# tonyckc/WT-PSE-code

Hardware: AMD Instinct MI355X
Metric: training images/sec (256x256 fundus) — full WT-PSE iteration (higher is better)
Workload: dtype f32 (layers with > 16 output channels and the fused 1x1 heads: x2h (2 fp16 terms per fp32 operand — power-of-two operand scaling —, 3 fp16 MFMA products per multiply, fp32 accumulation); the 16-channel layers the same on 16x16x32, the 1-/3-channel input layers and small 1x1 convs fp32-input MFMA)

## Files before the change

include/wtpse_hip.h:

```cpp
#ifndef WTPSE_HIP_H
#define WTPSE_HIP_H
#ifdef __cplusplus
extern "C" {
#endif


int wtpse_pack_conv_weights(const float* params, const int* desc, int n_desc, float* packed, void* stream);

int wtpse_conv_fwd(const float* in0, int C0, const float* in1, int C1, const float* wpacked, const float* bias,
                   const float* pro0, const float* pro1, int pro_relu, float* out0, float* out1, int Csplit, float* stats,
                   int B, int H, int W, int Cout, int ksize, int relu_out, const float* mask_ref, unsigned* out_amax, void* stream);
int wtpse_conv_stats_blocks(int B, int H, int W);
int wtpse_conv_fwd_gram(const float* in0, int C0, const float* wpacked, const float* bias, const float* pro0, int pro_relu,
                        float* out0, float* gram_partial, int B, int H, int W, int Cout, int relu_out, unsigned* out_amax,
                        void* stream);

int wtpse_conv_x3_stats_blocks(int B, int H, int W, int Cout, int ksize);
int wtpse_x3r_enable(int on);
int wtpse_x3_xcd(int on);
int wtpse_x3_small_wide(int on);
int wtpse_x3_terms(int terms);
int wtpse_amax(const float* x, long long n, unsigned* amax_table, void* stream);
int wtpse_pack_conv_weights_x3(const float* params, const int* desc, int n_desc, unsigned short* packed, void* stream);
int wtpse_conv_fwd_x3(const float* in0, int C0, const float* in1, int C1, const unsigned short* wpacked, const float* bias,
                      const float* pro0, const float* pro1, int pro_relu, float* out0, float* out1, int Csplit, float* stats,
                      int B, int H, int W, int Cout, int ksize, int relu_out, const float* mask_ref, const unsigned* in_amax,
                      const unsigned* in_amax1, unsigned* out_amax, void* stream);

int wtpse_conv16_x3(const float* in0, int C0, const unsigned short* wx16, const float* bias, const float* pro0, int pro_relu,
                    float* out0, float* stats, float* gram_partial, const float* mask_ref, const float* bn_ss,
                    const float* bn_mean, int bn_relu, int B, int H, int W, int Cout, int relu_out, int in_is_grad,
                    const unsigned* in_amax, unsigned* out_amax, void* stream);
int wtpse_pack_conv16_x3(const float* params, const int* desc, int n_desc, unsigned short* packed, void* stream);

int wtpse_dgrad_bnb(const float* dy, int C, const float* wpacked, float* out0, float* out1, int Csplit, const float* bn_y,
                    const float* bn_ss, const float* bn_mean, int bn_relu, int bn_c0, int bn_c1, float* stats, int B, int H, int W,
                    int Cout, int ksize, void* stream);
int wtpse_dgrad_x3_bnb(const float* dy, int C, const unsigned short* wpacked, float* out0, float* out1, int Csplit,
                       const float* bn_y, const float* bn_ss, const float* bn_mean, int bn_relu, int bn_c0, int bn_c1, float* stats,
                       int B, int H, int W, int Cout, int ksize, const unsigned* in_amax, void* stream);

int wtpse_conv_fwd_bnf(const float* in0, int C0, const float* in1, int C1, const void* wpacked, int layout, const float* bias,
                       const float* pro0, const float* pro1, int pro_relu, float* out0, float* stats, const float* gamma,
                       const float* beta, float* running_mean, float* running_var, long long* num_batches, float momentum, float eps,
                       float* scale_shift, float* save_mean, float* save_invstd, double* partial2, unsigned* tickets, int B, int H,
                       int W, int Cout, int ksize, const unsigned* in_amax0, const unsigned* in_amax1, unsigned* act_amax, void* stream);

int wtpse_bnb_tail_partial2(int nblk, int Cout);
int wtpse_bnb_tail_tickets(int nblk, int Cout);
int wtpse_dgrad_bnb_coef(const float* dy, int C, const void* wpacked, int layout, float* out0, float* out1, int Csplit,
                         const float* bn_y, const float* bn_ss, const float* bn_mean, int bn_relu, int bn_c0, int bn_c1,
                         float* stats, const float* gamma, const float* invstd, float* coef, float* dgamma, float* dbeta,
                         int accumulate, double* partial2, unsigned* tickets, int B, int H, int W, int Cout, int ksize,
                         const unsigned* in_amax, void* stream);
int wtpse_dgrad_bnb_coef_frozen(const float* dy, int C, const void* wpacked, int layout, float* out0, float* out1, int Csplit,
                                const float* bn_y, const float* bn_ss, const float* bn_mean, int bn_relu, int bn_c0, int bn_c1,
                                float* stats, const float* gamma, const float* invstd, float* coef, float* dgamma, float* dbeta,
                                float* dbias, int accumulate, double* partial2, unsigned* tickets, int B, int H, int W, int Cout,
                                int ksize, const unsigned* in_amax, void* stream);

int wtpse_conv_wgrad(const float* dy, const float* x0, int C0, const float* x1, int C1, const float* pro0,
                     const float* pro1, int pro_relu, float* slab, float* dbias_slab, int ksplit, float* dw, float* dbias, int accumulate, int B, int H,
                     int W, int Cout, int ksize, void* stream);
int wtpse_wgrad_ksplit(int B, int H, int W, int Cin, int Cout);
int wtpse_wgrad_x3_supported(int Cin, int Cout, int ksize, int C0);
int wtpse_wgrad_x3_ksplit(int B, int H, int W, int Cin, int Cout);
int wtpse_conv_wgrad_x3(const float* dy, const float* x0, int C0, const float* x1, int C1, const float* pro0,
                        const float* pro1, int pro_relu, float* slab, int ksplit, float* dw, int accumulate, int B, int H, int W,
                        int Cout, int ksize, void* stream);

int wtpse_wgrad_r_supported(int Cin, int Cout, int ksize, int C0, int W);
int wtpse_wgrad_r_slabs(int B, int H, int W, int Cin, int Cout);
int wtpse_conv_wgrad_r(const float* dy, const float* x0, int C0, const float* x1, int C1, const float* pro0,
                       const float* pro1, int pro_relu, float* slab, float* dbias_slab, int nslab, float* dw, float* dbias,
                       int accumulate, int B, int H, int W, int Cout, const unsigned* dy_amax, const unsigned* x_amax0,
                       const unsigned* x_amax1, void* stream);

int wtpse_conv_wgrad_r_bn(const float* g, const float* bn_y, const float* bn_coef, const float* x0, int C0, const float* x1,
                          int C1, const float* pro0, const float* pro1, int pro_relu, float* slab, int nslab, float* dw,
                          int accumulate, int B, int H, int W, int Cout, void* stream);

int wtpse_bn_finalize(const float* stats_partial, int nblk, int C, long long count, const float* gamma, const float* beta,
                      float* running_mean, float* running_var, long long* num_batches, float momentum, float eps,
                      float* scale_shift, float* save_mean, float* save_invstd, unsigned* act_amax, void* stream);
int wtpse_act_bound(const float* scale_shift, int C, const unsigned* raw_amax, unsigned* act_amax, void* stream);
int wtpse_bn_eval_coeffs(const float* gamma, const float* beta, const float* running_mean, const float* running_var,
                         float eps, int C, float* scale_shift, void* stream);
int wtpse_affine_act(const float* y, const float* scale_shift, int relu, float* z, int B, int C, int HW, void* stream);
int wtpse_bn_bwd(const float* dz, const float* y, const float* scale_shift, int relu, const float* gamma,
                 const float* save_mean, const float* save_invstd, float* partial, float* coef, float* dgamma,
                 float* dbeta, int accumulate, float* dy, int B, int C, int HW, unsigned* amax, void* stream);
int wtpse_bn_bwd_nsplit(int B, int C, int HW);
int wtpse_bn_bwd_reduce(const float* dz, const float* y, const float* scale_shift, int relu, const float* save_mean,
                        const float* save_invstd, float* partial, float* sums_local, int B, int C, int HW, void* stream);
int wtpse_bn_bwd_apply(const float* dz, const float* y, const float* scale_shift, int relu, const float* gamma,
                       const float* save_mean, const float* save_invstd, const float* sums_local, const float* sums_global,
                       long long count_global, float* coef, float* dgamma, float* dbeta, int accumulate, float* dy, int B,
                       int C, int HW, unsigned* amax, void* stream);
int wtpse_bn_bwd_from_stats(const float* g, const float* y, const float* stats_partial, int nblk, const float* gamma,
                            const float* save_mean, const float* save_invstd, float* coef, float* dgamma, float* dbeta,
                            int accumulate, float* dy, int B, int C, int HW, unsigned* amax, void* stream);

int wtpse_bn_bwd_finalize_coef(const float* stats_partial, int nblk, int C, long long count, const float* gamma,
                               const float* save_mean, const float* save_invstd, float* coef, float* dgamma, float* dbeta,
                               int accumulate, void* stream);
int wtpse_bn_bwd_apply_coef(const float* g, const float* y, const float* coef, float* dy, int B, int C, int HW, unsigned* amax, void* stream);

int wtpse_bn_eval_coeffs_stats(const float* gamma, const float* beta, const float* running_mean, const float* running_var,
                               float eps, int C, float* scale_shift, float* save_mean, float* save_invstd, void* stream);
int wtpse_bn_bwd_frozen(const float* dz, const float* y, const float* scale_shift, int relu, const float* gamma,
                        const float* mean, const float* invstd, float* partial, float* coef, float* dgamma, float* dbeta,
                        float* dbias, int accumulate, float* dy, int B, int C, int HW, unsigned* amax, void* stream);
int wtpse_bn_bwd_from_stats_frozen(const float* g, const float* stats_partial, int nblk, const float* gamma, const float* invstd,
                                   float* coef, float* dgamma, float* dbeta, float* dbias, int accumulate, float* dy, int B, int C,
                                   int HW, unsigned* amax, void* stream);
int wtpse_bn_bwd_finalize_coef_frozen(const float* stats_partial, int nblk, int C, const float* gamma, const float* invstd,
                                      float* coef, float* dgamma, float* dbeta, float* dbias, int accumulate, void* stream);
int wtpse_bn_bwd_scale_coef(const float* g, const float* coef, float* dy, int B, int C, int HW, unsigned* amax, void* stream);

int wtpse_wt_loss_fwd(const float* z, int B, int C, int HW, float eps, float margin, int domain_num, int per_domain,
                      float* partial, float* gram, float* v, float* offdiag, float* diag, double* rowval,
                      float* dmmd_dv, float* losses, void* stream);
int wtpse_wt_split(int B, int HW, int* chunk_out);
int wtpse_wt_loss_fwd_partials(const float* partial, int S, int B, int HW, float eps, float margin, int domain_num,
                               int per_domain, float* gram, float* v, float* offdiag, float* diag, double* rowval,
                               float* dmmd_dv, float* losses, void* stream);
int wtpse_wt_gram_fwd(const float* z, int B, int C, int HW, float eps, float* partial, float* gram, float* v, float* offdiag,
                      float* diag, void* stream);
int wtpse_wt_final(const float* offdiag, const float* diag, int B, int Bnorm, float margin, const double* rowval, int R,
                   float* losses, void* stream);
int wtpse_wt_loss_bwd(const float* z, int B, int C, int HW, float margin, int domain_num, int per_domain,
                      const float* gram, const float* offdiag, const float* diag, const float* dmmd_dv,
                      const float* g_off, const float* g_diag, const float* g_dom, float w_off, float w_diag, float w_dom,
                      float* Mws, float* dz, int accumulate, void* stream);
int wtpse_wt_combine(const float* losses, int nmaps, float den, int mode, float* out, void* stream);
int wtpse_mmd_fwd(const float* v, int domain_num, int per_domain, double* rowval, float* dmmd_dv, void* stream);

int wtpse_maxpool2_fwd(const float* x, const float* pro, int relu, float* out, int B, int C, int H, int W, void* stream);
int wtpse_maxpool2_bwd(const float* x, const float* pro, int relu, const float* dout, float* dx, int accumulate, int B,
                       int C, int H, int W, void* stream);
int wtpse_maxpool2_bwd_stats_blocks(int B, int H, int W);
int wtpse_maxpool2_bwd_bnb(const float* x, const float* pro, int relu, const float* dout, float* dx, int accumulate,
                           const float* mean, float* stats, int B, int C, int H, int W, void* stream);
int wtpse_upsample2x_fwd(const float* x, const float* pro, int relu, float* out, int B, int C, int H, int W, void* stream);
int wtpse_upsample2x_bwd(const float* dout, float* dx, int accumulate, int B, int C, int H, int W, unsigned* amax, void* stream);
int wtpse_upsample2x_bwd_bn(const float* g, const float* bn_y, const float* bn_coef, float* dx, int B, int C, int H, int W,
                            unsigned* amax, void* stream);
int wtpse_upsample2x_fwd_stats(const float* x, float* out, float* stats, int B, int C, int H, int W, void* stream);
int wtpse_upsample2x_stats_blocks(int B, int H, int W);

int wtpse_resize_bilinear(const float* x, float* out, int B, int C, int H, int W, int Ho, int Wo, void* stream);

int wtpse_attn_fuse_fwd(const float* z, const float* wb, const float* emb, float coef, float* att, float* att_pre,
                        float* mask, float* fuse, int B, int CE, int HW, void* stream);
int wtpse_attn_fuse_bwd(const float* dfuse, const float* z, const float* emb, const float* att, const float* wb, float coef,
                        float* demb, float* dz, float* partial, float* d_wb, int accumulate, int B, int CE, int HW,
                        void* stream);

int wtpse_reparam_fwd(const float* mu, const float* logvar, const float* eps, float* z, long long n, void* stream);
int wtpse_reparam_bwd(const float* dz, const float* logvar, const float* eps, float* dlogvar, long long n, void* stream);
int wtpse_exp_half(const float* logvar, float* std_, long long n, void* stream);
int wtpse_reparam_student(const float* mu, const float* std_, const float* eps, float* z, long long n, void* stream);
int wtpse_nan_scrub(float* x, long long n, int* flag, void* stream);
int wtpse_randn(float* out, long long n, unsigned long long seed, unsigned long long offset,
                const unsigned long long* offset_dev, void* stream);
int wtpse_counter_add(void* counter, long long inc, int is64, void* stream);

int wtpse_reduce_blocks(long long n);
int wtpse_bce_sigmoid_fwd(const float* x, const float* t, long long n, float* partial, float* loss, void* stream);
int wtpse_bce_sigmoid_bwd(const float* x, const float* t, const float* g, float w, long long n, float* dx, void* stream);
int wtpse_pos_weight(const float* mask, const float* t, long long n, float* partial, float* sums, float* pw, void* stream);
int wtpse_pos_weight_from_sums(const float* sums, float* pw, void* stream);
int wtpse_bce_logits_pw_fwd(const float* x, const float* mask, const float* t, const float* pw, long long n, float* partial,
                            float* loss, void* stream);
int wtpse_bce_logits_pw_bwd(const float* x, const float* mask, const float* t, const float* pw, const float* g, float w,
                            long long n, float* dx, void* stream);
int wtpse_mse_fwd(const float* a, const float* b, long long n, float* partial, float* loss, void* stream);
int wtpse_mse_bwd(const float* a, const float* b, const float* g, float w, long long n, float* da, void* stream);
int wtpse_roi(const float* image, const float* logit, float* roi, float* od_pred, int B, int C, int HW, void* stream);
int wtpse_adam(float* p, const float* g, float* m, float* v, long long n, double lr, double beta1, double beta2, double eps,
               int step, const int* step_dev, void* stream);
int wtpse_adam_dev(float* p, const float* g, float* m, float* v, long long n, const float* lr_dev, double beta1, double beta2,
                   double eps, int step, const int* step_dev, const int* hold, void* stream);
int wtpse_loss_log(const float* s0, const float* s1, const float* s2, const float* s3, const float* s4, const float* s5,
                   double* acc, int check_n, int* flag, const int* step_dev, void* stream);

int wtpse_avg_step(float* a0, const float* p0, long long n0, float* a1, const float* p1, long long n1, float* a2, const float* p2,
                   long long n2, float* a3, const float* p3, long long n3, int* count, const int* gate, const int* hold, void* stream);
int wtpse_avg_merge(float* acc, const float* seg, long long n, long long n_acc, long long n_seg, void* stream);

int wtpse_head_fwd(const float* x, const float* pro, int pro_relu, const float* w1, const float* b1, const float* w2,
                   const float* b2, const float* w3, const float* b3, int nc, float* h1, float* h2, float* y,
                   const unsigned* x_amax, int B, int HW, void* stream);
int wtpse_head_bwd(const float* dy, const float* x, const float* pro, int pro_relu, const float* h1, const float* h2,
                   const float* w1, const float* b1, const float* w2, const float* w3, int nc, float* dx, float* slab,
                   float* dparams, int accumulate, const unsigned* x_amax, const unsigned* dy_amax, int B, int HW, void* stream);
int wtpse_head_slabs(int B, int HW);

int wtpse_resample_u8(const unsigned char* in, unsigned char* out, const int* bounds, const int* kk, const int* tab, int ksize,
                      int N, int Hin, int Win, int C, int L, int vertical, void* stream);
int wtpse_input_finish(const unsigned char* img, const unsigned char* od, const int* xidx, const int* yidx, float* image,
                       float* od_out, float* oc_out, int N, int S, void* stream);
int wtpse_image_finish(const unsigned char* img, float* image, int N, int S, void* stream);

int wtpse_uniform_f64(double* out, long long n, unsigned long long seed, unsigned long long pos, void* stream);
int wtpse_aug_blur(const double* src, double* dst, const double* w, const int* src_index, int radius, int planes, int S, int axis,
                   int pre, double post, void* stream);
int wtpse_aug_geometry(const unsigned char* img, const unsigned char* od, const int* xidx, const int* yidx, const int* code,
                       unsigned char* img_out, unsigned char* mask_out, int N, int S, void* stream);
int wtpse_aug_warp(const unsigned char* img, const unsigned char* mask, const double* disp, const int* slot, unsigned char* img_out,
                   unsigned char* mask_out, int N, int S, void* stream);
int wtpse_aug_photometric(unsigned char* img, const unsigned char* lut, const int* rect, const int* pts, const int* pt_off,
                          const int* pt_val, int max_pts, int N, int S, void* stream);

int wtpse_postprocess_ws(int B, int h, int w);
int wtpse_postprocess(const float* logit, unsigned char* out, void* ws, float threshold, int B, int h, int w, void* stream);
int wtpse_seg_metrics_ws(int B, int h, int w);
int wtpse_seg_metrics(const unsigned char* mask, const float* label, long long* rec, void* ws, int B, int h, int w, void* stream);

int wtpse_overlay_ws(int B, int h, int w);
int wtpse_overlay(const float* img, const unsigned char* pred_od, const unsigned char* pred_oc, const unsigned char* gt_od,
                  const unsigned char* gt_oc, unsigned char* original, unsigned char* overlay, void* ws, int B, int h, int w,
                  void* stream);
int wtpse_label_thresholds(const unsigned char* mask, float* od, float* oc, long long n, void* stream);

int wtpse_overlay_pred_ws(int B, int h, int w);
int wtpse_overlay_pred(const float* img, const unsigned char* pred_od, const unsigned char* pred_oc, unsigned char* original,
                       unsigned char* overlay, int B, int h, int w, void* stream);
int wtpse_label_map(const unsigned char* disc, const unsigned char* cup, unsigned char* out, long long n, void* stream);
int wtpse_mask_geometry(const unsigned char* mask, long long* rec, int B, int h, int w, void* stream);
int wtpse_onh_profile(const unsigned char* disc, const unsigned char* cup, const long long* geom, const int* table, unsigned* profile,
                      long long* moments, int N, int B, int h, int w, void* stream);

int wtpse_locate_cells(const unsigned char* img, long long* cells, int N, int H, int W, int c, int t, void* stream);
int wtpse_crop_u8(const unsigned char* img, const int* boxes, unsigned char* out, int H, int W, int C, int M, int s, void* stream);
int wtpse_paste_u8(unsigned char* canvas, const unsigned char* patch, int H, int W, int C, int h, int w, int top, int left, void* stream);

#define WTPSE_CAL_BINS 1024
#define WTPSE_CAL_REC (2 * (WTPSE_CAL_BINS + 1) * 2 + 4)
int wtpse_calibration_hist(const float* prob, const float* spread, const float* label, const unsigned char* region, float threshold,
                           unsigned* rec, int B, int h, int w, void* stream);

int wtpse_shape_samples(const float* emb, int CE, const float* mu, const float* logvar, const float* wb, float coef,
                        const float* wout, const float* bout, const float* wz, float scale, int K, unsigned long long seed,
                        unsigned long long offset, const float* noise, float threshold, float* mean, float* std_,
                        unsigned char* votes, float* logits, int B, int HW, void* stream);

int wtpse_shape_samples_mask(const float* ref, float* mean, float* std_, unsigned char* votes, float* logits, int K, int B, int HW,
                             void* stream);

int wtpse_dihedral_views(const float* x, float* out, const int* codes, int V, int N, int S, void* stream);

int wtpse_views_merge(const float* logits, const int* codes, int V, int B, int K, int S, float threshold, float* logits_out,
                      float* mean, float* std_, unsigned char* votes, float* mean_logit, void* stream);

int wtpse_relu_mask(const float* dz, const float* ref, float* dy, int accumulate, long long n, void* stream);
int wtpse_axpy(float* dst, const float* src, float alpha, long long n, void* stream);
int wtpse_reduce_rows(const float* partial, int rows, int cols, float* out, int accumulate, float scale, void* stream);
int wtpse_zero(void* p, long long nbytes, void* stream);
int wtpse_copy_probe(const float* src, float* dst, long long n, int bytes_per_lane, void* stream);

int wtpse_dwt2_fwd(const float* x, float* coef, float* tmp, int planes, int H, int W, int wavelet, int levels, void* stream);
int wtpse_dwt2_inv(const float* coef, float* x, float* tmp, int planes, int H, int W, int wavelet, int levels, void* stream);

int wtpse_plan_fn_count(void);
const char* wtpse_plan_fn_name(int id);
void* wtpse_plan_create(void);
int wtpse_plan_destroy(void* plan);
int wtpse_plan_size(void* plan);
int wtpse_plan_add_call(void* plan, int fn, const void* args, int nargs, void* stream);
int wtpse_plan_add_wait(void* plan, void* waiter, void* waited);
int wtpse_plan_replay(void* plan);
int wtpse_tuning_state(void);

const char* wtpse_source_hash(void);

#ifdef __cplusplus
}
#endif
#endif
```

wt-pse-code_amd/wtpse_hip/csrc/conv.hip:

```cpp
#include "internal.h"

#define WTPSE_P16_KC(KS) ((KS) == 3 ? 4 : 8)

struct ConvArgs {
  const float* in0;
  const float* in1;
  const float* wp;
  const float* bias;
  const float* pro0;
  const float* pro1;
  float* out0;
  float* out1;
  float* stats;
  const float* mask;
  const unsigned* in_amax;
  float in_scale;
  unsigned* out_amax;
  float* gram;
  const float* bn_ss;
  const float* bn_mean;
  int bn_c0, bn_c1, bn_relu;
  BnbTail tail;
  BnfTail ftail;
  int B, H, W;
  int C0, C1, Cin, CinP;
  int Cout, CoutP, Csplit;
  int pro_relu;
  int relu_out;
  int tiles_x, tiles_y;
  int xcd_tiles;
};


template <bool P16> struct AccT { typedef f32x16 type; };
template <> struct AccT<true> { typedef f32x4 type; };
__device__ __forceinline__ f32x4 mfma(float a, float b, f32x4 c) { return mfma16(a, b, c); }
__device__ __forceinline__ f32x16 mfma(float a, float b, f32x16 c) { return mfma32(a, b, c); }

template <int PE>
struct PlaneStride {
  static constexpr int value = ((PE - 16 + 31) / 32) * 32 + 16;
};

template <int KS, int MODE, int TWL, bool DB, int EPI>
__global__ __launch_bounds__(256, 3) void conv_fwd_k(ConvArgs a) {
  constexpr bool MASK = EPI == 1, BNB = EPI == 2;
  constexpr int TAPS = KS * KS, PAD = KS / 2;
  constexpr int TW = 1 << TWL, TH = 256 / TW;
  constexpr int PITCH = TW + 2 * PAD, ROWS = TH + 2 * PAD;
  constexpr int PE = PITCH * ROWS;
  constexpr int NPOS = (PE + 255) / 256;
  constexpr int S = PlaneStride<NPOS * 256>::value;
  constexpr bool XP = (MODE == 3 || MODE == 4);
  constexpr int XT = MODE == 4 ? 2 : 3;
  constexpr bool P16 = (MODE == 0) || XP;
  static_assert(!XP || KS == 3, "MODE 3 / 4 is the 3x3 path");
  constexpr int MT = P16 ? 1 : MODE;
  constexpr int MB = P16 ? 16 : 32;
  constexpr int CB = MB * MT;
  constexpr int NT = P16 ? 4 : 2;
  constexpr int NB = P16 ? 16 : 32;
  constexpr int KC = P16 ? WTPSE_P16_KC(KS) : 8;
  constexpr int KQ = P16 ? 4 : 2;
  constexpr int NACC = P16 ? 4 : 16;
  constexpr int CB4 = CB / 4;
  constexpr int NW = (KC * TAPS * CB4 + 255) / 256;
  constexpr int PEP = (PE + 7) & ~7;
  constexpr int XS_SZ = XP ? 2 * XT * PEP * 4 : KC * S;
  constexpr int WS_SZ = XP ? 0 : NW * 1024;
  constexpr int GRAM_SZ = (P16 && KS == 3) ? 4 * 16 * 65 + 4 * 256 : 0;
  constexpr int RED_SZ = 4 * CB * 2 > GRAM_SZ ? 4 * CB * 2 : GRAM_SZ;
  constexpr int MAIN_SZ = (XS_SZ + WS_SZ) > RED_SZ ? (XS_SZ + WS_SZ) : RED_SZ;
  __shared__ __attribute__((aligned(16))) float smem[MAIN_SZ + CB + (BNB ? 4 * CB : 0)];
  float* bias_s = smem + MAIN_SZ;
  const float* bnp_s = bias_s + CB;
  float* Xs = smem;
  float* Ws = smem + XS_SZ;

  const int tid = threadIdx.x, lane = tid & 63, wave = tid >> 6;
  int tile = (int)blockIdx.x, cblk = (int)blockIdx.y;
  if (a.xcd_tiles > 0) {
    const int L = (int)(blockIdx.y * gridDim.x + blockIdx.x), sl = L >> 3;
    cblk = sl % (int)gridDim.y;
    tile = (L & 7) * a.xcd_tiles + sl / (int)gridDim.y;
  }
  int bx = tile;
  const int tx = bx % a.tiles_x;
  bx /= a.tiles_x;
  const int ty = bx % a.tiles_y;
  const int b = bx / a.tiles_y;
  const int cout0 = cblk * CB;
  const int HW = a.H * a.W;
  if (tid < CB) bias_s[tid] = (a.bias && cout0 + tid < a.Cout) ? a.bias[cout0 + tid] : 0.f;
  if (BNB && tid < CB) {
    const int c = cout0 + tid;
    const bool bn = c >= a.bn_c0 && c < a.bn_c1;
    float* q = bias_s + CB + tid;
    q[0] = (bn && a.bn_relu) ? a.bn_ss[2 * (c - a.bn_c0)] : 0.f;
    q[CB] = (bn && a.bn_relu) ? a.bn_ss[2 * (c - a.bn_c0) + 1] : 1.f;
    q[2 * CB] = bn ? a.bn_mean[c - a.bn_c0] : 0.f;
  }

  int off[NT];
#pragma unroll
  for (int nt = 0; nt < NT; ++nt) {
    int p = wave * 64 + nt * NB + (lane & (NB - 1));
    off[nt] = (p >> TWL) * PITCH + (p & (TW - 1));
  }

  typename AccT<P16>::type acc[MT][NT];
#pragma unroll
  for (int mt = 0; mt < MT; ++mt)
#pragma unroll
    for (int nt = 0; nt < NT; ++nt)
#pragma unroll
      for (int r = 0; r < NACC; ++r) acc[mt][nt][r] = 0.f;

  if constexpr (XP) {
    u32x4* Xq = reinterpret_cast<u32x4*>(smem);
    const int g4 = lane >> 4;
    constexpr int PB = (PE + 63) / 64, NIT = (2 * PB + 3) / 4;
    const __amdgpu_buffer_rsrc_t rs0 = make_rsrc(a.in0 + (size_t)b * a.C0 * HW, (unsigned)a.C0 * HW * 4u);
    const bool any_pro = MODE == 4 || a.pro0 != nullptr || a.pro_relu != 0;
    const unsigned sx_raw = MODE == 4 ? amax_load(a.in_amax) : 0u;
    __builtin_amdgcn_sched_barrier(0);
    float xv[NIT][8];
    int ipos[NIT], ihalf[NIT];
    bool iin[NIT];
    float psc[2][8], psh[2][8];
#pragma unroll
    for (int hh = 0; hh < 2; ++hh)
#pragma unroll
      for (int j = 0; j < 8; ++j) {
        const int cg = min(hh * 8 + j, a.C0 - 1);
        psc[hh][j] = a.pro0 ? a.pro0[2 * cg] : 1.f;
        psh[hh][j] = a.pro0 ? a.pro0[2 * cg + 1] : 0.f;
      }
#pragma unroll
    for (int i = 0; i < NIT; ++i) {
      const int blk = __builtin_amdgcn_readfirstlane(i * 4 + wave);
      ihalf[i] = blk >= PB ? 1 : 0;
      const int p = (blk - ihalf[i] * PB) * 64 + lane;
      ipos[i] = (blk < 2 * PB && p < PE) ? p : -1;
      const int r = p / PITCH, x = p - r * PITCH;
      const int gy = ty * TH + r - PAD, gx = tx * TW + x - PAD;
      iin[i] = ipos[i] >= 0 && gy >= 0 && gy < a.H && gx >= 0 && gx < a.W;
      const unsigned vo = iin[i] ? (unsigned)(gy * a.W + gx) * 4u : BUF_OOB;
#pragma unroll
      for (int j = 0; j < 8; ++j)
        xv[i][j] = buf_load(rs0, vo, (unsigned)min(ihalf[i] * 8 + j, a.C0) * (unsigned)HW * 4u);
    }
    const u32x4* wq = reinterpret_cast<const u32x4*>(a.wp) + 1 + (MODE == 4 ? 15 * 64 : 0);
    u32x4 afr[5][XT];
#pragma unroll
    for (int s5 = 0; s5 < 5; ++s5)
#pragma unroll
      for (int t = 0; t < XT; ++t) afr[s5][t] = wq[(s5 * XT + t) * 64 + lane];
    const float sx = MODE == 4 ? (a.in_amax ? x3_scale_from_amax(amax_reduce(sx_raw)) : a.in_scale) : 1.f;
    if constexpr (MODE == 4) {
#pragma unroll
      for (int hh = 0; hh < 2; ++hh)
#pragma unroll
        for (int j = 0; j < 8; ++j) {
          psc[hh][j] *= sx;
          psh[hh][j] *= sx;
        }
    }
    if (any_pro) {
      const float lo = (a.pro_relu & 1) ? 0.f : -INFINITY;
#pragma unroll
      for (int i = 0; i < NIT; ++i) {
        const int nc = iin[i] ? a.C0 - ihalf[i] * 8 : 0;
#pragma unroll
        for (int j = 0; j < 8; ++j) {
          const float sc = ihalf[i] ? psc[1][j] : psc[0][j], sh = ihalf[i] ? psh[1][j] : psh[0][j];
          const float v = fmaxf(fmaf(xv[i][j], sc, sh), lo);
          xv[i][j] = j < nc ? v : 0.f;
        }
      }
    }
#pragma unroll
    for (int i = 0; i < NIT; ++i) {
      if (ipos[i] >= 0) {
        u32x4 tt[XT];
#pragma unroll
        for (int j = 0; j < 4; ++j) {
          unsigned q0, q1, q2 = 0u;
          if constexpr (XT == 3) wt_split3_pair(xv[i][2 * j], xv[i][2 * j + 1], q0, q1, q2);
          else split2h_pair(xv[i][2 * j], xv[i][2 * j + 1], q0, q1);
          tt[0][j] = q0; tt[1][j] = q1;
          if constexpr (XT == 3) tt[2][j] = q2;
        }
#pragma unroll
        for (int t = 0; t < XT; ++t) Xq[(t * 2 + ihalf[i]) * PEP + ipos[i]] = tt[t];
      }
    }
    __syncthreads();
    int toff[5];
#pragma unroll
    for (int s5 = 0; s5 < 5; ++s5) {
      const int t = min(2 * s5 + (g4 >> 1), TAPS - 1);
      toff[s5] = (t / KS) * PITCH + (t % KS);
    }
    const int hsel = (g4 & 1) * PEP;
#pragma unroll
    for (int nt = 0; nt < NT; ++nt) {
#pragma unroll
      for (int s5 = 0; s5 < 5; ++s5) {
        u32x4 bfr[XT];
#pragma unroll
        for (int t = 0; t < XT; ++t) bfr[t] = Xq[(t * 2) * PEP + hsel + off[nt] + toff[s5]];
        f32x4 c = acc[0][nt];
        if constexpr (XT == 3) {
          c = wt_mfma16x32(afr[s5][0], bfr[2], c);
          c = wt_mfma16x32(afr[s5][1], bfr[1], c);
          c = wt_mfma16x32(afr[s5][2], bfr[0], c);
          c = wt_mfma16x32(afr[s5][0], bfr[1], c);
          c = wt_mfma16x32(afr[s5][1], bfr[0], c);
          c = wt_mfma16x32(afr[s5][0], bfr[0], c);
        } else {
          c = wt_mfma16x32h(afr[s5][0], bfr[1], c);
          c = wt_mfma16x32h(afr[s5][1], bfr[0], c);
          c = wt_mfma16x32h(afr[s5][0], bfr[0], c);
        }
        acc[0][nt] = c;
      }
    }
    if constexpr (MODE == 4) {
      const float inv = a.wp[0] / sx;
#pragma unroll
      for (int nt = 0; nt < NT; ++nt) acc[0][nt] *= inv;
    }
    __syncthreads();
  } else {
  int gpos[NPOS];
#pragma unroll
  for (int i = 0; i < NPOS; ++i) {
    int p = tid + 256 * i;
    int r = p / PITCH, x = p - r * PITCH;
    int gy = ty * TH + r - PAD, gx = tx * TW + x - PAD;
    gpos[i] = (p < PE && gy >= 0 && gy < a.H && gx >= 0 && gx < a.W) ? gy * a.W + gx : -1;
  }

  const __amdgpu_buffer_rsrc_t rs0 = make_rsrc(a.in0 + (size_t)b * a.C0 * HW, (unsigned)a.C0 * HW * 4u);
  const __amdgpu_buffer_rsrc_t rs1 = a.in1 ? make_rsrc(a.in1 + (size_t)b * a.C1 * HW, (unsigned)a.C1 * HW * 4u) : rs0;
  unsigned voff[NPOS];
#pragma unroll
  for (int i = 0; i < NPOS; ++i) voff[i] = gpos[i] >= 0 ? (unsigned)gpos[i] * 4u : BUF_OOB;
  const __amdgpu_buffer_rsrc_t rsw = make_rsrc(a.wp, (unsigned)a.CinP * TAPS * (unsigned)a.CoutP * 4u);
  unsigned woff[NW];
#pragma unroll
  for (int it = 0; it < NW; ++it) {
    const int e4 = tid + 256 * it;
    const int row = e4 / CB4, j4 = e4 - row * CB4;
    woff[it] = (row < KC * TAPS && cout0 + j4 * 4 < a.CoutP) ? (unsigned)(row * a.CoutP + cout0 + j4 * 4) * 4u : BUF_OOB;
  }
  const bool any_pro = a.pro0 != nullptr || a.pro1 != nullptr || a.pro_relu != 0;
  float xv[KC][NPOS];
  f32x4 wv[NW];
  auto issue_loads = [&](int c0) {
    const bool first = c0 < a.C0;
    const __amdgpu_buffer_rsrc_t rs = first ? rs0 : rs1;
    const int cbase = first ? c0 : c0 - a.C0;
    const int cmax = (first ? a.C0 : a.C1) - 1;
#pragma unroll
    for (int c = 0; c < KC; ++c) {
      const unsigned soff = (unsigned)min(cbase + c, cmax) * (unsigned)HW * 4u;
#pragma unroll
      for (int i = 0; i < NPOS; ++i) xv[c][i] = buf_load(rs, voff[i], soff);
    }
#pragma unroll
    for (int it = 0; it < NW; ++it) wv[it] = buf_load4(rsw, woff[it], (unsigned)(c0 * TAPS) * (unsigned)a.CoutP * 4u);
  };
  auto stash = [&](int c0) {
    const bool first = c0 < a.C0;
    if (any_pro) {
      const bool relu = first ? (a.pro_relu & 1) : (a.pro_relu & 2);
      const float* pro = first ? a.pro0 : a.pro1;
      const int cbase = first ? c0 : c0 - a.C0;
      const int cmax = (first ? a.C0 : a.C1) - 1;
#pragma unroll
      for (int c = 0; c < KC; ++c) {
        const int cg = min(cbase + c, cmax);
        const float sc = pro ? pro[2 * cg] : 1.f, sh = pro ? pro[2 * cg + 1] : 0.f;
#pragma unroll
        for (int i = 0; i < NPOS; ++i) {
          float v = fmaf(xv[c][i], sc, sh);
          if (relu) v = fmaxf(v, 0.f);
          xv[c][i] = gpos[i] >= 0 ? v : 0.f;
        }
      }
    }
#pragma unroll
    for (int c = 0; c < KC; ++c)
#pragma unroll
      for (int i = 0; i < NPOS; ++i) Xs[c * S + tid + 256 * i] = xv[c][i];
#pragma unroll
    for (int it = 0; it < NW; ++it) *reinterpret_cast<f32x4*>(Ws + (tid + 256 * it) * 4) = wv[it];
  };
  if (DB) issue_loads(0);
  for (int c0 = 0; c0 < a.CinP; c0 += KC) {
    const int kc = min(KC, a.CinP - c0);
    __syncthreads();
    if (!DB) issue_loads(c0);
    stash(c0);
    __syncthreads();
    if (DB && c0 + KC < a.CinP) issue_loads(c0 + KC);
    const int nq = kc / KQ;
    for (int q = 0; q < nq; ++q) {
      const int cl = q * KQ + (lane / NB);
      const float* xrow = Xs + cl * S;
      const float* wrow = Ws + cl * TAPS * CB + (lane & (MB - 1));
      float av[TAPS][MT], bv[TAPS][NT];
#pragma unroll
      for (int t = 0; t < TAPS; ++t) {
        const int toff = (t / KS) * PITCH + (t % KS);
#pragma unroll
        for (int mt = 0; mt < MT; ++mt) av[t][mt] = wrow[t * CB + mt * MB];
#pragma unroll
        for (int nt = 0; nt < NT; ++nt) bv[t][nt] = xrow[off[nt] + toff];
      }
#pragma unroll
      for (int t = 0; t < TAPS; ++t)
#pragma unroll
        for (int nt = 0; nt < NT; ++nt)
#pragma unroll
          for (int mt = 0; mt < MT; ++mt) acc[mt][nt] = mfma(av[t][mt], bv[t][nt], acc[mt][nt]);
    }
  }
  }
  if (a.bias) {
    float bz[MT][NACC];
#pragma unroll
    for (int mt = 0; mt < MT; ++mt)
#pragma unroll
      for (int r = 0; r < NACC; ++r)
        bz[mt][r] = bias_s[P16 ? ((lane >> 4) * 4 + r) : (mt * 32 + (r & 3) + 8 * (r >> 2) + 4 * (lane >> 5))];
#pragma unroll
    for (int mt = 0; mt < MT; ++mt)
#pragma unroll
      for (int r = 0; r < NACC; ++r)
#pragma unroll
        for (int nt = 0; nt < NT; ++nt) acc[mt][nt][r] += bz[mt][r];
  }

  const bool want_stats = a.stats != nullptr;
  if (want_stats) __syncthreads();
  float* red = smem;
  const int C1out = a.Cout - a.Csplit;
  int poff[NT];
#pragma unroll
  for (int nt = 0; nt < NT; ++nt) {
    int p = wave * 64 + nt * NB + (lane & (NB - 1));
    int gy = ty * TH + (p >> TWL), gx = tx * TW + (p & (TW - 1));
    poff[nt] = (gy < a.H && gx < a.W) ? gy * a.W + gx : -1;
  }
  const __amdgpu_buffer_rsrc_t rs_o0 = make_rsrc(a.out0 + (size_t)b * a.Csplit * HW, (unsigned)a.Csplit * HW * 4u);
  const __amdgpu_buffer_rsrc_t rs_o1 = a.out1 ? make_rsrc(a.out1 + (size_t)b * C1out * HW, (unsigned)C1out * HW * 4u) : rs_o0;
  const int Cbn = a.bn_c1 - a.bn_c0;
  const __amdgpu_buffer_rsrc_t rs_m = MASK ? make_rsrc(a.mask + (size_t)b * a.Cout * HW, (unsigned)a.Cout * HW * 4u)
                                      : BNB ? make_rsrc(a.mask + (size_t)b * Cbn * HW, (unsigned)Cbn * HW * 4u) : rs_o0;
  const int clane = P16 ? (lane >> 4) * 4 : (lane >> 5) * 4;
  unsigned pvo[NT];
#pragma unroll
  for (int nt = 0; nt < NT; ++nt) pvo[nt] = poff[nt] >= 0 ? (unsigned)(clane * HW + poff[nt]) * 4u : BUF_OOB;
  constexpr int NSV = NACC * 2;
  const bool full = ty * TH + TH <= a.H && tx * TW + TW <= a.W && cout0 + CB <= a.Cout;
  if (!full) {
#pragma unroll
    for (int mt = 0; mt < MT; ++mt)
#pragma unroll
      for (int r = 0; r < NACC; ++r) {
        const bool cvalid = cout0 + (P16 ? r : (mt * 32 + (r & 3) + 8 * (r >> 2))) + clane < a.Cout;
#pragma unroll
        for (int nt = 0; nt < NT; ++nt) acc[mt][nt][r] = (cvalid && poff[nt] >= 0) ? acc[mt][nt][r] : 0.f;
      }
  }
  if (a.relu_out) {
#pragma unroll
    for (int mt = 0; mt < MT; ++mt)
#pragma unroll
      for (int nt = 0; nt < NT; ++nt)
#pragma unroll
        for (int r = 0; r < NACC; ++r) acc[mt][nt][r] = out_clamp<EPI>(acc[mt][nt][r], 0.f);
  }
  if constexpr (P16 && KS == 3) {
    if (a.gram) {
      __syncthreads();
      float* zs = smem + wave * (16 * 65);
#pragma unroll
      for (int nt = 0; nt < NT; ++nt)
#pragma unroll
        for (int r = 0; r < NACC; ++r) zs[((lane >> 4) * 4 + r) * 65 + nt * 16 + (lane & 15)] = acc[0][nt][r];
      __builtin_amdgcn_wave_barrier();
      f32x4 g = {0.f, 0.f, 0.f, 0.f};
#pragma unroll
      for (int st = 0; st < 16; ++st) {
        const float v = zs[(lane & 15) * 65 + 4 * st + (lane >> 4)];
        g = mfma16(v, v, g);
      }
      float* gs = smem + 4 * 16 * 65 + wave * 256;
#pragma unroll
      for (int r = 0; r < 4; ++r) gs[((lane >> 4) * 4 + r) * 16 + (lane & 15)] = g[r];
      __syncthreads();
      const float* g0 = smem + 4 * 16 * 65;
      a.gram[(size_t)tile * 256 + tid] = g0[tid] + g0[256 + tid] + g0[512 + tid] + g0[768 + tid];
      __syncthreads();
    }
  }
  if constexpr (EPI == 0) {
    if (a.out_amax) {
      unsigned am = 0u;
#pragma unroll
      for (int mt = 0; mt < MT; ++mt)
#pragma unroll
        for (int nt = 0; nt < NT; ++nt)
#pragma unroll
          for (int r = 0; r < NACC; ++r) am = max(am, amax_bits(acc[mt][nt][r]));
      amax_publish_wave(a.out_amax, am, (unsigned)tile * 4u + (unsigned)wave);
    }
  }
  const unsigned hw4 = (unsigned)HW * 4u;
  const bool defer = want_stats && (BNB ? a.tail.tickets != nullptr : a.ftail.tickets != nullptr);
#pragma unroll
  for (int mt = 0; mt < MT; ++mt) {
    float mk[NACC][NT];
    if (MASK) {
#pragma unroll
      for (int r = 0; r < NACC; ++r) {
        const int cbase = cout0 + (P16 ? r : (mt * 32 + (r & 3) + 8 * (r >> 2)));
#pragma unroll
        for (int nt = 0; nt < NT; ++nt) mk[r][nt] = buf_load(rs_m, pvo[nt], (unsigned)min(cbase, a.Cout) * hw4);
      }
    }
    if (BNB) {
#pragma unroll
      for (int r = 0; r < NACC; ++r) {
        const int cbase = cout0 + (P16 ? r : (mt * 32 + (r & 3) + 8 * (r >> 2)));
        const bool bn = cbase >= a.bn_c0 && cbase < a.bn_c1;
        const unsigned soff = (unsigned)(bn ? cbase - a.bn_c0 : 0) * hw4;
#pragma unroll
        for (int nt = 0; nt < NT; ++nt) mk[r][nt] = buf_load(rs_m, bn ? pvo[nt] : BUF_OOB, soff);
      }
    }
    float bmu[NACC];
#pragma unroll
    for (int r = 0; r < NACC; ++r) {
      const int cbase = cout0 + (P16 ? r : (mt * 32 + (r & 3) + 8 * (r >> 2)));
      const bool second = a.out1 != nullptr && cbase >= a.Csplit;
      const __amdgpu_buffer_rsrc_t rs_o = second ? rs_o1 : rs_o0;
      const unsigned soff = (unsigned)(second ? min(cbase, a.Cout) - a.Csplit : min(cbase, a.Csplit)) * hw4;
      float bsc = 0.f, bsh = 1.f;
      bmu[r] = 0.f;
      if (BNB) {
        const int crel = (P16 ? r : (mt * 32 + (r & 3) + 8 * (r >> 2))) + clane;
        bsc = bnp_s[crel];
        bsh = bnp_s[CB + crel];
        bmu[r] = bnp_s[2 * CB + crel];
      }
#pragma unroll
      for (int nt = 0; nt < NT; ++nt) {
        float v = acc[mt][nt][r];
        if (MASK && !(mk[r][nt] > 0.f)) v = 0.f;
        if (BNB) {
          float zz = __builtin_fmaf(mk[r][nt], bsc, bsh);
          asm volatile("" : "+v"(zz));
          if (!(zz > 0.f)) v = 0.f;
          acc[mt][nt][r] = v;
        }
        if (!defer) buf_store(rs_o, pvo[nt], soff, v);
      }
    }
    if (want_stats) {
      float sv[NSV];
#pragma unroll
      for (int r = 0; r < NACC; ++r) {
        float s1 = 0.f, s2 = 0.f;
#pragma unroll
        for (int nt = 0; nt < NT; ++nt) {
#pragma clang fp contract(off)
          if (BNB) {
            const float v = acc[mt][nt][r];
            s1 += v;
            s2 += v * (mk[r][nt] - bmu[r]);
          } else {
            const float v = acc[mt][nt][r];
            s1 += v;
            s2 += v * v;
          }
        }
        sv[r * 2 + 0] = s1;
        sv[r * 2 + 1] = s2;
      }
      constexpr int LB = P16 ? 4 : 5;
      constexpr int HB = P16 ? 3 : 5;
#pragma unroll
      for (int st = 0; st < HB; ++st) {
        const int half = NSV >> (st + 1);
        const bool up = (lane >> st) & 1;
#pragma unroll
        for (int i = 0; i < NSV / 2; ++i) {
          if (i < half) {
            float keep = up ? sv[i + half] : sv[i];
            float send = up ? sv[i] : sv[i + half];
            sv[i] = keep + __shfl_xor(send, 1 << st, 64);
          }
        }
      }
#pragma unroll
      for (int st = HB; st < LB; ++st) sv[0] += __shfl_xor(sv[0], 1 << st, 64);
      int idx = 0;
#pragma unroll
      for (int st = 0; st < HB; ++st) idx += ((lane >> st) & 1) * (NSV >> (st + 1));
      const int k = idx & 1, rr = idx >> 1;
      const int crel = P16 ? ((lane >> 4) * 4 + rr) : (mt * 32 + (rr & 3) + 8 * (rr >> 2) + 4 * (lane >> 5));
      if (((lane & (NB - 1)) >> HB) == 0) red[(wave * CB + crel) * 2 + k] = sv[0];
    }
  }
  if (want_stats) {
    __syncthreads();
    if (tid < CB * 2) {
      int crel = tid >> 1;
      const float s = red[tid] + red[CB * 2 + tid] + red[2 * CB * 2 + tid] + red[3 * CB * 2 + tid];
      if (BNB) {
        const int c = cout0 + crel;
        if (c >= a.bn_c0 && c < a.bn_c1) pub_store(a.stats + ((size_t)tile * Cbn + c - a.bn_c0) * 2 + (tid & 1), s);
      } else if (cout0 + crel < a.Cout) {
        pub_store(a.stats + ((size_t)tile * a.Cout + cout0 + crel) * 2 + (tid & 1), s);
      }
    }
  }
  TailTicket tk;
  tk.old = 0u;
  tk.armed = 0;
  if (defer) {
    if constexpr (BNB) tk = bnb_tail_begin<CB>(a.tail, a.bn_c0, a.bn_c1, cout0, tile, cblk, tid);
    else tk = bnf_tail_begin(a.ftail, tile, cblk, tid);
  }
  if (defer) {
#pragma unroll
    for (int mt = 0; mt < MT; ++mt)
#pragma unroll
      for (int r = 0; r < NACC; ++r) {
        const int cbase = cout0 + (P16 ? r : (mt * 32 + (r & 3) + 8 * (r >> 2)));
        const bool second = a.out1 != nullptr && cbase >= a.Csplit;
        const __amdgpu_buffer_rsrc_t rs_o = second ? rs_o1 : rs_o0;
        const unsigned soff = (unsigned)(second ? min(cbase, a.Cout) - a.Csplit : min(cbase, a.Csplit)) * hw4;
#pragma unroll
        for (int nt = 0; nt < NT; ++nt) buf_store(rs_o, pvo[nt], soff, acc[mt][nt][r]);
      }
    if constexpr (BNB)
      bnb_tail<CB>(tk, a.tail, a.stats, a.bn_mean, a.bn_c0, a.bn_c1, cout0, tile, cblk, tid,
                   reinterpret_cast<double*>(red), reinterpret_cast<int*>(red + 520));
    else
      bnf_tail<CB>(tk, a.ftail, a.stats, a.Cout, cout0, tile, cblk, tid, reinterpret_cast<double*>(red),
                   reinterpret_cast<int*>(red + 520));
  }
}

template <int KS, int MODE, bool DB, int EPI>
static int launch_fwd(const ConvArgs& a, hipStream_t st) {
  constexpr int CB = (MODE == 0 || MODE == 3 || MODE == 4) ? 16 : 32 * MODE;
  ConvArgs args = a;
  const Tiling t = conv_tiling(a.B, a.H, a.W);
  args.tiles_x = t.tiles_x;
  args.tiles_y = t.tiles_y;
  dim3 grid((unsigned)t.tiles, (unsigned)ceil_div(a.CoutP, CB));
  static const bool xcd_on = [] { const char* e = getenv("WTPSE_C16_XCD"); return !(e && e[0] == '0'); }();
  args.xcd_tiles = (xcd_on && grid.x % 8 == 0 && (long long)grid.x * grid.y >= 64) ? (int)(grid.x / 8) : 0;
  const bool in_launch = tail_in_launch((long long)grid.x * grid.y);
  if (!in_launch) args.tail.tickets = args.ftail.tickets = nullptr;
  if (args.tail.tickets) bnb_tail_geometry(args.tail, (int)grid.x, a.Cout, (double)a.B * a.H * a.W);
  if (args.ftail.tickets) bnf_tail_geometry(args.ftail, (int)grid.x, a.Cout, (double)a.B * a.H * a.W);
  if (t.TW == 16)
    hipLaunchKernelGGL((conv_fwd_k<KS, MODE, 4, DB, EPI>), grid, dim3(256), 0, st, args);
  else
    hipLaunchKernelGGL((conv_fwd_k<KS, MODE, 5, DB, EPI>), grid, dim3(256), 0, st, args);
  const int rc = wtpse_status();
  return rc == 0 && !in_launch ? tail_after_launch(a, (int)grid.x, st) : rc;
}

extern "C" int wtpse_conv_stats_blocks(int B, int H, int W) { return conv_tiling(B, H, W).tiles; }

static int conv_check(const ConvCall& c, int layout) {
  const BnbArgs& bn = c.bn;
  const BnbTail& t = c.tail;
  const BnfTail& f = c.ftail;
  const bool bnb = bn.mean != nullptr;
  WTPSE_REQUIRE(layout == CONV_FP32 || layout == CONV_X3 || layout == CONV_C16);
  WTPSE_REQUIRE(c.in0 && c.w && c.out0 && c.B > 0 && c.H > 0 && c.W > 0 && c.C0 > 0 && c.C1 >= 0 && c.Cout > 0);
  WTPSE_REQUIRE(c.ksize == 1 || c.ksize == 3);
  WTPSE_REQUIRE((c.C1 == 0) == (c.in1 == nullptr));
  WTPSE_REQUIRE(c.Csplit > 0 && c.Csplit <= c.Cout && ((c.Csplit == c.Cout) == (c.out1 == nullptr)));
  WTPSE_REQUIRE(c.Csplit == c.Cout || c.Csplit % 16 == 0);
  WTPSE_REQUIRE(!(c.stats && c.relu_out));
  WTPSE_REQUIRE(bnb || !(c.stats && c.mask_ref));
  WTPSE_REQUIRE(bnb || !(c.mask_ref && c.out1));
  WTPSE_REQUIRE(!bnb || (c.mask_ref && c.stats && bn.ss && !c.bias && !c.relu_out && !c.gram && bn.c0 >= 0 && bn.c0 < bn.c1 &&
                         bn.c1 <= c.Cout && bn.c0 % 16 == 0 && (bn.c1 % 16 == 0 || bn.c1 == c.Cout)));
  WTPSE_REQUIRE(c.C1 == 0 || c.C0 % 16 == 0);
  WTPSE_REQUIRE(!(c.out_amax && (c.mask_ref || bnb)));
  WTPSE_REQUIRE(!c.gram || (c.Cout == 16 && !c.relu_out));
  WTPSE_REQUIRE(!t.tickets || (bnb && t.partial2 && t.gamma && t.invstd && t.coef && t.dgamma && t.dbeta));
  WTPSE_REQUIRE(!f.tickets || (!bnb && c.stats && !c.gram && f.partial2 && f.gamma && f.beta && f.scale_shift && f.save_mean &&
                               f.save_invstd && (f.rmean == nullptr) == (f.rvar == nullptr)));
  if (layout == CONV_X3) {
    const X3Tiling g = x3_tiling(c.B, c.H, c.W, c.Cout, c.ksize);
    WTPSE_REQUIRE(!c.gram && !(c.in_amax1 && !c.in1) && ((c.C0 + c.C1 + 15) & ~15) <= (g.mt == 2 && !g.half ? 512 : 256));
  }
  if (layout == CONV_C16)
    WTPSE_REQUIRE(c.ksize == 3 && c.C0 <= 16 && c.Cout <= 16 && (((uintptr_t)c.w) & 15) == 0 && !c.in1 && !c.pro1);
  return 0;
}

static int conv_launch_fwd(const ConvCall& c, bool c16, hipStream_t st) {
  const bool bnb = c.bn.mean != nullptr;
  ConvArgs a;
  a.tail = c.tail;
  a.ftail = c.ftail;
  a.bn_ss = c.bn.ss; a.bn_mean = c.bn.mean; a.bn_relu = c.bn.relu; a.bn_c0 = bnb ? c.bn.c0 : 0; a.bn_c1 = bnb ? c.bn.c1 : 0;
  a.in0 = c.in0; a.in1 = c.in1; a.wp = static_cast<const float*>(c.w); a.bias = c.bias; a.pro0 = c.pro0; a.pro1 = c.pro1;
  a.out0 = c.out0; a.out1 = c.out1; a.stats = c.stats; a.mask = c.mask_ref; a.gram = c.gram;
  a.in_amax = c16 ? c.in_amax0 : nullptr; a.in_scale = c16 ? X3_FWD_SCALE : 1.f; a.out_amax = c.out_amax;
  a.B = c.B; a.H = c.H; a.W = c.W; a.C0 = c.C0; a.C1 = c.C1; a.Cin = c.C0 + c.C1; a.CinP = c16 ? 16 : (a.Cin + 3) & ~3;
  a.Cout = c.Cout; a.CoutP = (c.Cout + 15) & ~15; a.Csplit = c.Csplit; a.pro_relu = c.pro_relu; a.relu_out = c.relu_out;
  a.tiles_x = a.tiles_y = 0;
#define FWD(KS, M, DB) (bnb ? launch_fwd<KS, M, DB, 2>(a, st) : c.mask_ref ? launch_fwd<KS, M, DB, 1>(a, st) : launch_fwd<KS, M, DB, 0>(a, st))
  if (c16) return (g_x3_terms == 2 && (!c.in_is_grad || c.in_amax0)) ? FWD(3, 4, false) : FWD(3, 3, false);
  int mode = c.Cout <= 16 ? 0 : (c.Cout % 64 == 0 ? 2 : 1);
  const int tiles = conv_tiling(c.B, c.H, c.W).tiles;
  if (mode == 2 && tiles * (a.CoutP / 64) < 512) mode = 1;
  if (mode == 1 && tiles * ceil_div(a.CoutP, 32) < 384) mode = 0;
  const int cb = mode == 0 ? 16 : 32 * mode;
  const bool db = tiles * ceil_div(a.CoutP, cb) < 768 && a.CinP > (mode == 0 ? WTPSE_P16_KC(c.ksize) : 8);
#define FWD_DB(KS, M) (db ? FWD(KS, M, true) : FWD(KS, M, false))
  if (c.ksize == 3) return mode == 0 ? FWD_DB(3, 0) : mode == 1 ? FWD_DB(3, 1) : FWD_DB(3, 2);
  return mode == 0 ? FWD_DB(1, 0) : mode == 1 ? FWD_DB(1, 1) : FWD_DB(1, 2);
#undef FWD_DB
#undef FWD
}

int conv_run(const ConvCall& c, int layout, hipStream_t st) {
  if (const int rc = conv_check(c, layout)) return rc;
  return layout == CONV_X3 ? conv_launch_x3(c, st) : conv_launch_fwd(c, layout == CONV_C16, st);
}

extern "C" int wtpse_conv_fwd(const float* in0, int C0, const float* in1, int C1, const float* wpacked,
                              const float* bias, const float* pro0, const float* pro1, int pro_relu, float* out0, float* out1,
                              int Csplit, float* stats, int B, int H, int W, int Cout, int ksize, int relu_out,
                              const float* mask_ref, unsigned* out_amax, void* stream) {
  ConvCall c;
  c.in0 = in0; c.C0 = C0; c.in1 = in1; c.C1 = C1; c.w = wpacked; c.bias = bias; c.pro0 = pro0; c.pro1 = pro1; c.pro_relu = pro_relu;
  c.out0 = out0; c.out1 = out1; c.Csplit = Csplit; c.stats = stats; c.mask_ref = mask_ref; c.out_amax = out_amax;
  c.B = B; c.H = H; c.W = W; c.Cout = Cout; c.ksize = ksize; c.relu_out = relu_out;
  return conv_run(c, CONV_FP32, (hipStream_t)stream);
}

extern "C" int wtpse_dgrad_bnb(const float* dy, int C, const float* wpacked, float* out0, float* out1, int Csplit,
                               const float* bn_y, const float* bn_ss, const float* bn_mean, int bn_relu, int bn_c0, int bn_c1,
                               float* stats, int B, int H, int W, int Cout, int ksize, void* stream) {
  WTPSE_REQUIRE(bn_y && bn_ss && bn_mean && stats);
  ConvCall c;
  c.in0 = dy; c.C0 = C; c.w = wpacked; c.out0 = out0; c.out1 = out1; c.Csplit = Csplit; c.stats = stats; c.mask_ref = bn_y;
  c.bn.ss = bn_ss; c.bn.mean = bn_mean; c.bn.relu = bn_relu; c.bn.c0 = bn_c0; c.bn.c1 = bn_c1;
  c.B = B; c.H = H; c.W = W; c.Cout = Cout; c.ksize = ksize;
  return conv_run(c, CONV_FP32, (hipStream_t)stream);
}

extern "C" int wtpse_conv16_x3(const float* in0, int C0, const unsigned short* wx16, const float* bias, const float* pro0,
                               int pro_relu, float* out0, float* stats, float* gram_partial, const float* mask_ref,
                               const float* bn_ss, const float* bn_mean, int bn_relu, int B, int H, int W, int Cout, int relu_out,
                               int in_is_grad, const unsigned* in_amax, unsigned* out_amax, void* stream) {
  ConvCall c;
  c.in0 = in0; c.C0 = C0; c.w = wx16; c.bias = bias; c.pro0 = pro0; c.pro_relu = pro_relu; c.out0 = out0; c.Csplit = Cout;
  c.stats = stats; c.gram = gram_partial; c.mask_ref = mask_ref; c.in_amax0 = in_amax; c.in_is_grad = in_is_grad; c.out_amax = out_amax;
  c.bn.ss = bn_ss; c.bn.mean = bn_mean; c.bn.relu = bn_relu; c.bn.c1 = Cout;
  c.B = B; c.H = H; c.W = W; c.Cout = Cout; c.ksize = 3; c.relu_out = relu_out;
  return conv_run(c, CONV_C16, (hipStream_t)stream);
}

extern "C" int wtpse_conv_fwd_bnf(const float* in0, int C0, const float* in1, int C1, const void* wpacked, int layout,
                                  const float* bias, const float* pro0, const float* pro1, int pro_relu, float* out0, float* stats,
                                  const float* gamma, const float* beta, float* running_mean, float* running_var,
                                  long long* num_batches, float momentum, float eps, float* scale_shift, float* save_mean,
                                  float* save_invstd, double* partial2, unsigned* tickets, int B, int H, int W, int Cout, int ksize,
                                  const unsigned* in_amax0, const unsigned* in_amax1, unsigned* act_amax, void* stream) {
  WTPSE_REQUIRE(stats && gamma && beta && scale_shift && save_mean && save_invstd && partial2 && tickets);
  ConvCall c;
  c.in0 = in0; c.C0 = C0; c.in1 = in1; c.C1 = C1; c.w = wpacked; c.bias = bias; c.pro0 = pro0; c.pro1 = pro1; c.pro_relu = pro_relu;
  c.out0 = out0; c.Csplit = Cout; c.stats = stats; c.in_amax0 = in_amax0; c.in_amax1 = in_amax1;
  BnfTail& t = c.ftail;
  t.partial2 = partial2; t.tickets = tickets; t.gamma = gamma; t.beta = beta; t.rmean = running_mean; t.rvar = running_var;
  t.nbt = num_batches; t.momentum = momentum; t.eps = eps; t.scale_shift = scale_shift; t.save_mean = save_mean;
  t.save_invstd = save_invstd; t.act_amax = act_amax;
  c.B = B; c.H = H; c.W = W; c.Cout = Cout; c.ksize = ksize;
  return conv_run(c, layout, (hipStream_t)stream);
}

extern "C" int wtpse_bnb_tail_partial2(int nblk, int Cout) { return bnb_tail_groups(nblk) * bnb_tail_ctot(Cout) * 2; }
extern "C" int wtpse_bnb_tail_tickets(int nblk, int Cout) { return bnb_tail_t2off(nblk, Cout) + (Cout + 15) / 16; }

static int dgrad_bnb_coef(ConvCall c, int layout, void* stream) {
  const BnbTail& t = c.tail;
  WTPSE_REQUIRE(c.mask_ref && c.bn.ss && c.bn.mean && c.stats && t.gamma && t.invstd && t.coef && t.dgamma && t.dbeta && t.partial2 &&
                t.tickets);
  c.in_is_grad = 1;
  return conv_run(c, layout, (hipStream_t)stream);
}

extern "C" int wtpse_dgrad_bnb_coef(const float* dy, int C, const void* wpacked, int layout, float* out0, float* out1, int Csplit,
                                    const float* bn_y, const float* bn_ss, const float* bn_mean, int bn_relu, int bn_c0, int bn_c1,
                                    float* stats, const float* gamma, const float* invstd, float* coef, float* dgamma,
                                    float* dbeta, int accumulate, double* partial2, unsigned* tickets, int B, int H, int W,
                                    int Cout, int ksize, const unsigned* in_amax, void* stream) {
  ConvCall c;
  c.in0 = dy; c.C0 = C; c.w = wpacked; c.out0 = out0; c.out1 = out1; c.Csplit = Csplit; c.stats = stats; c.mask_ref = bn_y;
  c.bn.ss = bn_ss; c.bn.mean = bn_mean; c.bn.relu = bn_relu; c.bn.c0 = bn_c0; c.bn.c1 = bn_c1; c.in_amax0 = in_amax;
  BnbTail& t = c.tail;
  t.partial2 = partial2; t.tickets = tickets; t.gamma = gamma; t.invstd = invstd; t.coef = coef; t.dgamma = dgamma; t.dbeta = dbeta;
  t.accumulate = accumulate;
  c.B = B; c.H = H; c.W = W; c.Cout = Cout; c.ksize = ksize;
  return dgrad_bnb_coef(c, layout, stream);
}

extern "C" int wtpse_dgrad_bnb_coef_frozen(const float* dy, int C, const void* wpacked, int layout, float* out0, float* out1,
                                           int Csplit, const float* bn_y, const float* bn_ss, const float* bn_mean, int bn_relu,
                                           int bn_c0, int bn_c1, float* stats, const float* gamma, const float* invstd, float* coef,
                                           float* dgamma, float* dbeta, float* dbias, int accumulate, double* partial2,
                                           unsigned* tickets, int B, int H, int W, int Cout, int ksize, const unsigned* in_amax,
                                           void* stream) {
  WTPSE_REQUIRE(dbias);
  ConvCall c;
  c.in0 = dy; c.C0 = C; c.w = wpacked; c.out0 = out0; c.out1 = out1; c.Csplit = Csplit; c.stats = stats; c.mask_ref = bn_y;
  c.bn.ss = bn_ss; c.bn.mean = bn_mean; c.bn.relu = bn_relu; c.bn.c0 = bn_c0; c.bn.c1 = bn_c1; c.in_amax0 = in_amax;
  BnbTail& t = c.tail;
  t.partial2 = partial2; t.tickets = tickets; t.gamma = gamma; t.invstd = invstd; t.coef = coef; t.dgamma = dgamma; t.dbeta = dbeta;
  t.dbias = dbias; t.accumulate = accumulate;
  c.B = B; c.H = H; c.W = W; c.Cout = Cout; c.ksize = ksize;
  return dgrad_bnb_coef(c, layout, stream);
}

__global__ __launch_bounds__(256) void pack_weights_x3p16_k(const float* __restrict__ params, const int* __restrict__ desc,
                                                            unsigned short* __restrict__ packed) {
  const int* d = desc + blockIdx.y * 8;
  const int w_off = d[0], Co = d[1], Ci = d[2];
  const float* w = params + w_off;
  __shared__ float red[4];
  float m = 0.f;
  for (int e = threadIdx.x; e < Co * Ci * 9; e += 256) m = fmaxf(m, fabsf(w[e]));
  for (int o = 32; o > 0; o >>= 1) m = fmaxf(m, __shfl_xor(m, o, 64));
  if ((threadIdx.x & 63) == 0) red[threadIdx.x >> 6] = m;
  __syncthreads();
  m = fmaxf(fmaxf(red[0], red[1]), fmaxf(red[2], red[3]));
  const float sc = x3_scale_from_amax(__builtin_bit_cast(unsigned, m));
  for (int dir = 0; dir < 2; ++dir) {
    const int base = d[4 + dir];
    if (base < 0) continue;
    const int R = dir == 0 ? Co : Ci, K = dir == 0 ? Ci : Co;
    if (blockIdx.x == 0 && threadIdx.x == 0) {
      float* hdr = reinterpret_cast<float*>(packed + base);
      hdr[0] = 1.f / sc; hdr[1] = sc; hdr[2] = hdr[3] = 0.f;
    }
    for (int e = blockIdx.x * 256 + threadIdx.x; e < 5 * 64 * 8; e += gridDim.x * 256) {
      const int j = e & 7, lane = (e >> 3) & 63, s5 = e >> 9;
      const int row = lane & 15, g = lane >> 4;
      const int tap = 2 * s5 + (g >> 1), k = 8 * (g & 1) + j;
      float v = 0.f;
      if (tap < 9 && row < R && k < K) v = dir == 0 ? w[(row * Ci + k) * 9 + tap] : w[(k * Ci + row) * 9 + (8 - tap)];
      unsigned q0, q1, q2;
      wt_split3_pair(v, 0.f, q0, q1, q2);
      unsigned short* o = packed + base + 8;
      o[((s5 * 3 + 0) * 64 + lane) * 8 + j] = (unsigned short)(q0 & 0xFFFFu);
      o[((s5 * 3 + 1) * 64 + lane) * 8 + j] = (unsigned short)(q1 & 0xFFFFu);
      o[((s5 * 3 + 2) * 64 + lane) * 8 + j] = (unsigned short)(q2 & 0xFFFFu);
      split2h_pair(v * sc, 0.f, q0, q1);
      unsigned short* oh = o + 5 * 3 * 64 * 8;
      oh[((s5 * 2 + 0) * 64 + lane) * 8 + j] = (unsigned short)(q0 & 0xFFFFu);
      oh[((s5 * 2 + 1) * 64 + lane) * 8 + j] = (unsigned short)(q1 & 0xFFFFu);
    }
  }
}

extern "C" int wtpse_pack_conv16_x3(const float* params, const int* desc, int n_desc, unsigned short* packed, void* stream) {
  WTPSE_REQUIRE(params && desc && packed && n_desc > 0);
  hipLaunchKernelGGL(pack_weights_x3p16_k, dim3(2, n_desc), dim3(256), 0, (hipStream_t)stream, params, desc, packed);
  return wtpse_status();
}

extern "C" int wtpse_conv_fwd_gram(const float* in0, int C0, const float* wpacked, const float* bias, const float* pro0,
                                   int pro_relu, float* out0, float* gram_partial, int B, int H, int W, int Cout, int relu_out,
                                   unsigned* out_amax, void* stream) {
  WTPSE_REQUIRE(gram_partial);
  ConvCall c;
  c.in0 = in0; c.C0 = C0; c.w = wpacked; c.bias = bias; c.pro0 = pro0; c.pro_relu = pro_relu; c.out0 = out0; c.Csplit = Cout;
  c.gram = gram_partial; c.out_amax = out_amax;
  c.B = B; c.H = H; c.W = W; c.Cout = Cout; c.ksize = 3; c.relu_out = relu_out;
  return conv_run(c, CONV_FP32, (hipStream_t)stream);
}

__global__ __launch_bounds__(256) void pack_weights_k(const float* __restrict__ params, const int* __restrict__ desc,
                                                      float* __restrict__ packed) {
  const int* d = desc + blockIdx.y * 8;
  const int w_off = d[0], Co = d[1], Ci = d[2], T = d[3], wf_off = d[4], wd_off = d[5];
  const int CiP4 = (Ci + 3) & ~3, CoP16 = (Co + 15) & ~15;
  const int CoP4 = (Co + 3) & ~3, CiP16 = (Ci + 15) & ~15;
  const float* w = params + w_off;
  const int nf = wf_off >= 0 ? CiP4 * T * CoP16 : 0;
  for (int e = blockIdx.x * 256 + threadIdx.x; e < nf; e += gridDim.x * 256) {
    int co = e % CoP16;
    int t = (e / CoP16) % T;
    int ci = e / (CoP16 * T);
    packed[wf_off + e] = (co < Co && ci < Ci) ? w[(co * Ci + ci) * T + t] : 0.f;
  }
  if (wd_off >= 0) {
    const int nd = CoP4 * T * CiP16;
    for (int e = blockIdx.x * 256 + threadIdx.x; e < nd; e += gridDim.x * 256) {
      int ci = e % CiP16;
      int t = (e / CiP16) % T;
      int co = e / (CiP16 * T);
      packed[wd_off + e] = (co < Co && ci < Ci) ? w[(co * Ci + ci) * T + (T - 1 - t)] : 0.f;
    }
  }
}

extern "C" int wtpse_pack_conv_weights(const float* params, const int* desc, int n_desc, float* packed, void* stream) {
  WTPSE_REQUIRE(params && desc && packed && n_desc > 0);
  hipLaunchKernelGGL(pack_weights_k, dim3(16, n_desc), dim3(256), 0, (hipStream_t)stream, params, desc, packed);
  return wtpse_status();
}

struct WgradArgs {
  const float* dy;
  const float* x0;
  const float* x1;
  const float* pro0;
  const float* pro1;
  float* slab;
  float* dbias;
  int B, H, W, C0, C1, Cin, Cout;
  int pro_relu;
  int tiles_x, tiles_y, ntiles;
  int cg, ngroups, nblk;
};

template <int KS, bool P32, int TWL, int NBLK>
__global__ __launch_bounds__(256, 2) void conv_wgrad_k(WgradArgs a) {
  constexpr int TAPS = KS * KS, PAD = KS / 2;
  constexpr int TW = 1 << TWL, TH = 256 / TW;
  constexpr int PITCH = TW + 2 * PAD, ROWS = TH + 2 * PAD;
  constexpr int PE = PITCH * ROWS;
  constexpr int MB = P32 ? 32 : 16;
  constexpr int KQ = P32 ? 2 : 4;
  constexpr int NACC = P32 ? 16 : 4;
  constexpr int MAXNB = NBLK;
  constexpr int SA = P32 ? 257 : 258;
  constexpr int SX = P32 ? (PE | 1) : (((PE - 2 + 31) / 32) * 32 + 2);
  constexpr int TILE_SZ = MB * SA + MB * SX;
  constexpr int RED_SZ = P32 ? 4 * 1024 : 4 * MAXNB * 256;
  __shared__ float smem[TILE_SZ > RED_SZ ? TILE_SZ : RED_SZ];
  float* Ys = smem;
  float* Xs = smem + MB * SA;

  const int tid = threadIdx.x, lane = tid & 63, wave = tid >> 6;
  int bx = blockIdx.x, ky = blockIdx.y;
  if ((gridDim.y & 7) == 0) {
    const int lin = blockIdx.y * gridDim.x + blockIdx.x;
    const int k = lin >> 3;
    ky = (lin & 7) + 8 * (k / (int)gridDim.x);
    bx = k % (int)gridDim.x;
  }
  const int group = bx % a.ngroups;
  const int cout0 = (bx / a.ngroups) * MB;
  const int cin0 = group * a.cg;
  const int HW = a.H * a.W;
  const int j = lane & (MB - 1), kl = lane / MB;
  const bool any_pro = a.pro0 != nullptr || a.pro1 != nullptr || a.pro_relu != 0;

  int boff[MAXNB];
#pragma unroll
  for (int nb = 0; nb < MAXNB; ++nb) {
    int slot = nb * MB + j;
    int ci = slot % a.cg, t = slot / a.cg;
    boff[nb] = (t < TAPS) ? ci * SX + (t / KS) * PITCH + (t % KS) : 0;
  }
  typename AccT<!P32>::type acc[MAXNB];
#pragma unroll
  for (int nb = 0; nb < MAXNB; ++nb)
#pragma unroll
    for (int r = 0; r < NACC; ++r) acc[nb][r] = 0.f;
  double db = 0.0;

  const int tiles_per_img = a.tiles_x * a.tiles_y;
  int it = 0;
  for (int tile = ky; tile < a.ntiles; tile += gridDim.y, ++it) {
    const int b = tile / tiles_per_img;
    const int trem = tile - b * tiles_per_img;
    const int ty = trem / a.tiles_x, tx = trem - ty * a.tiles_x;
    __syncthreads();
    const int gyp = ty * TH + (tid >> TWL), gxp = tx * TW + (tid & (TW - 1));
    const int ypos = (gyp < a.H && gxp < a.W) ? gyp * a.W + gxp : -1;
    constexpr int NPOS = (PE + 255) / 256;
    int lpos[NPOS], gpos[NPOS];
#pragma unroll
    for (int i = 0; i < NPOS; ++i) {
      int p = tid + 256 * i;
      int r = p / PITCH, x = p - r * PITCH;
      int gy = ty * TH + r - PAD, gx = tx * TW + x - PAD;
      lpos[i] = p < PE ? p : -1;
      gpos[i] = (p < PE && gy >= 0 && gy < a.H && gx >= 0 && gx < a.W) ? gy * a.W + gx : -1;
    }
#pragma unroll
    for (int g = 0; g < MB / 16; ++g) {
      float yv[16];
      float xv[16][NPOS];
      const __amdgpu_buffer_rsrc_t rsy = make_rsrc(a.dy + (size_t)b * a.Cout * HW, (unsigned)a.Cout * HW * 4u);
      const int ch0 = cin0 + g * 16;
      const bool xfirst = ch0 < a.C0 || a.x1 == nullptr;
      const int xbase = xfirst ? ch0 : ch0 - a.C0;
      const int xmax = (xfirst ? a.C0 : a.C1) - 1;
      const __amdgpu_buffer_rsrc_t rsx = xfirst ? make_rsrc(a.x0 + (size_t)b * a.C0 * HW, (unsigned)a.C0 * HW * 4u)
                                                : make_rsrc(a.x1 + (size_t)b * a.C1 * HW, (unsigned)a.C1 * HW * 4u);
      const unsigned yoff = ypos >= 0 ? (unsigned)ypos * 4u : BUF_OOB;
      unsigned voff[NPOS];
#pragma unroll
      for (int i = 0; i < NPOS; ++i) voff[i] = gpos[i] >= 0 ? (unsigned)gpos[i] * 4u : BUF_OOB;
#pragma unroll
      for (int c = 0; c < 16; ++c)
        yv[c] = buf_load(rsy, yoff, (unsigned)min(cout0 + g * 16 + c, a.Cout - 1) * (unsigned)HW * 4u);
#pragma unroll
      for (int c = 0; c < 16; ++c) {
        const unsigned soff = (unsigned)min(xbase + c, xmax) * (unsigned)HW * 4u;
#pragma unroll
        for (int i = 0; i < NPOS; ++i) xv[c][i] = buf_load(rsx, voff[i], soff);
      }
      if (any_pro) {
        const bool relu = xfirst ? (a.pro_relu & 1) : (a.pro_relu & 2);
        const float* pro = xfirst ? a.pro0 : a.pro1;
#pragma unroll
        for (int c = 0; c < 16; ++c) {
          const int cgl = min(xbase + c, xmax);
          const float sc = pro ? pro[2 * cgl] : 1.f, sh = pro ? pro[2 * cgl + 1] : 0.f;
#pragma unroll
          for (int i = 0; i < NPOS; ++i) {
            float v = fmaf(xv[c][i], sc, sh);
            if (relu) v = fmaxf(v, 0.f);
            xv[c][i] = gpos[i] >= 0 ? v : 0.f;
          }
        }
      }
#pragma unroll
      for (int c = 0; c < 16; ++c) Ys[(g * 16 + c) * SA + tid] = yv[c];
#pragma unroll
      for (int c = 0; c < 16; ++c)
#pragma unroll
        for (int i = 0; i < NPOS; ++i)
          if (lpos[i] >= 0) Xs[(g * 16 + c) * SX + lpos[i]] = xv[c][i];
    }
    __syncthreads();
    if (a.dbias && group == 0) {
      int c = tid / (256 / MB), part = tid % (256 / MB);
      constexpr int PER = MB;
      float s = 0.f;
      for (int i = 0; i < PER; ++i) s += Ys[c * SA + part * PER + i];
      db += s;
    }
    constexpr int STEPS = 64 / KQ;
    const float* yrow = Ys + j * SA + wave * 64 + kl;
    auto lds_step = [&](int s, float& av, float (&bv)[MAXNB]) {
      const int pbase = wave * 64 + s * KQ;
      const int rowbase = (pbase >> TWL) * PITCH + (pbase & (TW - 1)) + kl;
      av = yrow[s * KQ];
      if constexpr (KS == 3 && NBLK == 9) {
        const float* xb = Xs + j * SX + rowbase;
#pragma unroll
        for (int nb = 0; nb < MAXNB; ++nb) bv[nb] = xb[(nb / 3) * PITCH + (nb % 3)];
      } else {
#pragma unroll
        for (int nb = 0; nb < MAXNB; ++nb) bv[nb] = Xs[boff[nb] + rowbase];
      }
    };
    float a0, a1, b0[MAXNB], b1[MAXNB];
    lds_step(0, a0, b0);
    for (int s = 0; s < STEPS; s += 2) {
      lds_step(s + 1, a1, b1);
      __builtin_amdgcn_sched_barrier(0);
#pragma unroll
      for (int nb = 0; nb < MAXNB; ++nb) acc[nb] = mfma(a0, b0[nb], acc[nb]);
      __builtin_amdgcn_sched_barrier(0);
      lds_step(s + 2 < STEPS ? s + 2 : s, a0, b0);
      __builtin_amdgcn_sched_barrier(0);
#pragma unroll
      for (int nb = 0; nb < MAXNB; ++nb) acc[nb] = mfma(a1, b1[nb], acc[nb]);
      __builtin_amdgcn_sched_barrier(0);
    }
  }

  float* slab = a.slab + (size_t)ky * a.Cout * a.Cin * TAPS;
  float* red = smem;
  if constexpr (!P32) {
    __syncthreads();
#pragma unroll
    for (int nb = 0; nb < MAXNB; ++nb)
#pragma unroll
      for (int r = 0; r < 4; ++r) red[((wave * MAXNB + nb) * 16 + (lane >> 4) * 4 + r) * 16 + j] = acc[nb][r];
    __syncthreads();
    for (int e = tid; e < MAXNB * 256; e += 256) {
      int nb = e >> 8, co = (e >> 4) & 15, jj = e & 15;
      float v = 0.f;
#pragma unroll
      for (int w = 0; w < 4; ++w) v += red[((w * MAXNB + nb) * 16 + co) * 16 + jj];
      int slot = nb * 16 + jj;
      int ci = slot % a.cg, t = slot / a.cg;
      if (t < TAPS && cout0 + co < a.Cout && cin0 + ci < a.Cin)
        slab[((size_t)(cout0 + co) * a.Cin + cin0 + ci) * TAPS + t] = v;
    }
  } else {
#pragma unroll
    for (int nb = 0; nb < MAXNB; ++nb) {
      {
        __syncthreads();
#pragma unroll
        for (int r = 0; r < 16; ++r) {
          int co = (r & 3) + 8 * (r >> 2) + 4 * (lane >> 5);
          red[(wave * 32 + co) * 32 + j] = acc[nb][r];
        }
        __syncthreads();
        for (int e = tid; e < 1024; e += 256) {
          int co = e >> 5, jj = e & 31;
          float v = red[e] + red[1024 + e] + red[2048 + e] + red[3072 + e];
          int slot = nb * 32 + jj;
          int ci = slot % a.cg, t = slot / a.cg;
          if (t < TAPS && cout0 + co < a.Cout && cin0 + ci < a.Cin)
            slab[((size_t)(cout0 + co) * a.Cin + cin0 + ci) * TAPS + t] = v;
        }
      }
    }
  }
  if (a.dbias && group == 0) {
    constexpr int TPC = 256 / MB;
    for (int m = 1; m <= TPC / 2; m <<= 1) db += __shfl_xor(db, m, 64);
    int c = tid / TPC;
    if ((tid % TPC) == 0 && cout0 + c < a.Cout) a.dbias[(size_t)ky * a.Cout + cout0 + c] = (float)db;
  }
}

__global__ __launch_bounds__(256) void wgrad_reduce_k(const float* __restrict__ slab, int ksplit, int n,
                                                      float* __restrict__ out, int accumulate, int nblk_w,
                                                      const float* __restrict__ slab_b, int n_b, float* __restrict__ out_b) {
  __shared__ double sh[8][32];
  const int j = threadIdx.x & 31, kq = threadIdx.x >> 5;
  int blk = blockIdx.x;
  if (blk >= nblk_w) { blk -= nblk_w; slab = slab_b; n = n_b; out = out_b; }
  const int i = blk * 32 + j;
  double s = 0.0;
  if (i < n)
    for (int k = kq; k < ksplit; k += 8) s += (double)slab[(size_t)k * n + i];
  sh[kq][j] = s;
  __syncthreads();
  if (kq == 0 && i < n) {
    double t = sh[0][j] + sh[1][j] + sh[2][j] + sh[3][j] + sh[4][j] + sh[5][j] + sh[6][j] + sh[7][j];
    out[i] = accumulate ? out[i] + (float)t : (float)t;
  }
}

__global__ __launch_bounds__(256) void wgrad_fold4_k(const float* __restrict__ slab, int ksplit, int n, float* __restrict__ out,
                                                     int accumulate) {
  __shared__ double sh[8][32][4];
  const int j = threadIdx.x & 31, kq = threadIdx.x >> 5;
  const int i = (blockIdx.x * 32 + j) * 4;
  double s0 = 0.0, s1 = 0.0, s2 = 0.0, s3 = 0.0;
  if (i < n) {
    int k = kq;
    for (; k + 24 < ksplit; k += 32) {
      const f32x4 a = *reinterpret_cast<const f32x4*>(slab + (size_t)k * n + i);
      const f32x4 b = *reinterpret_cast<const f32x4*>(slab + (size_t)(k + 8) * n + i);
      const f32x4 c = *reinterpret_cast<const f32x4*>(slab + (size_t)(k + 16) * n + i);
      const f32x4 d = *reinterpret_cast<const f32x4*>(slab + (size_t)(k + 24) * n + i);
      s0 += (double)a[0]; s1 += (double)a[1]; s2 += (double)a[2]; s3 += (double)a[3];
      s0 += (double)b[0]; s1 += (double)b[1]; s2 += (double)b[2]; s3 += (double)b[3];
// ... 108 lines not shown
```

wt-pse-code_amd/wtpse_hip/csrc/conv_x3.hip:

```cpp
#include "conv_x3_kernels.h"

int x3_dispatch_t1(const ConvX3Args& a, const X3Launch& L, hipStream_t st);
int x3_dispatch_t2(const ConvX3Args& a, const X3Launch& L, hipStream_t st);
int x3_dispatch_t3(const ConvX3Args& a, const X3Launch& L, hipStream_t st);

__global__ __launch_bounds__(1024) void pack_scale_x3_k(const float* __restrict__ params, const int* __restrict__ desc,
                                                        unsigned short* __restrict__ packed, int terms) {
  const int* d = desc + blockIdx.y * 8;
  const int n = d[1] * d[2] * d[3];
  const float* w = params + d[0];
  float m = 0.f;
  if (terms == 2)
    for (int e = blockIdx.x * 1024 + threadIdx.x; e < n; e += X3_WSLICES * 1024) m = fmaxf(m, fabsf(w[e]));
  __shared__ float red[16];
  for (int o = 32; o > 0; o >>= 1) m = fmaxf(m, __shfl_xor(m, o, 64));
  if ((threadIdx.x & 63) == 0) red[threadIdx.x >> 6] = m;
  __syncthreads();
  if (threadIdx.x == 0) {
    for (int i = 1; i < 16; ++i) m = fmaxf(m, red[i]);
    reinterpret_cast<float*>(packed + (d[4] >= 0 ? d[4] : d[5]))[4 + blockIdx.x] = m;
  }
}

__global__ __launch_bounds__(256) void pack_weights_x3_k(const float* __restrict__ params, const int* __restrict__ desc,
                                                         unsigned short* __restrict__ packed, int terms) {
  const int* d = desc + blockIdx.y * 8;
  const int w_off = d[0], Co = d[1], Ci = d[2], T = d[3];
  const float* w = params + w_off;
  for (int dir = 0; dir < 2; ++dir) {
    const int base = d[4 + dir];
    if (base < 0) continue;
    float sc = 1.f;
    if (terms == 2) {
      const float* part = reinterpret_cast<const float*>(packed + (d[4] >= 0 ? d[4] : d[5])) + 4;
      float m = 0.f;
#pragma unroll
      for (int i = 0; i < X3_WSLICES; ++i) m = fmaxf(m, part[i]);
      sc = x3_scale_from_amax(__builtin_bit_cast(unsigned, m));
    }
    if (blockIdx.x == 0 && threadIdx.x == 0) {
      float* hdr = reinterpret_cast<float*>(packed + base);
      hdr[0] = 1.f / sc;
      hdr[1] = sc;
      hdr[2] = hdr[3] = 0.f;
    }
    const int R = dir == 0 ? Co : Ci, K = dir == 0 ? Ci : Co;
    const int RP = (R + 31) & ~31, KP = (K + 15) & ~15;
    const int n = (KP / 8) * RP * T;
    for (int e = blockIdx.x * 256 + threadIdx.x; e < n; e += gridDim.x * 256) {
      const int row32 = e & 31, hh = (e >> 5) & 1;
      int q = e >> 6;
      const int t = q % T; q /= T;
      const int rb = q % (RP / 32), chunk = q / (RP / 32);
      const int row = rb * 32 + row32, k0 = chunk * 16 + hh * 8;
      float v[8];
#pragma unroll
      for (int k8 = 0; k8 < 8; ++k8) {
        const int k = k0 + k8;
        v[k8] = (row < R && k < K) ? (dir == 0 ? w[(row * Ci + k) * T + t] : w[(k * Ci + row) * T + (T - 1 - t)]) : 0.f;
      }
      u32x4v o0, o1, o2;
#pragma unroll
      for (int j = 0; j < 4; ++j) {
        unsigned q0, q1, q2;
        if (terms == 2) {
          split2h_pair(v[2 * j] * sc, v[2 * j + 1] * sc, q0, q1);
          q2 = 0u;
        } else {
          split3_pair(v[2 * j], v[2 * j + 1], q0, q1, q2);
        }
        o0[j] = q0; o1[j] = q1; o2[j] = q2;
      }
      const size_t slot = ((((size_t)chunk * (RP / 32) + rb) * T + t) * 6);
      u32x4v* o = reinterpret_cast<u32x4v*>(packed + base + X3_WHDR);
      o[(slot + 0 * 2 + hh) * 32 + row32] = o0;
      o[(slot + 1 * 2 + hh) * 32 + row32] = o1;
      o[(slot + 2 * 2 + hh) * 32 + row32] = o2;
    }
  }
}

int g_x3_terms = [] { const char* e = getenv("WTPSE_X3_TERMS"); return (e && e[0] >= '1' && e[0] <= '3') ? e[0] - '0' : 2; }();
extern "C" int wtpse_x3_terms(int terms) {
  const int was = g_x3_terms;
  if (terms >= 1 && terms <= 3) g_x3_terms = terms;
  return was;
}

extern "C" int wtpse_pack_conv_weights_x3(const float* params, const int* desc, int n_desc, unsigned short* packed, void* stream) {
  WTPSE_REQUIRE(params && desc && packed && n_desc > 0);
  hipLaunchKernelGGL(pack_scale_x3_k, dim3(X3_WSLICES, n_desc), dim3(1024), 0, (hipStream_t)stream, params, desc, packed, g_x3_terms);
  hipLaunchKernelGGL(pack_weights_x3_k, dim3(48, n_desc), dim3(256), 0, (hipStream_t)stream, params, desc, packed, g_x3_terms);
  return wtpse_status();
}

static int g_x3_small_wide = [] { const char* e = getenv("WTPSE_X3_SMALL_WIDE"); return (e && e[0] >= '0' && e[0] <= '1') ? e[0] - '0' : 0; }();
extern "C" int wtpse_x3_small_wide(int on) {
  const int was = g_x3_small_wide;
  if (on >= 0) g_x3_small_wide = on ? 1 : 0;
  return was;
}
static bool x3_small_tiles(int B, int H, int W, int CoutP, bool mt2) {
  if (mt2) return false;
  if (W > 16) return g_x3_small_wide != 0 && W % 32 == 0;
  return conv_tiling(B, H, W).tiles * (CoutP / 32) < 512;
}

static int g_x3r = [] { const char* e = getenv("WTPSE_X3R"); return (e && e[0] >= '0' && e[0] <= '2') ? e[0] - '0' : 1; }();
extern "C" int wtpse_x3r_enable(int on) {
  const int was = g_x3r;
  if (on >= 0) g_x3r = on > 2 ? 2 : on;
  return was;
}

static int g_x3_xcd = [] { const char* e = getenv("WTPSE_X3_XCD"); return (e && e[0] == '0') ? 0 : 1; }();
extern "C" int wtpse_x3_xcd(int on) {
  const int was = g_x3_xcd;
  if (on >= 0) g_x3_xcd = on ? 1 : 0;
  return was;
}

extern "C" int wtpse_tuning_state(void) { return g_x3_terms | (g_x3r << 4) | (g_x3_xcd << 8) | (g_x3_small_wide << 12); }

static bool x3_mt2(int B, int H, int W, int CoutP) {
  const int tiles = conv_tiling(B, H, W).tiles;
  bool mt2 = (CoutP % 64 == 0) && tiles * (CoutP / 64) >= 512;
  static const int mt_override = [] { const char* e = getenv("WTPSE_X3_MT"); return (e && (e[0] == '1' || e[0] == '2')) ? e[0] - '0' : 0; }();
  if (mt_override == 1) mt2 = false;
  if (mt_override == 2 && CoutP % 64 == 0) mt2 = true;
  return mt2;
}

static int g_x3_half_min = [] { const char* e = getenv("WTPSE_X3_HALF"); if (e && e[0] == '0') return 0;
                                const char* m = getenv("WTPSE_X3_HALF_MIN"); const int v = m ? atoi(m) : 256; return v > 0 ? v : 256; }();
static bool x3_half(int B, int H, int W, int CoutP, int ksize, bool mt2) {
  if (ksize != 3 || g_x3_half_min == 0 || g_x3r == 0 || CoutP % 64 != 0 || mt2) return false;
  return conv_tiling(B, H, W, 128).tiles * (CoutP / 64) >= g_x3_half_min;
}

X3Tiling x3_tiling(int B, int H, int W, int Cout, int ksize) {
  const int CoutP = (Cout + 31) & ~31;
  const bool mt2 = x3_mt2(B, H, W, CoutP);
  X3Tiling g;
  g.half = x3_half(B, H, W, CoutP, ksize, mt2) ? 1 : 0;
  g.small = !g.half && x3_small_tiles(B, H, W, CoutP, mt2) ? 1 : 0;
  g.mt = (mt2 || g.half) ? 2 : 1;
  g.px = (g.half || g.small) ? 128 : 256;
  g.t = conv_tiling(B, H, W, g.px);
  return g;
}

extern "C" int wtpse_conv_x3_stats_blocks(int B, int H, int W, int Cout, int ksize) { return x3_tiling(B, H, W, Cout, ksize).t.tiles; }

int conv_launch_x3(const ConvCall& c, hipStream_t st) {
  const bool bnb = c.bn.mean != nullptr;
  ConvX3Args a;
  a.in0 = c.in0; a.in1 = c.in1; a.wx = static_cast<const unsigned short*>(c.w); a.bias = c.bias; a.pro0 = c.pro0; a.pro1 = c.pro1;
  a.out0 = c.out0; a.out1 = c.out1; a.stats = c.stats; a.mask = c.mask_ref;
  a.in_amax = c.in_amax0; a.in_amax1 = c.in_amax1; a.in_scale = X3_FWD_SCALE; a.out_amax = c.out_amax;
  a.bn_ss = c.bn.ss; a.bn_mean = c.bn.mean; a.bn_relu = c.bn.relu; a.bn_c0 = bnb ? c.bn.c0 : 0; a.bn_c1 = bnb ? c.bn.c1 : 0;
  a.tail = c.tail;
  a.ftail = c.ftail;
  a.B = c.B; a.H = c.H; a.W = c.W; a.C0 = c.C0; a.C1 = c.C1; a.Cin = c.C0 + c.C1; a.CinP = (a.Cin + 15) & ~15;
  a.Cout = c.Cout; a.CoutP = (c.Cout + 31) & ~31; a.Csplit = c.Csplit; a.pro_relu = c.pro_relu; a.relu_out = c.relu_out;
  a.tiles_x = a.tiles_y = 0;
  X3Launch L;
  L.g = x3_tiling(c.B, c.H, c.W, c.Cout, c.ksize);
  L.ksize = c.ksize; L.epi = bnb ? 2 : c.mask_ref ? 1 : 0; L.x3r = g_x3r; L.xcd = g_x3_xcd;
  return g_x3_terms == 1 ? x3_dispatch_t1(a, L, st) : g_x3_terms == 2 ? x3_dispatch_t2(a, L, st) : x3_dispatch_t3(a, L, st);
}

extern "C" int wtpse_conv_fwd_x3(const float* in0, int C0, const float* in1, int C1, const unsigned short* wpacked,
                                 const float* bias, const float* pro0, const float* pro1, int pro_relu, float* out0, float* out1,
                                 int Csplit, float* stats, int B, int H, int W, int Cout, int ksize, int relu_out,
                                 const float* mask_ref, const unsigned* in_amax, const unsigned* in_amax1, unsigned* out_amax,
                                 void* stream) {
  ConvCall c;
  c.in0 = in0; c.C0 = C0; c.in1 = in1; c.C1 = C1; c.w = wpacked; c.bias = bias; c.pro0 = pro0; c.pro1 = pro1; c.pro_relu = pro_relu;
  c.out0 = out0; c.out1 = out1; c.Csplit = Csplit; c.stats = stats; c.mask_ref = mask_ref;
  c.in_amax0 = in_amax; c.in_amax1 = in_amax1; c.out_amax = out_amax;
  c.B = B; c.H = H; c.W = W; c.Cout = Cout; c.ksize = ksize; c.relu_out = relu_out;
  return conv_run(c, CONV_X3, (hipStream_t)stream);
}

extern "C" int wtpse_dgrad_x3_bnb(const float* dy, int C, const unsigned short* wpacked, float* out0, float* out1, int Csplit,
                                  const float* bn_y, const float* bn_ss, const float* bn_mean, int bn_relu, int bn_c0, int bn_c1,
                                  float* stats, int B, int H, int W, int Cout, int ksize, const unsigned* in_amax, void* stream) {
  WTPSE_REQUIRE(bn_y && bn_ss && bn_mean && stats);
  ConvCall c;
  c.in0 = dy; c.C0 = C; c.w = wpacked; c.out0 = out0; c.out1 = out1; c.Csplit = Csplit; c.stats = stats; c.mask_ref = bn_y;
  c.bn.ss = bn_ss; c.bn.mean = bn_mean; c.bn.relu = bn_relu; c.bn.c0 = bn_c0; c.bn.c1 = bn_c1; c.in_amax0 = in_amax;
  c.B = B; c.H = H; c.W = W; c.Cout = Cout; c.ksize = ksize;
  return conv_run(c, CONV_X3, (hipStream_t)stream);
}

typedef short s16x4 __attribute__((ext_vector_type(4)));
typedef short s16x8 __attribute__((ext_vector_type(8)));

struct WgradX3Args {
  const float* dy;
  const float* x0;
  const float* x1;
  const float* pro0;
  const float* pro1;
  float* slab;
  int B, H, W, C0, C1, Cin, Cout;
  int pro_relu;
  int tiles_x, tiles_y, ntiles;
  int nci;
};

__device__ __forceinline__ bf16x8 lds_tr8(const u32x4v* base, int byte_off) {
  typedef s16x4 __attribute__((address_space(3))) * lds_p;
  const char __attribute__((address_space(3)))* p =
      (const char __attribute__((address_space(3)))*)base + byte_off;
  const s16x4 lo = __builtin_amdgcn_ds_read_tr16_b64_v4i16((lds_p)p);
  const s16x4 hi = __builtin_amdgcn_ds_read_tr16_b64_v4i16((lds_p)(p + 64));
  const s16x8 v = __builtin_shufflevector(lo, hi, 0, 1, 2, 3, 4, 5, 6, 7);
  return __builtin_bit_cast(bf16x8, v);
}

constexpr int pad_plane(int n) {
  for (int m = n;; ++m)
    if (m % 16 == 4 || m % 16 == 12) return m;
}

#define WSPLIT(a, b, q0, q1, q2) split3_pair(a, b, q0, q1, q2)
#define WSTORE(dst, v) dst = v
template <int KS, int TWL, bool Q>
__global__ __launch_bounds__(256, 2) void conv_wgrad_x3_k(WgradX3Args a) {
  constexpr int TAPS = KS * KS, PAD = KS / 2;
  constexpr int NPX = Q ? 64 : 128;
  constexpr int TW = 1 << TWL, TH = NPX >> TWL;
  constexpr int PITCH = TW + 2 * PAD, ROWS = TH + 2 * PAD;
  constexpr int PE = PITCH * ROWS;
  constexpr int NCG = Q ? 8 : 4;
  constexpr int BLK = NCG * 8;
  constexpr int XP = pad_plane(PE), YP = pad_plane(NPX);
  constexpr int XS_U4 = 3 * NCG * XP, YS_U4 = 3 * NCG * YP;
  constexpr int RED_U4 = Q ? 0 : 4 * 1024 / 4;
  constexpr int SM_U4 = (XS_U4 + YS_U4) > RED_U4 ? (XS_U4 + YS_U4) : RED_U4;
  __shared__ u32x4v smem[SM_U4];
  u32x4v* Xs = smem;
  u32x4v* Ys = smem + XS_U4;

  const int tid = threadIdx.x, lane = tid & 63, wave = tid >> 6;
  int bx = blockIdx.x, ky = blockIdx.y;
  if ((gridDim.y & 7) == 0) {
    const int lin = blockIdx.y * gridDim.x + blockIdx.x;
    const int k = lin >> 3;
    ky = (lin & 7) + 8 * (k / (int)gridDim.x);
    bx = k % (int)gridDim.x;
  }
  const int cin0 = (bx % a.nci) * BLK, cout0 = (bx / a.nci) * BLK;
  const int HW = a.H * a.W;
  const int wco = Q ? (wave >> 1) : 0, wci = Q ? (wave & 1) : 0;
  const bool any_pro = a.pro0 != nullptr || a.pro1 != nullptr || a.pro_relu != 0;

  const int g = lane >> 4, q = (lane >> 2) & 3, p = lane & 3, h = g >> 1;
  const int cgl = 2 * (g & 1) + (p >> 1);
  const int a_base = (((wco * 4 + cgl) * YP) + 8 * h + q) * 16 + 8 * (p & 1);
  const int b_base = (((wci * 4 + cgl) * XP) + 8 * h + q) * 16 + 8 * (p & 1);

  f32x16 acc[TAPS];
#pragma unroll
  for (int t = 0; t < TAPS; ++t)
#pragma unroll
    for (int r = 0; r < 16; ++r) acc[t][r] = 0.f;

  constexpr int PBX = (PE + 63) / 64, NITX = (NCG * PBX + 3) / 4;
  constexpr int PBY = NPX / 64, NITY = NCG * PBY / 4;
  const int tiles_per_img = a.tiles_x * a.tiles_y;

  for (int tile = ky; tile < a.ntiles; tile += gridDim.y) {
    const int b = tile / tiles_per_img;
    const int trem = tile - b * tiles_per_img;
    const int ty = trem / a.tiles_x, tx = trem - ty * a.tiles_x;
    const __amdgpu_buffer_rsrc_t rsy = make_rsrc(a.dy + (size_t)b * a.Cout * HW, (unsigned)a.Cout * HW * 4u);
    const __amdgpu_buffer_rsrc_t rsx0 = make_rsrc(a.x0 + (size_t)b * a.C0 * HW, (unsigned)a.C0 * HW * 4u);
    const __amdgpu_buffer_rsrc_t rsx1 = a.x1 ? make_rsrc(a.x1 + (size_t)b * a.C1 * HW, (unsigned)a.C1 * HW * 4u) : rsx0;
    __syncthreads();
    auto x_item = [&](int i, float (&v)[8], int& cg, int& pos, bool& in, bool& first, int& cb, int& cn) {
      const int blk = __builtin_amdgcn_readfirstlane(i * 4 + wave);
      cg = blk / PBX;
      pos = (blk - cg * PBX) * 64 + lane;
      const int r = pos / PITCH, x = pos - r * PITCH;
      const int gy = ty * TH + r - PAD, gx = tx * TW + x - PAD;
      in = blk < NCG * PBX && pos < PE && gy >= 0 && gy < a.H && gx >= 0 && gx < a.W;
      if (blk >= NCG * PBX) pos = PE;
      const unsigned vo = in ? (unsigned)(gy * a.W + gx) * 4u : BUF_OOB;
      const int c = cin0 + min(cg, NCG - 1) * 8;
      first = c < a.C0 || a.x1 == nullptr;
      const __amdgpu_buffer_rsrc_t rs = first ? rsx0 : rsx1;
      cb = first ? c : c - a.C0;
      cn = first ? a.C0 : a.C1;
#pragma unroll
      for (int j = 0; j < 8; ++j) v[j] = buf_load(rs, vo, (unsigned)min(cb + j, cn) * (unsigned)HW * 4u);
    };
    auto x_finish = [&](float (&v)[8], int cg, int pos, bool in, bool first, int cb, int cn) {
      if (any_pro) {
        const bool relu = first ? (a.pro_relu & 1) : (a.pro_relu & 2);
        const float* pro = first ? a.pro0 : a.pro1;
#pragma unroll
        for (int j = 0; j < 8; ++j) {
          const int cgi = min(cb + j, cn - 1);
          const float sc = pro ? pro[2 * cgi] : 1.f, sh = pro ? pro[2 * cgi + 1] : 0.f;
          float w = fmaf(v[j], sc, sh);
          if (relu) w = fmaxf(w, 0.f);
          v[j] = in ? w : 0.f;
        }
      }
      if (pos < PE) {
        u32x4v t0, t1, t2;
#pragma unroll
        for (int j = 0; j < 4; ++j) {
          unsigned q0, q1, q2;
          WSPLIT(v[2 * j], v[2 * j + 1], q0, q1, q2);
          t0[j] = q0; t1[j] = q1; t2[j] = q2;
        }
        WSTORE(Xs[(0 * NCG + cg) * XP + pos], t0);
        WSTORE(Xs[(1 * NCG + cg) * XP + pos], t1);
        WSTORE(Xs[(2 * NCG + cg) * XP + pos], t2);
      }
    };
#pragma unroll
    for (int i = 0; i < NITX; i += 2) {
      float v0[8], v1[8];
      int cg0, pos0, cb0, cn0, cg1 = 0, pos1 = PE, cb1 = 0, cn1 = 1;
      bool in0, f0, in1 = false, f1 = true;
      x_item(i, v0, cg0, pos0, in0, f0, cb0, cn0);
      if (i + 1 < NITX) x_item(i + 1, v1, cg1, pos1, in1, f1, cb1, cn1);
      x_finish(v0, cg0, pos0, in0, f0, cb0, cn0);
      if (i + 1 < NITX) x_finish(v1, cg1, pos1, in1, f1, cb1, cn1);
      __builtin_amdgcn_sched_barrier(0);
    }
#pragma unroll
    for (int i = 0; i < NITY; ++i) {
      const int blk = __builtin_amdgcn_readfirstlane(i * 4 + wave);
      const int cg = blk / PBY;
      const int px = (blk - cg * PBY) * 64 + lane;
      const int gy = ty * TH + (px >> TWL), gx = tx * TW + (px & (TW - 1));
      const unsigned vo = (gy < a.H && gx < a.W) ? (unsigned)(gy * a.W + gx) * 4u : BUF_OOB;
      const int c = cout0 + cg * 8;
      float v[8];
#pragma unroll
      for (int j = 0; j < 8; ++j) v[j] = buf_load(rsy, vo, (unsigned)min(c + j, a.Cout) * (unsigned)HW * 4u);
      u32x4v t0, t1, t2;
#pragma unroll
      for (int j = 0; j < 4; ++j) {
        unsigned q0, q1, q2;
        WSPLIT(v[2 * j], v[2 * j + 1], q0, q1, q2);
        t0[j] = q0; t1[j] = q1; t2[j] = q2;
      }
      WSTORE(Ys[(0 * NCG + cg) * YP + px], t0);
      WSTORE(Ys[(1 * NCG + cg) * YP + px], t1);
      WSTORE(Ys[(2 * NCG + cg) * YP + px], t2);
    }
    __builtin_amdgcn_sched_barrier(0);
    __syncthreads();
    constexpr int NSTEP = Q ? NPX / 16 : NPX / 64;
    auto step_p0 = [&](int s) { return (Q ? s : wave * NSTEP + s) * 16; };
    auto load_a = [&](int s, bf16x8 (&af)[3]) {
      const int p0 = step_p0(s);
#pragma unroll
      for (int t = 0; t < 3; ++t) af[t] = lds_tr8(Ys, a_base + (t * NCG * YP + p0) * 16);
    };
    auto load_b = [&](int s, int tap, bf16x8 (&bfr)[3]) {
      const int p0 = step_p0(s);
      const int toff = ((p0 >> TWL) + tap / KS) * PITCH + (p0 & (TW - 1)) + tap % KS;
#pragma unroll
      for (int t = 0; t < 3; ++t) bfr[t] = lds_tr8(Xs, b_base + (t * NCG * XP + toff) * 16);
    };
    bf16x8 af[2][3], bfr[2][3];
    load_a(0, af[0]);
    load_b(0, 0, bfr[0]);
#pragma unroll
    for (int idx = 0; idx < NSTEP * TAPS; ++idx) {
      const int s = idx / TAPS, tap = idx % TAPS;
      const int cur = idx & 1, acur = s & 1;
      if (idx + 1 < NSTEP * TAPS) {
        load_b((idx + 1) / TAPS, (idx + 1) % TAPS, bfr[cur ^ 1]);
        if (tap == TAPS - 1) load_a(s + 1, af[acur ^ 1]);
      }
      __builtin_amdgcn_sched_barrier(0);
      f32x16 c = acc[tap];
      c = mfma_bf16(af[acur][0], bfr[cur][2], c);
      c = mfma_bf16(af[acur][1], bfr[cur][1], c);
      c = mfma_bf16(af[acur][2], bfr[cur][0], c);
      c = mfma_bf16(af[acur][0], bfr[cur][1], c);
      c = mfma_bf16(af[acur][1], bfr[cur][0], c);
      c = mfma_bf16(af[acur][0], bfr[cur][0], c);
      acc[tap] = c;
      __builtin_amdgcn_sched_barrier(0);
    }
  }

  float* slab = a.slab + (size_t)ky * a.Cout * a.Cin * TAPS;
  if constexpr (Q) {
    const int ci = cin0 + wci * 32 + (lane & 31);
#pragma unroll
    for (int r = 0; r < 16; ++r) {
      const int co = cout0 + wco * 32 + (r & 3) + 8 * (r >> 2) + 4 * (lane >> 5);
      if (co < a.Cout && ci < a.Cin) {
        float* dst = slab + ((size_t)co * a.Cin + ci) * TAPS;
#pragma unroll
        for (int t = 0; t < TAPS; ++t) dst[t] = acc[t][r];
      }
    }
  } else {
    float* red = reinterpret_cast<float*>(smem);
#pragma unroll
    for (int t = 0; t < TAPS; ++t) {
      __syncthreads();
#pragma unroll
      for (int r = 0; r < 16; ++r) {
        const int co = (r & 3) + 8 * (r >> 2) + 4 * (lane >> 5);
        red[(wave * 32 + co) * 32 + (lane & 31)] = acc[t][r];
      }
      __syncthreads();
      for (int e = tid; e < 1024; e += 256) {
        const int co = e >> 5, ci = e & 31;
        const float v = red[e] + red[1024 + e] + red[2048 + e] + red[3072 + e];
        if (cout0 + co < a.Cout && cin0 + ci < a.Cin) slab[((size_t)(cout0 + co) * a.Cin + cin0 + ci) * TAPS + t] = v;
      }
    }
// ... 71 lines not shown
```

wt-pse-code_amd/wtpse_hip/csrc/internal.h:

```cpp
#pragma once
#include <cstdlib>
#include "common.h"

#define WTPSE_INTERNAL __attribute__((visibility("hidden")))

WTPSE_INTERNAL extern int g_x3_terms;

struct BnbArgs {
  const float* ss = nullptr;
  const float* mean = nullptr;
  int relu = 0, c0 = 0, c1 = 0;
};
struct ConvCall {
  const float* in0 = nullptr; int C0 = 0;
  const float* in1 = nullptr; int C1 = 0;
  const void* w = nullptr;
  const float* bias = nullptr;
  const float* pro0 = nullptr; const float* pro1 = nullptr; int pro_relu = 0;
  float* out0 = nullptr; float* out1 = nullptr; int Csplit = 0;
  float* stats = nullptr;
  const float* mask_ref = nullptr;
  float* gram = nullptr;
  const unsigned* in_amax0 = nullptr; const unsigned* in_amax1 = nullptr;
  int in_is_grad = 0;
  unsigned* out_amax = nullptr;
  BnbArgs bn;
  BnbTail tail = bnb_tail_none();
  BnfTail ftail = bnf_tail_none();
  int B = 0, H = 0, W = 0, Cout = 0, ksize = 0, relu_out = 0;
};
enum { CONV_FP32 = 0, CONV_X3 = 1, CONV_C16 = 2 };
WTPSE_INTERNAL int conv_run(const ConvCall& c, int layout, hipStream_t st);
WTPSE_INTERNAL int conv_launch_x3(const ConvCall& c, hipStream_t st);

struct Tiling {
  int TW, TH, tiles_x, tiles_y, tiles;
};
static inline Tiling make_tiling(int B, int H, int W, bool narrow, int pixels) {
  Tiling t;
  t.TW = narrow ? 16 : 32; t.TH = pixels / t.TW;
  t.tiles_x = ceil_div(W, t.TW); t.tiles_y = ceil_div(H, t.TH); t.tiles = B * t.tiles_x * t.tiles_y;
  return t;
}
static inline Tiling conv_tiling(int B, int H, int W, int pixels = 256) { return make_tiling(B, H, W, W <= 16, pixels); }
struct X3Tiling {
  int mt;
  int px;
  int half;
  int small;
  Tiling t;
};
WTPSE_INTERNAL X3Tiling x3_tiling(int B, int H, int W, int Cout, int ksize);

WTPSE_INTERNAL void wgrad_reduce_launch(const float* slab, int ksplit, int n, float* dw, int accumulate, void* stream);
WTPSE_INTERNAL void wgrad_reduce_launch2(const float* slab, int ksplit, int n, float* dw, int accumulate, const float* slab_b,
                                         int n_b, float* db, void* stream);

static inline bool tail_in_launch(long long workgroups) {
  static const long long max_wgs = [] { const char* e = getenv("WTPSE_TAIL_MAX_WGS"); return e ? atoll(e) : 8192ll; }();
  return workgroups <= max_wgs;
}
template <class Args>
static inline int tail_after_launch(const Args& a, int nblk, hipStream_t stream) {
  const BnbTail& tl = a.tail;
  const BnfTail& fl = a.ftail;
  const long long count = (long long)a.B * a.H * a.W;
  if (tl.tickets && tl.dbias)
    return wtpse_bn_bwd_finalize_coef_frozen(a.stats, nblk, a.bn_c1 - a.bn_c0, tl.gamma, tl.invstd, tl.coef, tl.dgamma, tl.dbeta,
                                             tl.dbias, tl.accumulate, stream);
  if (tl.tickets)
    return wtpse_bn_bwd_finalize_coef(a.stats, nblk, a.bn_c1 - a.bn_c0, count, tl.gamma, a.bn_mean, tl.invstd, tl.coef, tl.dgamma,
                                      tl.dbeta, tl.accumulate, stream);
  if (fl.tickets)
    return wtpse_bn_finalize(a.stats, nblk, a.Cout, count, fl.gamma, fl.beta, fl.rmean, fl.rvar, fl.nbt, fl.momentum, fl.eps,
                             fl.scale_shift, fl.save_mean, fl.save_invstd, fl.act_amax, stream);
  return 0;
}
```

wt-pse-code_amd/wtpse_hip/nn.py:

```python
import math
import os

import torch
import torch.nn as nn

from . import ops


class ConvP(nn.Module):

    def __init__(self, cin, cout, k):
        super().__init__()
        self.cin, self.cout, self.k = cin, cout, k
        self.weight = nn.Parameter(torch.empty(cout, cin, k, k))
        self.bias = nn.Parameter(torch.empty(cout))
        nn.init.kaiming_uniform_(self.weight, a=math.sqrt(5))
        bound = 1.0 / math.sqrt(cin * k * k)
        nn.init.uniform_(self.bias, -bound, bound)
        self.wf_off = self.wd_off = -1
        self.xf_off = self.xd_off = -1
        self.x16f_off = self.x16d_off = -1


class BNP(nn.Module):

    def __init__(self, c):
        super().__init__()
        self.c = c
        self.weight = nn.Parameter(torch.ones(c))
        self.bias = nn.Parameter(torch.zeros(c))
        self.register_buffer("running_mean", torch.zeros(c))
        self.register_buffer("running_var", torch.ones(c))
        self.register_buffer("num_batches_tracked", torch.tensor(0, dtype=torch.long))


class Seq(nn.Module):

    def __init__(self, **children):
        super().__init__()
        for name, mod in children.items():
            self.add_module(name.lstrip("_"), mod)

    def __getitem__(self, i):
        return getattr(self, str(i))


class ConvDBlock(nn.Module):
    def __init__(self, cin, c, first=False):
        super().__init__()
        self.first = first
        self.conv1, self.bn1 = ConvP(cin, c, 3), BNP(c)
        self.conv2, self.bn2 = ConvP(c, c, 3), BNP(c)
        self.conv3, self.bn3 = ConvP(c, c, 3), BNP(c)


class ConvUBlock(nn.Module):
    def __init__(self, planes, first=False):
        super().__init__()
        self.first = first
        if not first:
            self.conv1, self.bn1 = ConvP(2 * planes, planes, 3), BNP(planes)
        self.conv2, self.bn2 = ConvP(planes, planes // 2, 1), BNP(planes // 2)
        self.conv3, self.bn3 = ConvP(planes, planes, 3), BNP(planes)


class DoubleConvWTP(nn.Module):
    def __init__(self, cin, cout):
        super().__init__()
        self.double_conv = Seq(_0=ConvP(cin, cout, 3), _2=ConvP(cout, cout, 3))


class DeepWTP(nn.Module):

    def __init__(self, cin=3, c=16):
        super().__init__()
        self.DoubleConv = DoubleConvWTP(cin, c)
        self.DoubleConv2 = DoubleConvWTP(c, c)

    def forward(self, x):
        self._root.ensure_ready(repack=True)
        with ops.fwd_scope(x.device):
            t = deepwt_fwd(self, x.detach().to(torch.float32).contiguous(), want_tape=False)
            return [t.z1, t.z2, Act(t.z2, None, True).dense()]


class DoubleConvP(nn.Module):
    def __init__(self, cin, cout):
        super().__init__()
        self.double_conv = Seq(_0=ConvP(cin, cout, 3), _1=BNP(cout), _3=ConvP(cout, cout, 3), _4=BNP(cout))


def head_p(n=16, n_classes=1):
    return Seq(_0=ConvP(2 * n, 2 * n, 1), _2=ConvP(2 * n, 8, 1), _4=ConvP(8, n_classes, 1))


class UNetBody(nn.Module):

    def _make_body(self, n=16):
        self.down1 = ConvDBlock(n, 2 * n)
        self.down2 = ConvDBlock(2 * n, 4 * n)
        self.down3 = ConvDBlock(4 * n, 8 * n)
        self.down4 = ConvDBlock(8 * n, 16 * n)
        self.up1 = ConvUBlock(16 * n, first=True)
        self.up2 = ConvUBlock(8 * n)
        self.up3 = ConvUBlock(4 * n)
        self.up4 = ConvUBlock(2 * n)


class AttentionP(nn.Module):
    def __init__(self):
        super().__init__()
        self.layer1 = ConvP(1, 1, 1)

    def forward(self, x):
        root = self.layer1._root
        root.ensure_ready(repack=True)
        dummy = x.new_zeros((x.shape[0], 1, x.shape[2], x.shape[3]))
        att, pre, _, _ = ops.attn_fuse_fwd(x.contiguous(), self.layer1.weight.data_ptr(), dummy, 0.0, True, True, False)
        return att, pre


class TeacherP(UNetBody):

    def __init__(self, n=16):
        super().__init__()
        self.inc = DoubleConvP(1, n)
        self.fusion = Seq(_0=ConvP(2 * n, n, 1))
        self._make_body(n)
        self.mu_prior = head_p(n)
        self.logvar_prior = head_p(n)

    def sample_forward(self, inputs, mask=None, training=True):
        root = self.fusion[0]._root
        root.ensure_ready(repack=True)
        with ops.fwd_scope(inputs.device):
            t = teacher_fwd(self, inputs.contiguous(), mask.contiguous(), self.training, want_logvar=training,
                            want_tape=False)
        if not training:
            return t.mu
        eps = root.next_noise(t.mu.shape)
        return ops.reparam_fwd(t.mu, t.logvar, eps), t.mu


def _invalidate_on_load(module, incompatible_keys):
    root = module.__dict__.get("_root")
    if root is not None:
        root.invalidate_packed()


class HipNet(nn.Module):

    def _finish_init(self):
        for name, value in dict(_flat=None, _gflat=None, _gwork=None, _packed=None, _x3=None, _xdesc=None, _x16desc=None, _desc=None,
                                _packed_version=-1, _touched=[], _noise_queue=[], _noise_seed=0x5eed, _noise_ctr=None, _dp=None,
                                _flag=None, _packed_valid=False, _attach_grads=True, _defer_allreduce=False, _join=[],
                                _frozen_bias={}, _frozen_pass=False, bn_momentum=0.1).items():
            object.__setattr__(self, name, value)
        self._convs = [m for m in self.modules() if isinstance(m, ConvP)]
        for m in self.modules():
            if isinstance(m, (ConvP, BNP, AttentionP, TeacherP, DeepWTP)):
                object.__setattr__(m, "_root", self)
        for m in self.modules():
            if isinstance(m, (ConvP, BNP)):
                m.register_load_state_dict_post_hook(_invalidate_on_load)
        off = 0
        self._x3_convs = []
        for c in self._convs:
            fwd = x3_eligible(c.cin, c.cout, c.k) and os.environ.get("WTPSE_X3_FWD", "1") != "0"
            bwd = x3_eligible(c.cout, c.cin, c.k) and os.environ.get("WTPSE_X3_DGRAD", "1") != "0"
            if fwd:
                c.xf_off = off
                off += ops.x3_packed_size(c.cout, c.cin, c.k * c.k)
            if bwd:
                c.xd_off = off
                off += ops.x3_packed_size(c.cin, c.cout, c.k * c.k)
            if fwd or bwd:
                self._x3_convs.append(c)
        self._x16_convs = []
        for c in self._convs:
            c.x16f_off = c.x16d_off = -1
            if X16 and c.k == 3 and c.cin <= 16 and c.cout <= 16:
                if c.cin >= X16_MIN_K:
                    c.x16f_off = off
                    off += ops.X16_SIZE
                if c.cout >= X16_MIN_K:
                    c.x16d_off = off
                    off += ops.X16_SIZE
                if c.x16f_off >= 0 or c.x16d_off >= 0:
                    self._x16_convs.append(c)
        self._x3_size = off
        off = 0
        for c in self._convs:
            t = c.k * c.k
            c.wf_off = c.wd_off = -1
            if c.xf_off < 0:
                c.wf_off = off
                off += ((c.cin + 3) & ~3) * t * ((c.cout + 15) & ~15)
            if c.xd_off < 0:
                c.wd_off = off
                off += ((c.cout + 3) & ~3) * t * ((c.cin + 15) & ~15)
        self._packed_size = max(off, 4)

    def _is_flat(self):
        f = self._flat
        if f is None:
            return False
        p0, pl = self._plist[0], self._plist[-1]
        return (p0.device == f.device and p0.data_ptr() == f.data_ptr()
                and pl.data_ptr() == f.data_ptr() + 4 * self._offsets[-1])

    def _flatten(self):
        params = list(self.parameters())
        dev = params[0].device
        if dev.type != "cuda":
            raise RuntimeError("the WT-PSE MI355X path runs in device memory only: move the module to a HIP device "
                               "(`.to('cuda')`); there is no CPU fallback")
        total = sum(p.numel() for p in params)
        flat = torch.empty(total, dtype=torch.float32, device=dev)
        offsets, off = [], 0
        with torch.no_grad():
            for p in params:
                n = p.numel()
                flat[off:off + n].copy_(p.detach().reshape(-1).to(dev, torch.float32))
                p.data = flat[off:off + n].view(p.shape)
                p.grad = None
                offsets.append(off)
                off += n
        object.__setattr__(self, "_flat", flat)
        object.__setattr__(self, "_offsets", offsets)
        object.__setattr__(self, "_pindex", {id(p): i for i, p in enumerate(params)})
        object.__setattr__(self, "_plist", params)
        object.__setattr__(self, "_gflat", torch.zeros(total, dtype=torch.float32, device=dev))
        object.__setattr__(self, "_gwork", None)
        object.__setattr__(self, "_packed", torch.empty(self._packed_size, dtype=torch.float32, device=dev))

        def table(convs, fwd, bwd):
            desc = [v for c in convs for v in (self.param_offset(c.weight), c.cout, c.cin, c.k * c.k, getattr(c, fwd), getattr(c, bwd), 0, 0)]
            return torch.tensor(desc, dtype=torch.int32).to(dev) if desc else None

        object.__setattr__(self, "_desc", table(self._convs, "wf_off", "wd_off"))
        object.__setattr__(self, "_packed_version", -1)
        object.__setattr__(self, "_x3", torch.empty(max(self._x3_size, 8), dtype=torch.int16, device=dev))
        object.__setattr__(self, "_xdesc", table(self._x3_convs, "xf_off", "xd_off"))
        object.__setattr__(self, "_x16desc", table(self._x16_convs, "x16f_off", "x16d_off"))
        object.__setattr__(self, "_flag", torch.zeros(1, dtype=torch.int32, device=dev))
        ops._tickets(0, dev)
        ops.amax_begin(dev)
        object.__setattr__(self, "_noise_ctr", torch.zeros(1, dtype=torch.int64, device=dev))
        for b in self.buffers():
            if b.device != dev:
                raise RuntimeError("parameters and buffers live on different devices")

    def ensure_ready(self, repack=False):
        if not self._is_flat():
            self._flatten()
        terms = ops.x3_terms()
        if self._packed_version < 0 or (repack and not self._packed_valid) or self._packed_version != terms:
            ops.lib().call("wtpse_pack_conv_weights", self._flat.data_ptr(), self._desc.data_ptr(), len(self._convs),
                           self._packed.data_ptr(), ops.stream_ptr())
            if self._xdesc is not None:
                ops.lib().call("wtpse_pack_conv_weights_x3", self._flat.data_ptr(), self._xdesc.data_ptr(), len(self._x3_convs),
                               self._x3.data_ptr(), ops.stream_ptr())
            if self._x16desc is not None:
                ops.lib().call("wtpse_pack_conv16_x3", self._flat.data_ptr(), self._x16desc.data_ptr(), len(self._x16_convs),
                               self._x3.data_ptr(), ops.stream_ptr())
            object.__setattr__(self, "_packed_version", terms)

    def invalidate_packed(self):
        object.__setattr__(self, "_packed_version", -1)

    def packed_ptr(self, off):
        return self._packed.data_ptr() + 4 * off

    def x3_ptr(self, off):
        return self._x3.data_ptr() + 2 * off

    def flat_params(self):
        self.ensure_ready()
        return self._flat

    def flat_grads(self):
        self.ensure_ready()
        return self._gflat

    def param_offset(self, p):
        return self._offsets[self._pindex[id(p)]]

    def grange(self, first_param, n):
        off = self.param_offset(first_param)
        return self._gtarget[off:off + n]

    @property
    def bn_synced(self):
        return self._dp is not None and self._dp.bn_sync

    def begin_backward(self):
        self._touched.clear()
        ops.amax_begin(self._flat.device)
        clean = all(p.grad is None for p in self._plist)
        if clean:
            object.__setattr__(self, "_gtarget", self._gflat)
        else:
            if self._gwork is None:
                object.__setattr__(self, "_gwork", torch.zeros_like(self._gflat))
            object.__setattr__(self, "_gtarget", self._gwork)

    def gview(self, p):
        self._touched.append(p)
        return self.grange(p, p.numel())

    def gbias(self, conv):
        object.__setattr__(self, "_frozen_pass", True)
        if self._gtarget is self._gflat:
            self._frozen_bias[id(conv.bias)] = conv.bias
        return self.gview(conv.bias)

    def grads_ready(self, first, last=None):
        dp = self._dp
        if dp is None or not dp.overlap or self._gtarget is not self._gflat or ops.lib()._rec is not None:
            return
        if self._gflat.is_cuda and torch.cuda.is_current_stream_capturing():
            return
        last = first if last is None else last
        pf, pl = next(first.parameters()), list(last.parameters())[-1]
        lo, hi = self.param_offset(pf), self.param_offset(pl) + pl.numel()
        cur = torch.cuda.current_stream()
        streams = [cur]
        side = _SIDE.get((self._gflat.device, ops.stream_ptr()))
        if side is not None:
            streams.append(side)
        dp.bucket_ready(self, self._gtarget, lo, hi, streams)

    def end_backward(self):
        joins = self._join
        if joins:
            cur = torch.cuda.current_stream()
            for st in joins:
                stream_wait(cur, st)
            joins.clear()
        if self._dp is not None and not self._defer_allreduce:
            self._dp.allreduce_grads(self, self._gtarget)
        direct = self._gtarget is self._gflat
        if direct and self._frozen_bias and not self._frozen_pass:
            for p in self._frozen_bias.values():
                ops.zero_(self.grange(p, p.numel()))
            self._frozen_bias.clear()
        object.__setattr__(self, "_frozen_pass", False)
        if direct and not self._attach_grads:
            self._touched.clear()
            return
        for p in self._touched:
            g = self.grange(p, p.numel()).view(p.shape)
            if direct:
                p.grad = g
            elif p.grad is None:
                p.grad = g.clone()
            else:
                ops.axpy(p.grad, g.contiguous(), 1.0) if p.grad.is_contiguous() else p.grad.add_(g)
        self._touched.clear()

    def set_noise(self, tensors):
        object.__setattr__(self, "_noise_queue", list(tensors))

    def seed_noise(self, seed):
        self.ensure_ready()
        object.__setattr__(self, "_noise_seed", int(seed))
        ops.zero_(self._noise_ctr)

    def next_noise(self, shape):
        if self._noise_queue:
            e = self._noise_queue.pop(0)
            assert tuple(e.shape) == tuple(shape), (e.shape, shape)
            return e.to(self._flat.device, torch.float32).contiguous()
        ctr = self._noise_ctr
        if self._dp is not None:
            eps, used = self._dp.noise(tuple(int(v) for v in shape), self._noise_seed, ctr)
        else:
            n = 1
            for s in shape:
                n *= int(s)
            eps, used = ops.randn(shape, self._flat.device, self._noise_seed, 0, ctr), (n + 3) & ~3
        ops.counter_add(ctr, used)
        return eps


class Tape:
    frozen = False


class Act:
    __slots__ = ("t", "pro", "relu", "amax")

    def __init__(self, t, pro=None, relu=False, amax=None):
        self.t, self.pro, self.relu = t, pro, bool(relu)
        self.amax = amax if amax is not None else (getattr(t, "wt_amax", None) if pro is None else None)

    def dense(self):
        if self.pro is None and not self.relu:
            return self.t
        z = ops.affine_act(self.t, self.pro, self.relu)
        if self.amax is not None:
            z.wt_amax = self.amax
        return z


    @staticmethod
    def parts(a):
        return (a.t, a.pro) if a is not None else (None, None)


def as_act(x):
    return x if isinstance(x, Act) else Act(x)


FWD_AMAX = os.environ.get("WTPSE_FWD_AMAX", "1") != "0"


def act_amax(a):
    if a is None or ops.x3_terms() != 2 or not FWD_AMAX:
        return None
    if a.amax is None:
        raw = ops.amax_of(a.t)
        a.amax = raw if a.pro is None else ops.act_bound(a.pro, raw)
    return a.amax


def _relu_bits(a0, a1):
    return (1 if a0.relu else 0) | (2 if (a1 is not None and a1.relu) else 0)


X3 = os.environ.get("WTPSE_X3", "1") != "0"
X3_WGRAD = os.environ.get("WTPSE_X3_WGRAD", "1") != "0"
WGRAD_R = os.environ.get("WTPSE_WGRAD_R", "1") != "0"
X16 = os.environ.get("WTPSE_X16", "1") != "0" and X3
X16_MIN_K = int(os.environ.get("WTPSE_X16_MIN_K", "8"))


def x3_eligible(k_dim, rows, ksize):
    return X3 and rows > 16 and 16 <= k_dim <= 256 and (ksize == 3 or k_dim >= 64)


def _weights(layer, dgrad=False, wide=False):
    root = layer._root
    x16, x3, w = (layer.x16d_off, layer.xd_off, layer.wd_off) if dgrad else (layer.x16f_off, layer.xf_off, layer.wf_off)
    if x16 >= 0 and not wide:
        return 2, root.x3_ptr(x16)
    if x3 >= 0:
        return 1, root.x3_ptr(x3)
    return 0, root.packed_ptr(w)


def _conv(layer, a0, a1=None, relu_out=False, want_stats=False, want_amax=False):
    a0 = as_act(a0)
    a1 = as_act(a1) if a1 is not None else None
    t1, pro1 = Act.parts(a1)
    out_amax = ops.fwd_amax_table(a0.t.device) if want_amax else None
    layout, wptr = _weights(layer, wide=a1 is not None)
    if layout == 2:
        y, stats, _ = ops.conv16_x3(a0.t, wptr, layer.bias, layer.cout, a0.pro, _relu_bits(a0, None), relu_out, want_stats,
                                    in_amax=act_amax(a0), out_amax=out_amax)
    elif layout == 1:
        y, _, stats = ops.conv_fwd_x3(a0.t, t1, wptr, layer.bias, layer.cout, layer.k, a0.pro, _relu_bits(a0, a1), relu_out, want_stats,
                                      None, None, pro1, act_amax(a0), act_amax(a1), out_amax)
    else:
        y, _, stats = ops.conv_fwd(a0.t, t1, wptr, layer.bias, layer.cout, layer.k, a0.pro, _relu_bits(a0, a1), relu_out, want_stats,
                                   None, None, pro1, out_amax)
    return y, stats


class PreBN:
    __slots__ = ("g", "stats", "coef")

    def __init__(self, g, stats, coef=None):
        self.g, self.stats, self.coef = g, stats, coef


BN_FUSED_STATS = os.environ.get("WTPSE_BN_FUSED_STATS", "1") != "0"
BN_TAIL = os.environ.get("WTPSE_BN_TAIL", "1") != "0"


def _gamax(dy):
    return ops.amax_of(dy) if ops.x3_terms() == 2 else None


def _dgrad(layer, dy, split=None, mask_ref=None, below0=None, below1=None):
    root = layer._root
    below = below0 if below0 is not None else below1
    layout, wptr = _weights(layer, dgrad=True, wide=split is not None)
    if (BN_FUSED_STATS and below is not None and mask_ref is None and below.mean is not None
            and not root.bn_synced and (below1 is None or split is not None)):
        bn = below.bn
        tail = (bn.weight, below.invstd, root.gview(bn.weight), root.gview(bn.bias)) if BN_TAIL else None
        if tail is not None and below.frozen:
            tail += (root.gbias(below.conv),)
        d0, d1, stats, coef = ops.dgrad_bnb(dy, wptr, layout, layer.cin, layer.k, below.y, below.ss, below.mean, below.relu, split,
                                            below1 is not None and below0 is None, tail,
                                            _gamax(dy) if layout == 1 else getattr(dy, "wt_amax", None) if layout == 2 else None)
        if below0 is not None:
            return PreBN(d0, stats, coef), d1
        return d0, PreBN(d1, stats, coef)
    if layout == 2:
        return ops.conv16_x3(dy, wptr, None, layer.cin, mask_ref=mask_ref, grad_in=True)[0], None
    if layout == 1:
        return ops.conv_fwd_x3(dy, None, wptr, None, layer.cin, layer.k, None, 0, False, False, split, mask_ref, None, _gamax(dy))[:2]
    return ops.conv_fwd(dy, None, wptr, None, layer.cin, layer.k, None, 0, False, False, split, mask_ref)[:2]


_SIDE = {}
WGRAD_SIDE_STREAM = os.environ.get("WTPSE_WGRAD_STREAM", "1") != "0"


def _side_stream(device, owner=None):
    key = (device, ops.stream_ptr() if owner is None else owner)
    st = _SIDE.get(key)
    if st is None:
        st = _SIDE[key] = torch.cuda.Stream(device=device)
    return st


_SECOND = {}
TEACHER_SIDE_STREAM = os.environ.get("WTPSE_TEACHER_STREAM", "1") != "0"


def second_stream(device):
    if not TEACHER_SIDE_STREAM:
        return None
    key = (device, ops.stream_ptr())
    st = _SECOND.get(key)
    if st is None:
        st = _SECOND[key] = torch.cuda.Stream(device=device)
    return st


def stream_wait(waiter, waited):
    waiter.wait_stream(waited)
    ops.lib().plan_wait(waiter.cuda_stream, waited.cuda_stream)


def note_join(root, stream):
    if all(s is not stream for s in root._join):
        root._join.append(stream)


def _wgrad_side(layer, dy, a0, a1=None):
    root = layer._root
    if not WGRAD_SIDE_STREAM:
        return _wgrad(layer, dy, a0, a1, with_bias=False)
    a0 = as_act(a0)
    a1 = as_act(a1) if a1 is not None else None
    amax = _gamax(dy)
    kernel, tables = _wgrad_kernel(layer, dy, a0, a1, False)
    main = torch.cuda.current_stream()
    side = _side_stream(dy.device)
    stream_wait(side, main)
    with torch.cuda.stream(side):
        _wgrad_launch(kernel, tables, layer, dy, a0, a1, False)
    for t in (dy, amax, a0.t, a0.pro) + tables[1:] + Act.parts(a1):
        if t is not None:
            t.record_stream(side)
    note_join(root, side)


def _wgrad_kernel(layer, dy, a0, a1, with_bias):
    c0, small = a0.t.shape[1], layer.cin % 32 != 0 and layer.cout % 32 != 0
    if (X3 and X3_WGRAD and WGRAD_R and layer.k == 3 and
            ops.wgrad_r_supported(layer.cin, layer.cout, 3, c0 if a1 is not None else 16, a0.t.shape[3]) and (not with_bias or small)):
        return "r", (getattr(dy, "wt_amax", None) if small else _gamax(dy), act_amax(a0), act_amax(a1))
    if X3 and X3_WGRAD and not with_bias and ops.wgrad_x3_supported(layer.cin, layer.cout, layer.k, c0 if a1 is not None else 8):
        return "x3", (None, None, None)
    return "fp32", (None, None, None)


def _wgrad_launch(kernel, tables, layer, dy, a0, a1, with_bias):
    root = layer._root
    t1, pro1 = Act.parts(a1)
    dw = root.gview(layer.weight)
    db = root.gview(layer.bias) if with_bias else None
    if kernel == "r":
        ops.conv_wgrad_r(dy, a0.t, t1, dw, db, a0.pro, _relu_bits(a0, a1), False, pro1, *tables)
    elif kernel == "x3":
        ops.conv_wgrad_x3(dy, a0.t, t1, layer.k, dw, a0.pro, _relu_bits(a0, a1), False, pro1)
    else:
        ops.conv_wgrad(dy, a0.t, t1, layer.k, dw, db, a0.pro, _relu_bits(a0, a1), False, pro1)


def _wgrad(layer, dy, a0, a1=None, with_bias=True):
    a0 = as_act(a0)
    a1 = as_act(a1) if a1 is not None else None
    kernel, tables = _wgrad_kernel(layer, dy, a0, a1, with_bias)
    _wgrad_launch(kernel, tables, layer, dy, a0, a1, with_bias)


def _bn_coeffs(root, bn, y, stats, training, tab=None, raw_amax=None, want_tape=False):
    if not training:
        if want_tape:
            ss, mean, invstd = ops.bn_eval_coeffs_stats(bn.weight, bn.bias, bn.running_mean, bn.running_var)
        else:
            ss, mean, invstd = ops.bn_eval_coeffs(bn.weight, bn.bias, bn.running_mean, bn.running_var), None, None
        return ss, mean, invstd, (ops.act_bound(ss, raw_amax) if raw_amax is not None else None)
    B, _, H, W = y.shape
    count = B * H * W
    if root.bn_synced:
        stats, count = root._dp.sync_bn_stats(stats, count)
    if tab is None:
        tab = ops.fwd_amax_table(y.device)
    return ops.bn_finalize(stats, count, bn.weight, bn.bias, bn.running_mean, bn.running_var, bn.num_batches_tracked,
                           momentum=root.bn_momentum, act_amax=tab) + (tab,)


def convbn_fwd(conv, bn, a0, a1, relu, training, want_tape=True):
    root = conv._root
    a0 = as_act(a0)
    a1 = as_act(a1) if a1 is not None else None
    tab = ops.fwd_amax_table(a0.t.device) if training else None
    if training and BN_TAIL and not root.bn_synced:
        layout, wptr = _weights(conv, wide=a1 is not None)
        t1, pro1 = Act.parts(a1)
        y, ss, mean, invstd = ops.conv_fwd_bnf(a0.t, t1, wptr, layout, conv.bias, conv.cout, conv.k, a0.pro, _relu_bits(a0, a1), pro1,
                                               bn.weight, bn.bias, bn.running_mean, bn.running_var, bn.num_batches_tracked,
                                               momentum=root.bn_momentum, in_amax0=act_amax(a0) if layout else None,
                                               in_amax1=act_amax(a1) if layout == 1 else None, act_amax=tab)
    else:
        y, stats = _conv(conv, a0, a1, False, training, want_amax=not training)
        ss, mean, invstd, tab = _bn_coeffs(root, bn, y, stats, training, tab, getattr(y, "wt_amax", None), want_tape)
    z = Act(y, ss, relu, tab)
    if not want_tape:
        return z, None
    t = Tape()
    t.a0, t.a1, t.y, t.ss, t.mean, t.invstd, t.relu = a0, a1, y, ss, mean, invstd, relu
    t.bn, t.conv, t.frozen = bn, conv, not training
    return z, t


BN_IN = os.environ.get("WTPSE_BN_IN", "1") != "0"
def _bn_bwd(bn, t, dz, root):
    if t.frozen:
        if root.bn_synced:
            raise RuntimeError("frozen BatchNorm statistics are not supported together with synchronised BatchNorm")
        if isinstance(dz, PreBN):
            if dz.coef is not None:
                return ops.bn_bwd_scale_coef(dz.g, dz.coef)
            return ops.bn_bwd_from_stats_frozen(dz.g, dz.stats, bn.weight, t.invstd, root.gview(bn.weight), root.gview(bn.bias),
                                                root.gbias(t.conv))
        return ops.bn_bwd_frozen(dz, t.y, t.ss, t.relu, bn.weight, t.mean, t.invstd, root.gview(bn.weight), root.gview(bn.bias),
                                 root.gbias(t.conv))
    if isinstance(dz, PreBN):
        if dz.coef is not None:
            return ops.bn_bwd_apply_coef(dz.g, t.y, dz.coef)
        return ops.bn_bwd_from_stats(dz.g, t.y, dz.stats, bn.weight, t.mean, t.invstd, root.gview(bn.weight), root.gview(bn.bias))
    if root.bn_synced:
        return root._dp.bn_bwd_synced(dz, t, bn, root)
    return ops.bn_bwd(dz, t.y, t.ss, t.relu, bn.weight, t.mean, t.invstd, root.gview(bn.weight), root.gview(bn.bias))


def convbn_bwd(conv, bn, t, dz, need_dx=True, below0=None, below1=None):
    root = conv._root
    dy = _bn_bwd(bn, t, dz, root)
    _wgrad_side(conv, dy, t.a0, t.a1)
    if not need_dx:
        return None, None
    split = t.a0.t.shape[1] if t.a1 is not None else None
    return _dgrad(conv, dy, split, below0=below0, below1=below1)


def convd_fwd(blk, x, training, want_tape=True):
    t = Tape()
    x = as_act(x)
    t.x = x
    h = x if blk.first else Act(ops.maxpool2_fwd(x.t, x.pro, x.relu), amax=x.amax)
    a, t.c1 = convbn_fwd(blk.conv1, blk.bn1, h, None, False, training, want_tape)
    b, t.c2 = convbn_fwd(blk.conv2, blk.bn2, a, None, True, training, want_tape)
    c, t.c3 = convbn_fwd(blk.conv3, blk.bn3, b, None, True, training, want_tape)
    return c, t


def convd_bwd(blk, t, dz, dx_accum=None, need_dx=True, mask_x=False, below=None):
    d, _ = convbn_bwd(blk.conv3, blk.bn3, t.c3, dz, below0=t.c2)
    d, _ = convbn_bwd(blk.conv2, blk.bn2, t.c2, d, below0=t.c1)
    d, _ = convbn_bwd(blk.conv1, blk.bn1, t.c1, d, need_dx=need_dx)
    if not need_dx:
        return None
    if blk.first:
        if dx_accum is not None:
            ops.axpy(dx_accum, d)
            d = dx_accum
        return ops.relu_mask(d, t.x.t) if mask_x else d
    root = blk.conv1._root
    if (BN_FUSED_STATS and below is not None and below.mean is not None and t.x.relu and t.x.pro is not None
            and not root.bn_synced):
        r = ops.maxpool2_bwd_bnb(t.x.t, d, dx_accum, t.x.pro, t.x.relu, below.mean)
        if r is not None:
            return PreBN(r[0], r[1])
    return ops.maxpool2_bwd(t.x.t, d, dx_accum, dx_accum is not None, t.x.pro, t.x.relu, mask=mask_x)


CONVU_CONV_FIRST = os.environ.get("WTPSE_CONVU_REFERENCE_ORDER", "0") != "1"


def upbn_fwd(conv, bn, a0, training, want_tape=True):
    root = conv._root
    z, _ = _conv(conv, a0, None, False, False, want_amax=not training)
    y, stats = ops.upsample2x_fwd_stats(z) if training else (ops.upsample2x_fwd(z), None)
    ss, mean, invstd, tab = _bn_coeffs(root, bn, y, stats, training, None, getattr(z, "wt_amax", None), want_tape)
    out = Act(y, ss, True, tab)
    if not want_tape:
        return out, None
    t = Tape()
    t.a0, t.a1, t.y, t.ss, t.mean, t.invstd, t.relu = a0, None, y, ss, mean, invstd, True
    t.bn, t.conv, t.frozen = bn, conv, not training
    return out, t


def upbn_bwd(conv, bn, t, dz, below=None):
    root = conv._root
    if BN_IN and isinstance(dz, PreBN) and dz.coef is not None and dz.g.shape[3] % 8 == 0:
        dzl = ops.upsample2x_bwd_bn(dz.g, t.y, dz.coef)
    else:
        dzl = ops.upsample2x_bwd(_bn_bwd(bn, t, dz, root))
    _wgrad_side(conv, dzl, t.a0, None)
    return _dgrad(conv, dzl, below0=below)[0]


def convu_fwd(blk, x, prev, training, want_tape=True):
    t = Tape()
    x = as_act(x)
    if not blk.first:
        x, t.c1 = convbn_fwd(blk.conv1, blk.bn1, x, None, True, training, want_tape)
    B, _, H, W = x.t.shape
    t.swapped = CONVU_CONV_FIRST and W % 2 == 0 and B * blk.conv2.cout < 32768
    if t.swapped:
        y, t.c2 = upbn_fwd(blk.conv2, blk.bn2, x, training, want_tape)
    else:
        u = Act(ops.upsample2x_fwd(x.t, x.pro, x.relu), amax=x.amax)
        y, t.c2 = convbn_fwd(blk.conv2, blk.bn2, u, None, True, training, want_tape)
    out, t.c3 = convbn_fwd(blk.conv3, blk.bn3, prev, y, True, training, want_tape)
    return out, t


def convu_bwd(blk, t, dout, below_x=None):
    dprev, dy = convbn_bwd(blk.conv3, blk.bn3, t.c3, dout, below1=t.c2)
    if t.swapped:
        dx = upbn_bwd(blk.conv2, blk.bn2, t.c2, dy, below=(below_x if blk.first else t.c1))
    else:
        du, _ = convbn_bwd(blk.conv2, blk.bn2, t.c2, dy)
        dx = ops.upsample2x_bwd(du)
    if not blk.first:
        dx, _ = convbn_bwd(blk.conv1, blk.bn1, t.c1, dx, below0=below_x)
    return dx, dprev


def unet_fwd(net, x1, training, want_tape=True):
    t = Tape()
    x1 = as_act(x1)
    x2, t.d1 = convd_fwd(net.down1, x1, training, want_tape)
    x3, t.d2 = convd_fwd(net.down2, x2, training, want_tape)
    x4, t.d3 = convd_fwd(net.down3, x3, training, want_tape)
    x5, t.d4 = convd_fwd(net.down4, x4, training, want_tape)
    x, t.u1 = convu_fwd(net.up1, x5, x4, training, want_tape)
    x, t.u2 = convu_fwd(net.up2, x, x3, training, want_tape)
    x, t.u3 = convu_fwd(net.up3, x, x2, training, want_tape)
    x, t.u4 = convu_fwd(net.up4, x, x1, training, want_tape)
    return x, t


def unet_bwd(net, t, dfeat, need_dx1=True, decoder_done=None, mask_x=None, below_x1=None):
    d, g1 = convu_bwd(net.up4, t.u4, dfeat, below_x=t.u3.c3)
    d, g2 = convu_bwd(net.up3, t.u3, d, below_x=t.u2.c3)
    d, g3 = convu_bwd(net.up2, t.u2, d, below_x=t.u1.c3)
    g5, g4 = convu_bwd(net.up1, t.u1, d, below_x=t.d4.c3)
    if decoder_done is not None:
        decoder_done()
    g4 = convd_bwd(net.down4, t.d4, g5, g4, below=t.d3.c3)
    g3 = convd_bwd(net.down3, t.d3, g4, g3, below=t.d2.c3)
    g2 = convd_bwd(net.down2, t.d2, g3, g2, below=t.d1.c3)
    g1 = convd_bwd(net.down1, t.d1, g2, g1, mask_x=mask_x is not None, below=below_x1)
    return g1 if need_dx1 else None


def _head_fusable(seq, idxs, x):
    ls = [seq[i] for i in idxs]
    if len(ls) not in (2, 3) or (ls[0].cin, ls[0].cout, ls[1].cin, ls[1].cout) != (32, 32, 32, 8):
        return None
    if len(ls) == 3 and not (ls[2].cin == 8 and 1 <= ls[2].cout <= 4):
        return None
    if any(l.k != 1 for l in ls) or (x.t.shape[2] * x.t.shape[3]) % 32 != 0:
        return None
    root = ls[0]._root
    off = root.param_offset(ls[0].weight)
    for l in ls:
        for prm in (l.weight, l.bias):
            if root.param_offset(prm) != off:
                return None
            off += prm.numel()
    return ls


def head_fwd(seq, x, idxs, want_tape=True):
    t = Tape()
    t.x, t.acts = as_act(x), []
    ls = _head_fusable(seq, idxs, t.x)
    t.fused = ls is not None
    if t.fused:
        w3, b3 = (ls[2].weight, ls[2].bias) if len(ls) == 3 else (None, None)
        out, t.h1, t.h2 = ops.head_fwd(t.x.t, t.x.pro, t.x.relu, ls[0].weight, ls[0].bias, ls[1].weight, ls[1].bias, w3, b3,
                                       want_tape, x_amax=act_amax(t.x))
# ... 100 lines not shown
```

wt-pse-code_amd/wtpse_hip/ops.py:

```python
import torch

from .lib import lib

_WS = {}


_RAW_STREAM = getattr(torch._C, "_cuda_getCurrentRawStream", None)


def stream_ptr():
    if _RAW_STREAM is not None:
        return _RAW_STREAM(torch.cuda.current_device())
    return torch.cuda.current_stream().cuda_stream


def ptr(t):
    return 0 if t is None else t.data_ptr()


def _chk(t, name="tensor"):
    if t is None:
        return
    if not (t.is_cuda and t.dtype == torch.float32 and t.is_contiguous()):
        raise ValueError("%s must be a contiguous fp32 tensor in device memory (got %s, %s, contiguous=%s)"
                         % (name, t.device, t.dtype, t.is_contiguous()))


def workspace(tag, nfloats, device):
    key = (str(device), stream_ptr(), tag)
    buf = _WS.get(key)
    if buf is None or buf.numel() < nfloats:
        buf = torch.empty(max(int(nfloats), 1024), dtype=torch.float32, device=device)
        _WS[key] = buf
    return buf


def _out_pair(split, B, cout, H, W, device):
    if split is None:
        return torch.empty((B, cout, H, W), dtype=torch.float32, device=device), None, cout
    csplit = int(split)
    return (torch.empty((B, csplit, H, W), dtype=torch.float32, device=device),
            torch.empty((B, cout - csplit, H, W), dtype=torch.float32, device=device), csplit)


def _stats_blocks(layout, B, H, W, cout=0, ksize=0):
    if layout == 1:
        return lib().query("wtpse_conv_x3_stats_blocks", B, H, W, cout, int(ksize))
    return lib().query("wtpse_conv_stats_blocks", B, H, W)


def _conv_launch(name, layout, in_amax, in0, in1, wpacked_ptr, bias, cout, ksize, pro0, pro_relu, relu_out, want_stats, split, mask_ref,
                 pro1, out_amax):
    _chk(in0, "in0"); _chk(in1, "in1"); _chk(pro0, "pro0"); _chk(pro1, "pro1")
    B, C0, H, W = in0.shape
    C1 = 0 if in1 is None else in1.shape[1]
    out0, out1, csplit = _out_pair(split, B, cout, H, W, in0.device)
    stats = None
    if want_stats:
        stats = torch.empty((_stats_blocks(layout, B, H, W, cout, ksize), cout, 2), dtype=torch.float32, device=in0.device)
    lib().call(name, ptr(in0), C0, ptr(in1), C1, wpacked_ptr, ptr(bias), ptr(pro0), ptr(pro1), int(pro_relu), ptr(out0),
               ptr(out1), csplit, ptr(stats), B, H, W, cout, ksize, int(relu_out), ptr(mask_ref), *in_amax, ptr(out_amax), stream_ptr())
    if out_amax is not None:
        out0.wt_amax = out_amax
    return out0, out1, stats


def conv_fwd(in0, in1, wpacked_ptr, bias, cout, ksize, pro0=None, pro_relu=0, relu_out=False, want_stats=False,
             split=None, mask_ref=None, pro1=None, out_amax=None):
    return _conv_launch("wtpse_conv_fwd", 0, (), in0, in1, wpacked_ptr, bias, cout, ksize, pro0, pro_relu, relu_out, want_stats, split,
                        mask_ref, pro1, out_amax)


def conv_fwd_gram(in0, wpacked_ptr, bias, pro0=None, pro_relu=0, relu_out=False, out_amax=None):
    _chk(in0, "in0"); _chk(pro0, "pro0")
    B, C0, H, W = in0.shape
    L = lib()
    out = torch.empty((B, 16, H, W), dtype=torch.float32, device=in0.device)
    nblk = _stats_blocks(0, B, H, W)
    partial = torch.empty((nblk, 256), dtype=torch.float32, device=in0.device)
    L.call("wtpse_conv_fwd_gram", ptr(in0), C0, wpacked_ptr, ptr(bias), ptr(pro0), int(pro_relu), ptr(out), ptr(partial), B, H, W,
           16, int(relu_out), ptr(out_amax), stream_ptr())
    if out_amax is not None:
        out.wt_amax = out_amax
    return out, (partial, nblk // B)


X16_SIZE = 8 + 5 * 3 * 64 * 8 + 5 * 2 * 64 * 8


def conv16_x3(in0, wx16_ptr, bias, cout, pro0=None, pro_relu=0, relu_out=False, want_stats=False, want_gram=False, mask_ref=None,
              bnb=None, grad_in=False, in_amax=None, out_amax=None):
    _chk(in0, "in0"); _chk(pro0, "pro0"); _chk(mask_ref, "mask_ref")
    B, C0, H, W = in0.shape
    L = lib()
    out = torch.empty((B, cout, H, W), dtype=torch.float32, device=in0.device)
    nblk = _stats_blocks(2, B, H, W)
    stats = torch.empty((nblk, cout, 2), dtype=torch.float32, device=in0.device) if (want_stats or bnb is not None) else None
    gram = torch.empty((nblk, 256), dtype=torch.float32, device=in0.device) if want_gram else None
    bn_ss = bn_mean = None
    bn_relu = 0
    if bnb is not None:
        mask_ref, bn_ss, bn_mean, bn_relu = bnb
        _chk(mask_ref, "bn_y"); _chk(bn_ss, "bn_ss"); _chk(bn_mean, "bn_mean")
        assert mask_ref.shape == out.shape
    L.call("wtpse_conv16_x3", ptr(in0), C0, wx16_ptr, ptr(bias), ptr(pro0), int(pro_relu), ptr(out), ptr(stats), ptr(gram),
           ptr(mask_ref), ptr(bn_ss), ptr(bn_mean), int(bool(bn_relu)), B, H, W, cout, int(relu_out), int(bool(grad_in)),
           ptr(getattr(in0, "wt_amax", None)) if grad_in else ptr(in_amax), ptr(out_amax), stream_ptr())
    if out_amax is not None:
        out.wt_amax = out_amax
    return out, stats, ((gram, nblk // B) if want_gram else None)


def x3_packed_size(rows, k, taps):
    return 32 + ((k + 15) & ~15) * ((rows + 31) & ~31) * taps * 3


def x3_terms():
    return lib().query("wtpse_x3_terms", -1)


AMAX_WORDS = 1024
_AMAX = {}
_AMAX_TABLES = 512


class _Arena:
    __slots__ = ("buf", "next", "retired")

    def __init__(self, buf):
        self.buf, self.next, self.retired = buf, 0, []

    def take(self, n):
        off = self.next
        if self.buf is None or off + n > self.buf.numel():
            return None
        self.next = off + n
        return self.buf[off:off + n]

    def renew(self, buf):
        self.retired.append(self.buf)
        del self.retired[:-3]
        self.buf, self.next = buf, 0

    def __getitem__(self, i):
        return (self.buf, self.next)[i]


def amax_begin(device):
    buf = zero_(torch.empty(_AMAX_TABLES * AMAX_WORDS, dtype=torch.int32, device=device))
    st = _AMAX.get(device)
    if st is None:
        _AMAX[device] = _Arena(buf)
    else:
        st.renew(buf)


def _amax_table(device):
    if x3_terms() != 2:
        return None
    st = _AMAX.get(device)
    t = st.take(AMAX_WORDS) if st is not None else None
    return t if t is not None else zero_(torch.empty(AMAX_WORDS, dtype=torch.int32, device=device))


_FWD_SCOPES = []
FWD_SCOPE_TABLES = 256


class fwd_scope(_Arena):
    __slots__ = ()

    def __init__(self, device):
        super().__init__(zero_(torch.empty(FWD_SCOPE_TABLES * AMAX_WORDS, dtype=torch.int32, device=device)) if x3_terms() == 2 else None)

    def __enter__(self):
        _FWD_SCOPES.append(self)
        return self

    def __exit__(self, *exc):
        assert _FWD_SCOPES and _FWD_SCOPES[-1] is self
        _FWD_SCOPES.pop()
        return False


def fwd_amax_table(device):
    if x3_terms() != 2:
        return None
    sc = _FWD_SCOPES[-1] if _FWD_SCOPES else None
    t = sc.take(AMAX_WORDS) if sc is not None and sc.buf is not None and sc.buf.device == device else None
    return t if t is not None else zero_(torch.empty(AMAX_WORDS, dtype=torch.int32, device=device))


def act_bound(ss, raw_amax):
    tab = torch.empty(AMAX_WORDS, dtype=torch.int32, device=ss.device)
    lib().call("wtpse_act_bound", ptr(ss), ss.shape[0], ptr(raw_amax), ptr(tab), stream_ptr())
    return tab


def amax_of(t):
    tab = getattr(t, "wt_amax", None)
    if tab is None:
        tab = torch.empty(AMAX_WORDS, dtype=torch.int32, device=t.device)
        lib().call("wtpse_amax", ptr(t), t.numel(), ptr(tab), stream_ptr())
        t.wt_amax = tab
    return tab


def conv_fwd_x3(in0, in1, wpacked_ptr, bias, cout, ksize, pro0=None, pro_relu=0, relu_out=False, want_stats=False,
                split=None, mask_ref=None, pro1=None, in_amax=None, in_amax1=None, out_amax=None):
    return _conv_launch("wtpse_conv_fwd_x3", 1, (ptr(in_amax), ptr(in_amax1)), in0, in1, wpacked_ptr, bias, cout, ksize, pro0, pro_relu,
                        relu_out, want_stats, split, mask_ref, pro1, out_amax)


_TICKETS = {}
_TICKET_RING = 1 << 22
_TICKET_SCOPE = None
_DEBUG = __import__("os").environ.get("WTPSE_DEBUG", "0") == "1"


class ticket_scope(_Arena):
    __slots__ = ()

    def __init__(self, device, n=1 << 21):
        super().__init__(torch.zeros(n, dtype=torch.int32, device=device))
        torch.cuda.current_stream(device).synchronize()

    def __enter__(self):
        global _TICKET_SCOPE
        assert _TICKET_SCOPE is None, "ticket scopes do not nest"
        self.next = 0
        _TICKET_SCOPE = self
        return self

    def __exit__(self, *exc):
        global _TICKET_SCOPE
        _TICKET_SCOPE = None
        return False


def _tickets(n, device):
    n = (n + 63) & ~63
    st = _TICKET_SCOPE
    if st is not None:
        view = st.take(n)
        if view is None:
            raise RuntimeError("ticket_scope exhausted (%d unsigneds): a recorded step uses more ticket words than reserved" % st.buf.numel())
        return st.buf.data_ptr() + 4 * view.storage_offset(), view
    st = _TICKETS.get(device)
    if st is None:
        if torch.cuda.is_current_stream_capturing():
            raise RuntimeError("the ticket ring must exist before a step is captured: HipNet.ensure_ready() creates it")
        st = _TICKETS[device] = _Arena(torch.zeros(_TICKET_RING, dtype=torch.int32, device=device))
        torch.cuda.current_stream(device).synchronize()
    view = st.take(n)
    if view is None:
        st.next = 0
        view = st.take(n)
    if _DEBUG and n and not torch.cuda.is_current_stream_capturing():
        torch.cuda.synchronize(device)
        off = view.storage_offset()
        assert not bool(view.any()), "ticket slice [%d, %d) is not zero on entry: a launch that used it failed or is still running" % (off, off + n)
    return st.buf.data_ptr() + 4 * view.storage_offset(), view


def _ticket_call(view, name, *args):
    try:
        lib().call(name, *args)
    except Exception:
        if view.numel() and not torch.cuda.is_current_stream_capturing():
            torch.cuda.synchronize(view.device)
            zero_(view)
        raise


def dgrad_bnb(dy, wpacked_ptr, layout, cout, ksize, bn_y, bn_ss, bn_mean, bn_relu, split=None, bn_second=False, tail=None,
              in_amax=None):
    _chk(dy, "dy"); _chk(bn_y, "bn_y"); _chk(bn_ss, "bn_ss"); _chk(bn_mean, "bn_mean")
    layout = int(layout)
    B, C, H, W = dy.shape
    L = lib()
    out0, out1, csplit = _out_pair(split, B, cout, H, W, dy.device)
    c0, c1 = (csplit, cout) if (bn_second and split is not None) else (0, csplit)
    assert bn_y.shape == (B, c1 - c0, H, W), (bn_y.shape, (B, c1 - c0, H, W))
    nblk = _stats_blocks(layout, B, H, W, cout, ksize)
    stats = torch.empty((nblk, c1 - c0, 2), dtype=torch.float32, device=dy.device)
    if tail is not None:
        gamma, invstd, dgamma, dbeta = tail[:4]
        coef = torch.empty((c1 - c0, 3), dtype=torch.float32, device=dy.device)
        partial2 = torch.empty(L.query("wtpse_bnb_tail_partial2", nblk, cout), dtype=torch.float64, device=dy.device)
        tickets, tview = _tickets(L.query("wtpse_bnb_tail_tickets", nblk, cout), dy.device)
        frozen = len(tail) == 5
        args = [ptr(dy), C, wpacked_ptr, layout, ptr(out0), ptr(out1), csplit, ptr(bn_y), ptr(bn_ss), ptr(bn_mean), int(bool(bn_relu)),
                c0, c1, ptr(stats), ptr(gamma), ptr(invstd), ptr(coef), ptr(dgamma), ptr(dbeta)] + ([ptr(tail[4])] if frozen else [])
        _ticket_call(tview, "wtpse_dgrad_bnb_coef_frozen" if frozen else "wtpse_dgrad_bnb_coef", *args, 0, ptr(partial2), tickets,
                     B, H, W, cout, ksize, ptr(in_amax), stream_ptr())
        return out0, out1, stats, coef
    if layout == 2:
        L.call("wtpse_conv16_x3", ptr(dy), C, wpacked_ptr, 0, 0, 0, ptr(out0), ptr(stats), 0, ptr(bn_y), ptr(bn_ss), ptr(bn_mean),
               int(bool(bn_relu)), B, H, W, cout, 0, 1, ptr(in_amax), 0, stream_ptr())
    elif layout == 1:
        L.call("wtpse_dgrad_x3_bnb", ptr(dy), C, wpacked_ptr, ptr(out0), ptr(out1), csplit, ptr(bn_y), ptr(bn_ss), ptr(bn_mean),
               int(bool(bn_relu)), c0, c1, ptr(stats), B, H, W, cout, ksize, ptr(in_amax), stream_ptr())
    else:
        L.call("wtpse_dgrad_bnb", ptr(dy), C, wpacked_ptr, ptr(out0), ptr(out1), csplit,
               ptr(bn_y), ptr(bn_ss), ptr(bn_mean), int(bool(bn_relu)), c0, c1, ptr(stats), B, H, W, cout, ksize, stream_ptr())
    return out0, out1, stats, None


def _wgrad_dims(dy, x0, x1):
    _chk(dy, "dy"); _chk(x0, "x0"); _chk(x1, "x1")
    B, cout, H, W = dy.shape
    C0 = x0.shape[1]
    C1 = 0 if x1 is None else x1.shape[1]
    return lib(), B, cout, H, W, C0, C1, C0 + C1


def conv_wgrad(dy, x0, x1, ksize, dw, dbias, pro0=None, pro_relu=0, accumulate=False, pro1=None):
    L, B, cout, H, W, C0, C1, cin = _wgrad_dims(dy, x0, x1)
    ks = L.query("wtpse_wgrad_ksplit", B, H, W, cin, cout)
    slab = workspace("wgrad_slab", ks * cout * cin * ksize * ksize, dy.device)
    dbs = workspace("wgrad_dbias", ks * cout, dy.device) if dbias is not None else None
    L.call("wtpse_conv_wgrad", ptr(dy), ptr(x0), C0, ptr(x1), C1, ptr(pro0), ptr(pro1), int(pro_relu), ptr(slab), ptr(dbs), ks,
           ptr(dw), ptr(dbias), int(accumulate), B, H, W, cout, ksize, stream_ptr())


def wgrad_x3_supported(cin, cout, ksize, c0):
    return bool(lib().query("wtpse_wgrad_x3_supported", int(cin), int(cout), int(ksize), int(c0)))


def conv_wgrad_x3(dy, x0, x1, ksize, dw, pro0=None, pro_relu=0, accumulate=False, pro1=None):
    L, B, cout, H, W, C0, C1, cin = _wgrad_dims(dy, x0, x1)
    ks = L.query("wtpse_wgrad_x3_ksplit", B, H, W, cin, cout)
    slab = workspace("wgrad_slab", ks * cout * cin * ksize * ksize, dy.device)
    L.call("wtpse_conv_wgrad_x3", ptr(dy), ptr(x0), C0, ptr(x1), C1, ptr(pro0), ptr(pro1), int(pro_relu), ptr(slab), ks, ptr(dw),
           int(accumulate), B, H, W, cout, ksize, stream_ptr())


def wgrad_r_supported(cin, cout, ksize, c0, w):
    return bool(lib().query("wtpse_wgrad_r_supported", int(cin), int(cout), int(ksize), int(c0), int(w)))


def conv_wgrad_r(dy, x0, x1, dw, dbias=None, pro0=None, pro_relu=0, accumulate=False, pro1=None, dy_amax=None, x_amax0=None,
                 x_amax1=None):
    L, B, cout, H, W, C0, C1, cin = _wgrad_dims(dy, x0, x1)
    ns = L.query("wtpse_wgrad_r_slabs", B, H, W, cin, cout)
    slab = workspace("wgrad_slab", ns * cout * cin * 9, dy.device)
    dbs = workspace("wgrad_dbias", ns * cout, dy.device) if dbias is not None else None
    L.call("wtpse_conv_wgrad_r", ptr(dy), ptr(x0), C0, ptr(x1), C1, ptr(pro0), ptr(pro1), int(pro_relu), ptr(slab), ptr(dbs), ns,
           ptr(dw), ptr(dbias), int(accumulate), B, H, W, cout, ptr(dy_amax), ptr(x_amax0), ptr(x_amax1), stream_ptr())


def conv_wgrad_r_bn(g, bn_y, coef, x0, x1, dw, pro0=None, pro_relu=0, accumulate=False, pro1=None):
    _chk(bn_y, "bn_y")
    L, B, cout, H, W, C0, C1, cin = _wgrad_dims(g, x0, x1)
    ns = L.query("wtpse_wgrad_r_slabs", B, H, W, cin, cout)
    slab = workspace("wgrad_slab", ns * cout * cin * 9, g.device)
    L.call("wtpse_conv_wgrad_r_bn", ptr(g), ptr(bn_y), ptr(coef), ptr(x0), C0, ptr(x1), C1, ptr(pro0), ptr(pro1), int(pro_relu),
           ptr(slab), ns, ptr(dw), int(accumulate), B, H, W, cout, stream_ptr())


def conv_fwd_bnf(in0, in1, wpacked_ptr, layout, bias, cout, ksize, pro0, pro_relu, pro1, gamma, beta, rmean, rvar, nbt,
                 momentum=0.1, eps=1e-5, in_amax0=None, in_amax1=None, act_amax=None):
    _chk(in0, "in0"); _chk(in1, "in1"); _chk(pro0, "pro0"); _chk(pro1, "pro1")
    layout = int(layout)
    B, C0, H, W = in0.shape
    C1 = 0 if in1 is None else in1.shape[1]
    L = lib()
    dev = in0.device
    out = torch.empty((B, cout, H, W), dtype=torch.float32, device=dev)
    nblk = _stats_blocks(layout, B, H, W, cout, ksize)
    stats = torch.empty((nblk, cout, 2), dtype=torch.float32, device=dev)
    ss = torch.empty((cout, 2), dtype=torch.float32, device=dev)
    mean = torch.empty((cout,), dtype=torch.float32, device=dev)
    invstd = torch.empty((cout,), dtype=torch.float32, device=dev)
    partial2 = torch.empty(L.query("wtpse_bnb_tail_partial2", nblk, cout), dtype=torch.float64, device=dev)
    tickets, tview = _tickets(L.query("wtpse_bnb_tail_tickets", nblk, cout), dev)
    _ticket_call(tview, "wtpse_conv_fwd_bnf", ptr(in0), C0, ptr(in1), C1, wpacked_ptr, layout, ptr(bias), ptr(pro0), ptr(pro1), int(pro_relu),
           ptr(out), ptr(stats), ptr(gamma), ptr(beta), ptr(rmean), ptr(rvar), ptr(nbt), float(momentum), float(eps), ptr(ss),
           ptr(mean), ptr(invstd), ptr(partial2), tickets, B, H, W, cout, ksize, ptr(in_amax0), ptr(in_amax1), ptr(act_amax),
           stream_ptr())
    return out, ss, mean, invstd


def bn_finalize(stats, count, gamma, beta, rmean, rvar, nbt, momentum=0.1, eps=1e-5, act_amax=None):
    nblk, C, _ = stats.shape
    dev = stats.device
    ss = torch.empty((C, 2), dtype=torch.float32, device=dev)
    mean = torch.empty((C,), dtype=torch.float32, device=dev)
    invstd = torch.empty((C,), dtype=torch.float32, device=dev)
    lib().call("wtpse_bn_finalize", ptr(stats), nblk, C, int(count), ptr(gamma), ptr(beta), ptr(rmean), ptr(rvar),
               ptr(nbt), float(momentum), float(eps), ptr(ss), ptr(mean), ptr(invstd), ptr(act_amax), stream_ptr())
    return ss, mean, invstd


def bn_eval_coeffs(gamma, beta, rmean, rvar, eps=1e-5):
    C = gamma.numel()
    ss = torch.empty((C, 2), dtype=torch.float32, device=gamma.device)
    lib().call("wtpse_bn_eval_coeffs", ptr(gamma), ptr(beta), ptr(rmean), ptr(rvar), float(eps), C, ptr(ss), stream_ptr())
    return ss


def bn_eval_coeffs_stats(gamma, beta, rmean, rvar, eps=1e-5):
    C = gamma.numel()
    ss = torch.empty((C, 2), dtype=torch.float32, device=gamma.device)
    mean = torch.empty((C,), dtype=torch.float32, device=gamma.device)
    invstd = torch.empty((C,), dtype=torch.float32, device=gamma.device)
    lib().call("wtpse_bn_eval_coeffs_stats", ptr(gamma), ptr(beta), ptr(rmean), ptr(rvar), float(eps), C, ptr(ss), ptr(mean),
               ptr(invstd), stream_ptr())
    return ss, mean, invstd


def affine_act(y, ss, relu):
    _chk(y, "y")
    B, C, H, W = y.shape
    z = torch.empty_like(y)
    lib().call("wtpse_affine_act", ptr(y), ptr(ss), int(relu), ptr(z), B, C, H * W, stream_ptr())
    return z


def bn_bwd(dz, y, ss, relu, gamma, mean, invstd, dgamma, dbeta, accumulate=False):
    _chk(dz, "dz"); _chk(y, "y")
    B, C, H, W = y.shape
    L = lib()
    ns = L.query("wtpse_bn_bwd_nsplit", B, C, H * W)
    partial = workspace("bn_bwd_partial", ns * C * 2, y.device)
    coef = workspace("bn_bwd_coef", C * 3, y.device)
    dy = torch.empty_like(y)
    dy.wt_amax = _amax_table(y.device)
    L.call("wtpse_bn_bwd", ptr(dz), ptr(y), ptr(ss), int(relu), ptr(gamma), ptr(mean), ptr(invstd), ptr(partial),
           ptr(coef), ptr(dgamma), ptr(dbeta), int(accumulate), ptr(dy), B, C, H * W, ptr(dy.wt_amax), stream_ptr())
    return dy


def bn_bwd_from_stats(g, y, stats, gamma, mean, invstd, dgamma, dbeta, accumulate=False):
    _chk(g, "g"); _chk(y, "y"); _chk(stats, "stats")
    B, C, H, W = y.shape
    assert stats.shape[1] == C
    coef = workspace("bn_bwd_coef", C * 3, y.device)
    dy = torch.empty_like(y)
    dy.wt_amax = _amax_table(y.device)
    lib().call("wtpse_bn_bwd_from_stats", ptr(g), ptr(y), ptr(stats), stats.shape[0], ptr(gamma), ptr(mean), ptr(invstd), ptr(coef),
               ptr(dgamma), ptr(dbeta), int(accumulate), ptr(dy), B, C, H * W, ptr(dy.wt_amax), stream_ptr())
    return dy


def bn_bwd_frozen(dz, y, ss, relu, gamma, mean, invstd, dgamma, dbeta, dbias, accumulate=False):
    _chk(dz, "dz"); _chk(y, "y")
    B, C, H, W = y.shape
    L = lib()
    ns = L.query("wtpse_bn_bwd_nsplit", B, C, H * W)
    partial = workspace("bn_bwd_partial", ns * C * 2, y.device)
    coef = workspace("bn_bwd_coef", C * 3, y.device)
    dy = torch.empty_like(y)
    dy.wt_amax = _amax_table(y.device)
    L.call("wtpse_bn_bwd_frozen", ptr(dz), ptr(y), ptr(ss), int(relu), ptr(gamma), ptr(mean), ptr(invstd), ptr(partial), ptr(coef),
           ptr(dgamma), ptr(dbeta), ptr(dbias), int(accumulate), ptr(dy), B, C, H * W, ptr(dy.wt_amax), stream_ptr())
    return dy


def bn_bwd_from_stats_frozen(g, stats, gamma, invstd, dgamma, dbeta, dbias, accumulate=False):
    _chk(g, "g"); _chk(stats, "stats")
    B, C, H, W = g.shape
    assert stats.shape[1] == C
    coef = workspace("bn_bwd_coef", C * 3, g.device)
    dy = torch.empty_like(g)
    dy.wt_amax = _amax_table(g.device)
    lib().call("wtpse_bn_bwd_from_stats_frozen", ptr(g), ptr(stats), stats.shape[0], ptr(gamma), ptr(invstd), ptr(coef), ptr(dgamma),
               ptr(dbeta), ptr(dbias), int(accumulate), ptr(dy), B, C, H * W, ptr(dy.wt_amax), stream_ptr())
    return dy


def bn_bwd_finalize_coef_frozen(stats, gamma, invstd, dgamma, dbeta, dbias, accumulate=False):
    _chk(stats, "stats")
    C = stats.shape[1]
    coef = torch.empty((C, 3), dtype=torch.float32, device=stats.device)
    lib().call("wtpse_bn_bwd_finalize_coef_frozen", ptr(stats), stats.shape[0], C, ptr(gamma), ptr(invstd), ptr(coef), ptr(dgamma),
               ptr(dbeta), ptr(dbias), int(accumulate), stream_ptr())
    return coef


def bn_bwd_scale_coef(g, coef):
    _chk(g, "g"); _chk(coef, "coef")
    B, C, H, W = g.shape
    dy = torch.empty_like(g)
    dy.wt_amax = _amax_table(g.device)
    lib().call("wtpse_bn_bwd_scale_coef", ptr(g), ptr(coef), ptr(dy), B, C, H * W, ptr(dy.wt_amax), stream_ptr())
    return dy


def bn_frozen_fold_spec(g, y, gamma, running_mean, running_var, eps=1e-5):
    r = 1.0 / torch.sqrt(running_var + eps)
    s = gamma * r
    sum_g = g.sum(dim=(0, 2, 3))
    sum_gy = (g * (y - running_mean.view(1, -1, 1, 1))).sum(dim=(0, 2, 3))
    return s.view(1, -1, 1, 1) * g, r * sum_gy, sum_g, s * sum_g, running_mean, r


class WtLossState:
    __slots__ = ("z", "gram", "offdiag", "diag", "dmmd_dv", "losses", "v", "B", "HW", "D", "n", "margin")


def bn_bwd_apply_coef(g, y, coef):
    _chk(g, "g"); _chk(y, "y")
    B, C, H, W = y.shape
    dy = torch.empty_like(y)
    dy.wt_amax = _amax_table(y.device)
    lib().call("wtpse_bn_bwd_apply_coef", ptr(g), ptr(y), ptr(coef), ptr(dy), B, C, H * W, ptr(dy.wt_amax), stream_ptr())
    return dy


def wt_loss_fwd(z, domain_num, per_domain, margin=0.0, eps=1e-5, losses_out=None, gram_partial=None):
    _chk(z, "z")
    B, C, H, W = z.shape
    HW = H * W
    dev = z.device
    L = lib()
    S = L.query("wtpse_wt_split", B, HW, 0)
    R = domain_num * per_domain
    st = WtLossState()
    partial = workspace("wt_partial", B * S * 256, dev) if gram_partial is None else None
    st.gram = torch.empty((B, 256), dtype=torch.float32, device=dev)
    st.v = torch.empty((B, 120), dtype=torch.float32, device=dev)
    st.offdiag = torch.empty((B,), dtype=torch.float32, device=dev)
    st.diag = torch.empty((B,), dtype=torch.float32, device=dev)
    rowval = torch.empty((max(R, 1) + 1,), dtype=torch.float64, device=dev)
    st.dmmd_dv = torch.empty((max(R, 1), 120), dtype=torch.float32, device=dev)
    st.losses = losses_out if losses_out is not None else torch.empty((3,), dtype=torch.float32, device=dev)
    if gram_partial is not None:
        gp, gs = gram_partial
        assert C == 16 and gp.shape[0] == B * gs
        L.call("wtpse_wt_loss_fwd_partials", ptr(gp), int(gs), B, HW, float(eps), float(margin), int(domain_num), int(per_domain),
               ptr(st.gram), ptr(st.v), ptr(st.offdiag), ptr(st.diag), ptr(rowval), ptr(st.dmmd_dv), ptr(st.losses), stream_ptr())
    else:
        L.call("wtpse_wt_loss_fwd", ptr(z), B, C, HW, float(eps), float(margin), int(domain_num), int(per_domain),
               ptr(partial), ptr(st.gram), ptr(st.v), ptr(st.offdiag), ptr(st.diag), ptr(rowval), ptr(st.dmmd_dv),
               ptr(st.losses), stream_ptr())
    st.z, st.B, st.HW, st.D, st.n, st.margin = z, B, HW, domain_num, per_domain, float(margin)
    return st


def wt_loss_bwd(st, dz, accumulate, g_off=None, g_diag=None, g_dom=None, w_off=1.0, w_diag=1.0, w_dom=1.0):
    _chk(dz, "dz")
    _amax_stale(dz)
    Mws = workspace("wt_M", st.B * 256, dz.device)
    lib().call("wtpse_wt_loss_bwd", ptr(st.z), st.B, 16, st.HW, st.margin, st.D, st.n, ptr(st.gram), ptr(st.offdiag),
               ptr(st.diag), ptr(st.dmmd_dv), ptr(g_off), ptr(g_diag), ptr(g_dom), float(w_off), float(w_diag),
               float(w_dom), ptr(Mws), ptr(dz), int(accumulate), stream_ptr())


def wt_combine(losses, den, mode, out=None):
    if out is None:
        out = torch.empty((4,), dtype=torch.float32, device=losses.device)
    lib().call("wtpse_wt_combine", ptr(losses), losses.shape[0], float(den), int(mode), ptr(out), stream_ptr())
    return out


def maxpool2_fwd(x, pro=None, relu=False):
    _chk(x, "x")
    B, C, H, W = x.shape
    out = torch.empty((B, C, H // 2, W // 2), dtype=torch.float32, device=x.device)
    lib().call("wtpse_maxpool2_fwd", ptr(x), ptr(pro), int(relu), ptr(out), B, C, H, W, stream_ptr())
    return out


def maxpool2_bwd(x, dout, dx, accumulate, pro=None, relu=False, mask=False):
    B, C, H, W = x.shape
    if dx is None:
        dx = torch.empty_like(x)
        accumulate = False
    _amax_stale(dx)
    lib().call("wtpse_maxpool2_bwd", ptr(x), ptr(pro), int(relu), ptr(dout), ptr(dx), int(bool(accumulate)) | (2 if mask else 0),
               B, C, H, W, stream_ptr())
    return dx


def maxpool2_bwd_bnb(x, dout, dx, pro, relu, mean):
    B, C, H, W = x.shape
    if W % 4 or H % 2 or B * C >= 32768 or pro is None:
        return None
    L = lib()
    acc = dx is not None
    if dx is None:
        dx = torch.empty_like(x)
    _amax_stale(dx)
    stats = torch.empty((L.query("wtpse_maxpool2_bwd_stats_blocks", B, H, W), C, 2), dtype=torch.float32, device=x.device)
    L.call("wtpse_maxpool2_bwd_bnb", ptr(x), ptr(pro), int(relu), ptr(dout), ptr(dx), int(acc), ptr(mean), ptr(stats), B, C, H, W,
           stream_ptr())
    return dx, stats


def upsample2x_fwd(x, pro=None, relu=False):
    _chk(x, "x")
    B, C, H, W = x.shape
    out = torch.empty((B, C, 2 * H, 2 * W), dtype=torch.float32, device=x.device)
    lib().call("wtpse_upsample2x_fwd", ptr(x), ptr(pro), int(relu), ptr(out), B, C, H, W, stream_ptr())
    return out


def upsample2x_fwd_stats(x):
    _chk(x, "x")
    B, C, H, W = x.shape
    out = torch.empty((B, C, 2 * H, 2 * W), dtype=torch.float32, device=x.device)
# ... 545 lines not shown
```

Baseline: 818.9.

## Add thin-channel x2h conv path for 16-32 channel 3x3 dgrad

Adds a new conv kernel mode (MODE 5/6) that handles 3x3 convolutions with 17-32 input channels and at most 16 outputs. It stages the input as two 16-channel chunks of split fp16 terms in shared memory and runs 16x16x32 MFMA with prefetch of the second chunk. Layers with cin<=16 and 16<cout<=32 now use this path for their dgrad instead of the fp32 or x3 paths, and the packer emits two-chunk weights for them. The aim is to cut the per-layer cost of thin dgrad convolutions, at the price of a new code path and extra packed-weight storage.

Measured after the change: 820.6 (median of 5 runs). Within noise of the previous version (+0.2%).

```diff
diff --git a/include/wtpse_hip.h b/include/wtpse_hip.h
--- a/include/wtpse_hip.h
+++ b/include/wtpse_hip.h
@@ -32,6 +32,11 @@
                     const float* bn_mean, int bn_relu, int B, int H, int W, int Cout, int relu_out, int in_is_grad,
                     const unsigned* in_amax, unsigned* out_amax, void* stream);
 int wtpse_pack_conv16_x3(const float* params, const int* desc, int n_desc, unsigned short* packed, void* stream);
+int wtpse_conv_thin(const float* in0, int C0, const float* in1, int C1, const unsigned short* wthin, const float* bias,
+                    const float* pro0, const float* pro1, int pro_relu, float* out0, float* stats, const float* mask_ref,
+                    const float* bn_ss, const float* bn_mean, int bn_relu, int B, int H, int W, int Cout, int relu_out,
+                    int in_is_grad, const unsigned* in_amax0, const unsigned* in_amax1, unsigned* out_amax, void* stream);
+int wtpse_thin_x2h(int on);
 
 int wtpse_dgrad_bnb(const float* dy, int C, const float* wpacked, float* out0, float* out1, int Csplit, const float* bn_y,
                     const float* bn_ss, const float* bn_mean, int bn_relu, int bn_c0, int bn_c1, float* stats, int B, int H, int W,
diff --git a/wt-pse-code_amd/wtpse_hip/csrc/conv.hip b/wt-pse-code_amd/wtpse_hip/csrc/conv.hip
--- a/wt-pse-code_amd/wtpse_hip/csrc/conv.hip
+++ b/wt-pse-code_amd/wtpse_hip/csrc/conv.hip
@@ -29,6 +29,7 @@
   int relu_out;
   int tiles_x, tiles_y;
   int xcd_tiles;
+  const unsigned* in_amax1;
 };
 
 
@@ -52,8 +53,10 @@
   constexpr int NPOS = (PE + 255) / 256;
   constexpr int S = PlaneStride<NPOS * 256>::value;
   constexpr bool XP = (MODE == 3 || MODE == 4);
-  constexpr int XT = MODE == 4 ? 2 : 3;
-  constexpr bool P16 = (MODE == 0) || XP;
+  constexpr bool XW = (MODE == 5 || MODE == 6);
+  constexpr int XT = (MODE == 4 || MODE == 6) ? 2 : 3;
+  constexpr bool P16 = (MODE == 0) || XP || XW;
+  static_assert(!XW || KS == 3, "MODE 5 / 6 is a 3x3 path");
   static_assert(!XP || KS == 3, "MODE 3 / 4 is the 3x3 path");
   constexpr int MT = P16 ? 1 : MODE;
   constexpr int MB = P16 ? 16 : 32;
@@ -66,8 +69,8 @@
   constexpr int CB4 = CB / 4;
   constexpr int NW = (KC * TAPS * CB4 + 255) / 256;
   constexpr int PEP = (PE + 7) & ~7;
-  constexpr int XS_SZ = XP ? 2 * XT * PEP * 4 : KC * S;
-  constexpr int WS_SZ = XP ? 0 : NW * 1024;
+  constexpr int XS_SZ = (XP || XW) ? 2 * XT * PEP * 4 : KC * S;
+  constexpr int WS_SZ = (XP || XW) ? 0 : NW * 1024;
   constexpr int GRAM_SZ = (P16 && KS == 3) ? 4 * 16 * 65 + 4 * 256 : 0;
   constexpr int RED_SZ = 4 * CB * 2 > GRAM_SZ ? 4 * CB * 2 : GRAM_SZ;
   constexpr int MAIN_SZ = (XS_SZ + WS_SZ) > RED_SZ ? (XS_SZ + WS_SZ) : RED_SZ;
@@ -227,6 +230,132 @@
       }
     }
     if constexpr (MODE == 4) {
+      const float inv = a.wp[0] / sx;
+#pragma unroll
+      for (int nt = 0; nt < NT; ++nt) acc[0][nt] *= inv;
+    }
+    __syncthreads();
+  } else if constexpr (XW) {
+    constexpr bool X2H = MODE == 6;
+    u32x4* Xq = reinterpret_cast<u32x4*>(smem);
+    const int g4 = lane >> 4;
+    constexpr int PB = (PE + 63) / 64, NIT = (2 * PB + 3) / 4;
+    const __amdgpu_buffer_rsrc_t rs0 = make_rsrc(a.in0 + (size_t)b * a.C0 * HW, (unsigned)a.C0 * HW * 4u);
+    const __amdgpu_buffer_rsrc_t rs1 = a.in1 ? make_rsrc(a.in1 + (size_t)b * a.C1 * HW, (unsigned)a.C1 * HW * 4u) : rs0;
+    const bool any_pro = X2H || a.pro0 != nullptr || a.pro1 != nullptr || a.pro_relu != 0;
+    const unsigned sx_raw = X2H ? max(amax_load(a.in_amax), amax_load(a.in_amax1)) : 0u;
+    __builtin_amdgcn_sched_barrier(0);
+    float xv[NIT][8];
+    int ipos[NIT], ihalf[NIT];
+    bool iin[NIT];
+    unsigned vo[NIT];
+#pragma unroll
+    for (int i = 0; i < NIT; ++i) {
+      const int blk = __builtin_amdgcn_readfirstlane(i * 4 + wave);
+      ihalf[i] = blk >= PB ? 1 : 0;
+      const int p = (blk - ihalf[i] * PB) * 64 + lane;
+      ipos[i] = (blk < 2 * PB && p < PE) ? p : -1;
+      const int r = p / PITCH, x = p - r * PITCH;
+      const int gy = ty * TH + r - PAD, gx = tx * TW + x - PAD;
+      iin[i] = ipos[i] >= 0 && gy >= 0 && gy < a.H && gx >= 0 && gx < a.W;
+      vo[i] = iin[i] ? (unsigned)(gy * a.W + gx) * 4u : BUF_OOB;
+    }
+    auto issue = [&](int ch) {
+      const bool first = ch * 16 < a.C0;
+      const __amdgpu_buffer_rsrc_t rs = first ? rs0 : rs1;
+      const int cbase = first ? ch * 16 : ch * 16 - a.C0, cn = first ? a.C0 : a.C1;
+#pragma unroll
+      for (int i = 0; i < NIT; ++i)
+#pragma unroll
+        for (int j = 0; j < 8; ++j)
+          xv[i][j] = buf_load(rs, vo[i], (unsigned)min(cbase + ihalf[i] * 8 + j, cn) * (unsigned)HW * 4u);
+    };
+    issue(0);
+    const u32x4* wq = reinterpret_cast<const u32x4*>(a.wp) + 1 + (X2H ? 2 * 15 * 64 : 0);
+    const float sx = X2H ? (a.in_amax ? x3_scale_from_amax(amax_reduce(sx_raw)) : a.in_scale) : 1.f;
+    int toff[5];
+#pragma unroll
+    for (int s5 = 0; s5 < 5; ++s5) {
+      const int t = min(2 * s5 + (g4 >> 1), TAPS - 1);
+      toff[s5] = (t / KS) * PITCH + (t % KS);
+    }
+    const int hsel = (g4 & 1) * PEP;
+#pragma unroll
+    for (int ch = 0; ch < 2; ++ch) {
+      const bool first = ch * 16 < a.C0;
+      const int cbase = first ? ch * 16 : ch * 16 - a.C0, cn = first ? a.C0 : a.C1;
+      const float* pro = first ? a.pro0 : a.pro1;
+      if (any_pro) {
+        const float lo = (a.pro_relu & (first ? 1 : 2)) ? 0.f : -INFINITY;
+        float psc[2][8], psh[2][8];
+#pragma unroll
+        for (int hh = 0; hh < 2; ++hh)
+#pragma unroll
+          for (int j = 0; j < 8; ++j) {
+            const int cg = min(cbase + hh * 8 + j, cn - 1);
+            psc[hh][j] = (pro ? pro[2 * cg] : 1.f) * sx;
+            psh[hh][j] = (pro ? pro[2 * cg + 1] : 0.f) * sx;
+          }
+#pragma unroll
+        for (int i = 0; i < NIT; ++i) {
+          const int nc = iin[i] ? cn - cbase - ihalf[i] * 8 : 0;
+#pragma unroll
+          for (int j = 0; j < 8; ++j) {
+            const float sc = ihalf[i] ? psc[1][j] : psc[0][j], sh = ihalf[i] ? psh[1][j] : psh[0][j];
+            const float v = fmaxf(fmaf(xv[i][j], sc, sh), lo);
+            xv[i][j] = j < nc ? v : 0.f;
+          }
+        }
+      }
+      if (ch) __syncthreads();
+#pragma unroll
+      for (int i = 0; i < NIT; ++i) {
+        if (ipos[i] >= 0) {
+          u32x4 tt[XT];
+#pragma unroll
+          for (int j = 0; j < 4; ++j) {
+            unsigned q0, q1, q2 = 0u;
+            if constexpr (XT == 3) wt_split3_pair(xv[i][2 * j], xv[i][2 * j + 1], q0, q1, q2);
+            else split2h_pair(xv[i][2 * j], xv[i][2 * j + 1], q0, q1);
+            tt[0][j] = q0; tt[1][j] = q1;
+            if constexpr (XT == 3) tt[2][j] = q2;
+          }
+#pragma unroll
+          for (int t = 0; t < XT; ++t) Xq[(t * 2 + ihalf[i]) * PEP + ipos[i]] = tt[t];
+        }
+      }
+      u32x4 afr[5][XT];
+#pragma unroll
+      for (int s5 = 0; s5 < 5; ++s5)
+#pragma unroll
+        for (int t = 0; t < XT; ++t) afr[s5][t] = wq[((ch * 5 + s5) * XT + t) * 64 + lane];
+      __syncthreads();
+      if (ch == 0) issue(1);
+#pragma unroll
+      for (int nt = 0; nt < NT; ++nt) {
+#pragma unroll
+        for (int s5 = 0; s5 < 5; ++s5) {
+          u32x4 bfr[XT];
+#pragma unroll
+          for (int t = 0; t < XT; ++t) bfr[t] = Xq[(t * 2) * PEP + hsel + off[nt] + toff[s5]];
+          f32x4 c = acc[0][nt];
+          if constexpr (XT == 3) {
+            c = wt_mfma16x32(afr[s5][0], bfr[2], c);
+            c = wt_mfma16x32(afr[s5][1], bfr[1], c);
+            c = wt_mfma16x32(afr[s5][2], bfr[0], c);
+            c = wt_mfma16x32(afr[s5][0], bfr[1], c);
+            c = wt_mfma16x32(afr[s5][1], bfr[0], c);
+            c = wt_mfma16x32(afr[s5][0], bfr[0], c);
+          } else {
+            c = wt_mfma16x32h(afr[s5][0], bfr[1], c);
+            c = wt_mfma16x32h(afr[s5][1], bfr[0], c);
+            c = wt_mfma16x32h(afr[s5][0], bfr[0], c);
+          }
+          acc[0][nt] = c;
+        }
+      }
+    }
+    if constexpr (X2H) {
       const float inv = a.wp[0] / sx;
 #pragma unroll
       for (int nt = 0; nt < NT; ++nt) acc[0][nt] *= inv;
@@ -560,7 +689,7 @@
 
 template <int KS, int MODE, bool DB, int EPI>
 static int launch_fwd(const ConvArgs& a, hipStream_t st) {
-  constexpr int CB = (MODE == 0 || MODE == 3 || MODE == 4) ? 16 : 32 * MODE;
+  constexpr int CB = (MODE == 0 || MODE >= 3) ? 16 : 32 * MODE;
   ConvArgs args = a;
   const Tiling t = conv_tiling(a.B, a.H, a.W);
   args.tiles_x = t.tiles_x;
@@ -587,7 +716,7 @@
   const BnbTail& t = c.tail;
   const BnfTail& f = c.ftail;
   const bool bnb = bn.mean != nullptr;
-  WTPSE_REQUIRE(layout == CONV_FP32 || layout == CONV_X3 || layout == CONV_C16);
+  WTPSE_REQUIRE(layout == CONV_FP32 || layout == CONV_X3 || layout == CONV_C16 || layout == CONV_THIN);
   WTPSE_REQUIRE(c.in0 && c.w && c.out0 && c.B > 0 && c.H > 0 && c.W > 0 && c.C0 > 0 && c.C1 >= 0 && c.Cout > 0);
   WTPSE_REQUIRE(c.ksize == 1 || c.ksize == 3);
   WTPSE_REQUIRE((c.C1 == 0) == (c.in1 == nullptr));
@@ -610,10 +739,16 @@
   }
   if (layout == CONV_C16)
     WTPSE_REQUIRE(c.ksize == 3 && c.C0 <= 16 && c.Cout <= 16 && (((uintptr_t)c.w) & 15) == 0 && !c.in1 && !c.pro1);
+  if (layout == CONV_THIN)
+    WTPSE_REQUIRE(c.ksize == 3 && c.Cout <= 16 && c.C0 + c.C1 > 16 && c.C0 + c.C1 <= 32 && (!c.in1 || c.C0 == 16) && !c.gram &&
+                  (bnb || !c.stats) &&
+                  (((uintptr_t)c.w) & 15) == 0 && (!c.in1 || (c.in_amax0 == nullptr) == (c.in_amax1 == nullptr)) &&
+                  !(c.in_amax1 && !c.in1));
   return 0;
 }
 
-static int conv_launch_fwd(const ConvCall& c, bool c16, hipStream_t st) {
+static int conv_launch_fwd(const ConvCall& c, int layout, hipStream_t st) {
+  const bool c16 = layout == CONV_C16, thin = layout == CONV_THIN;
   const bool bnb = c.bn.mean != nullptr;
   ConvArgs a;
   a.tail = c.tail;
@@ -621,12 +756,14 @@
   a.bn_ss = c.bn.ss; a.bn_mean = c.bn.mean; a.bn_relu = c.bn.relu; a.bn_c0 = bnb ? c.bn.c0 : 0; a.bn_c1 = bnb ? c.bn.c1 : 0;
   a.in0 = c.in0; a.in1 = c.in1; a.wp = static_cast<const float*>(c.w); a.bias = c.bias; a.pro0 = c.pro0; a.pro1 = c.pro1;
   a.out0 = c.out0; a.out1 = c.out1; a.stats = c.stats; a.mask = c.mask_ref; a.gram = c.gram;
-  a.in_amax = c16 ? c.in_amax0 : nullptr; a.in_scale = c16 ? X3_FWD_SCALE : 1.f; a.out_amax = c.out_amax;
-  a.B = c.B; a.H = c.H; a.W = c.W; a.C0 = c.C0; a.C1 = c.C1; a.Cin = c.C0 + c.C1; a.CinP = c16 ? 16 : (a.Cin + 3) & ~3;
+  a.in_amax = (c16 || thin) ? c.in_amax0 : nullptr; a.in_amax1 = thin ? c.in_amax1 : nullptr;
+  a.in_scale = (c16 || thin) ? X3_FWD_SCALE : 1.f; a.out_amax = c.out_amax;
+  a.B = c.B; a.H = c.H; a.W = c.W; a.C0 = c.C0; a.C1 = c.C1; a.Cin = c.C0 + c.C1; a.CinP = c16 ? 16 : thin ? 32 : (a.Cin + 3) & ~3;
   a.Cout = c.Cout; a.CoutP = (c.Cout + 15) & ~15; a.Csplit = c.Csplit; a.pro_relu = c.pro_relu; a.relu_out = c.relu_out;
   a.tiles_x = a.tiles_y = 0;
 #define FWD(KS, M, DB) (bnb ? launch_fwd<KS, M, DB, 2>(a, st) : c.mask_ref ? launch_fwd<KS, M, DB, 1>(a, st) : launch_fwd<KS, M, DB, 0>(a, st))
   if (c16) return (g_x3_terms == 2 && (!c.in_is_grad || c.in_amax0)) ? FWD(3, 4, false) : FWD(3, 3, false);
+  if (thin) return (g_x3_terms == 2 && (!c.in_is_grad || c.in_amax0)) ? FWD(3, 6, false) : FWD(3, 5, false);
   int mode = c.Cout <= 16 ? 0 : (c.Cout % 64 == 0 ? 2 : 1);
   const int tiles = conv_tiling(c.B, c.H, c.W).tiles;
   if (mode == 2 && tiles * (a.CoutP / 64) < 512) mode = 1;
@@ -642,7 +779,7 @@
 
 int conv_run(const ConvCall& c, int layout, hipStream_t st) {
   if (const int rc = conv_check(c, layout)) return rc;
-  return layout == CONV_X3 ? conv_launch_x3(c, st) : conv_launch_fwd(c, layout == CONV_C16, st);
+  return layout == CONV_X3 ? conv_launch_x3(c, st) : conv_launch_fwd(c, layout, st);
 }
 
 extern "C" int wtpse_conv_fwd(const float* in0, int C0, const float* in1, int C1, const float* wpacked,
@@ -677,6 +814,25 @@
   c.bn.ss = bn_ss; c.bn.mean = bn_mean; c.bn.relu = bn_relu; c.bn.c1 = Cout;
   c.B = B; c.H = H; c.W = W; c.Cout = Cout; c.ksize = 3; c.relu_out = relu_out;
   return conv_run(c, CONV_C16, (hipStream_t)stream);
+}
+
+extern "C" int wtpse_conv_thin(const float* in0, int C0, const float* in1, int C1, const unsigned short* wthin, const float* bias,
+                               const float* pro0, const float* pro1, int pro_relu, float* out0, float* stats, const float* mask_ref,
+                               const float* bn_ss, const float* bn_mean, int bn_relu, int B, int H, int W, int Cout, int relu_out,
+                               int in_is_grad, const unsigned* in_amax0, const unsigned* in_amax1, unsigned* out_amax, void* stream) {
+  ConvCall c;
+  c.in0 = in0; c.C0 = C0; c.in1 = in1; c.C1 = C1; c.w = wthin; c.bias = bias; c.pro0 = pro0; c.pro1 = pro1; c.pro_relu = pro_relu;
+  c.out0 = out0; c.Csplit = Cout; c.stats = stats; c.mask_ref = mask_ref; c.in_amax0 = in_amax0; c.in_amax1 = in_amax1;
+  c.in_is_grad = in_is_grad; c.out_amax = out_amax;
+  c.bn.ss = bn_ss; c.bn.mean = bn_mean; c.bn.relu = bn_relu; c.bn.c1 = Cout;
+  c.B = B; c.H = H; c.W = W; c.Cout = Cout; c.ksize = 3; c.relu_out = relu_out;
+  return conv_run(c, CONV_THIN, (hipStream_t)stream);
+}
+
+int g_thin_x2h = [] { const char* e = getenv("WTPSE_THIN_X2H"); return (e && e[0] == '0') ? 0 : 1; }();
+extern "C" int wtpse_thin_x2h(int on) {
+  if (on >= 0) g_thin_x2h = on ? 1 : 0;
+  return g_thin_x2h;
 }
 
 extern "C" int wtpse_conv_fwd_bnf(const float* in0, int C0, const float* in1, int C1, const void* wpacked, int layout,
@@ -761,10 +917,11 @@
       float* hdr = reinterpret_cast<float*>(packed + base);
       hdr[0] = 1.f / sc; hdr[1] = sc; hdr[2] = hdr[3] = 0.f;
     }
-    for (int e = blockIdx.x * 256 + threadIdx.x; e < 5 * 64 * 8; e += gridDim.x * 256) {
+    const int nch = d[6 + dir] ? 2 : 1;
+    for (int e = blockIdx.x * 256 + threadIdx.x; e < nch * 5 * 64 * 8; e += gridDim.x * 256) {
       const int j = e & 7, lane = (e >> 3) & 63, s5 = e >> 9;
       const int row = lane & 15, g = lane >> 4;
-      const int tap = 2 * s5 + (g >> 1), k = 8 * (g & 1) + j;
+      const int tap = 2 * (s5 % 5) + (g >> 1), k = 16 * (s5 / 5) + 8 * (g & 1) + j;
       float v = 0.f;
       if (tap < 9 && row < R && k < K) v = dir == 0 ? w[(row * Ci + k) * 9 + tap] : w[(k * Ci + row) * 9 + (8 - tap)];
       unsigned q0, q1, q2;
@@ -774,7 +931,7 @@
       o[((s5 * 3 + 1) * 64 + lane) * 8 + j] = (unsigned short)(q1 & 0xFFFFu);
       o[((s5 * 3 + 2) * 64 + lane) * 8 + j] = (unsigned short)(q2 & 0xFFFFu);
       split2h_pair(v * sc, 0.f, q0, q1);
-      unsigned short* oh = o + 5 * 3 * 64 * 8;
+      unsigned short* oh = o + nch * 5 * 3 * 64 * 8;
       oh[((s5 * 2 + 0) * 64 + lane) * 8 + j] = (unsigned short)(q0 & 0xFFFFu);
       oh[((s5 * 2 + 1) * 64 + lane) * 8 + j] = (unsigned short)(q1 & 0xFFFFu);
     }
diff --git a/wt-pse-code_amd/wtpse_hip/csrc/conv_x3.hip b/wt-pse-code_amd/wtpse_hip/csrc/conv_x3.hip
--- a/wt-pse-code_amd/wtpse_hip/csrc/conv_x3.hip
+++ b/wt-pse-code_amd/wtpse_hip/csrc/conv_x3.hip
@@ -120,7 +120,9 @@
   return was;
 }
 
-extern "C" int wtpse_tuning_state(void) { return g_x3_terms | (g_x3r << 4) | (g_x3_xcd << 8) | (g_x3_small_wide << 12); }
+extern "C" int wtpse_tuning_state(void) {
+  return g_x3_terms | (g_x3r << 4) | (g_x3_xcd << 8) | (g_x3_small_wide << 12) | (g_thin_x2h << 16);
+}
 
 static bool x3_mt2(int B, int H, int W, int CoutP) {
   const int tiles = conv_tiling(B, H, W).tiles;
diff --git a/wt-pse-code_amd/wtpse_hip/csrc/internal.h b/wt-pse-code_amd/wtpse_hip/csrc/internal.h
--- a/wt-pse-code_amd/wtpse_hip/csrc/internal.h
+++ b/wt-pse-code_amd/wtpse_hip/csrc/internal.h
@@ -5,6 +5,7 @@
 #define WTPSE_INTERNAL __attribute__((visibility("hidden")))
 
 WTPSE_INTERNAL extern int g_x3_terms;
+WTPSE_INTERNAL extern int g_thin_x2h;
 
 struct BnbArgs {
   const float* ss = nullptr;
@@ -29,7 +30,7 @@
   BnfTail ftail = bnf_tail_none();
   int B = 0, H = 0, W = 0, Cout = 0, ksize = 0, relu_out = 0;
 };
-enum { CONV_FP32 = 0, CONV_X3 = 1, CONV_C16 = 2 };
+enum { CONV_FP32 = 0, CONV_X3 = 1, CONV_C16 = 2, CONV_THIN = 3 };
 WTPSE_INTERNAL int conv_run(const ConvCall& c, int layout, hipStream_t st);
 WTPSE_INTERNAL int conv_launch_x3(const ConvCall& c, hipStream_t st);
 
diff --git a/wt-pse-code_amd/wtpse_hip/nn.py b/wt-pse-code_amd/wtpse_hip/nn.py
--- a/wt-pse-code_amd/wtpse_hip/nn.py
+++ b/wt-pse-code_amd/wtpse_hip/nn.py
@@ -179,6 +179,11 @@
         self._x16_convs = []
         for c in self._convs:
             c.x16f_off = c.x16d_off = -1
+            c.x16d_two = 0
+            if THIN_X2H and c.k == 3 and c.cin <= 16 and 16 < c.cout <= 32:
+                c.x16d_off, c.x16d_two = off, 1
+                off += ops.X16_SIZE2
+                self._x16_convs.append(c)
             if X16 and c.k == 3 and c.cin <= 16 and c.cout <= 16:
                 if c.cin >= X16_MIN_K:
                     c.x16f_off = off
@@ -196,7 +201,7 @@
             if c.xf_off < 0:
                 c.wf_off = off
                 off += ((c.cin + 3) & ~3) * t * ((c.cout + 15) & ~15)
-            if c.xd_off < 0:
+            if c.xd_off < 0 and not c.x16d_two:
                 c.wd_off = off
                 off += ((c.cout + 3) & ~3) * t * ((c.cin + 15) & ~15)
         self._packed_size = max(off, 4)
@@ -234,15 +239,16 @@
         object.__setattr__(self, "_gwork", None)
         object.__setattr__(self, "_packed", torch.empty(self._packed_size, dtype=torch.float32, device=dev))
 
-        def table(convs, fwd, bwd):
-            desc = [v for c in convs for v in (self.param_offset(c.weight), c.cout, c.cin, c.k * c.k, getattr(c, fwd), getattr(c, bwd), 0, 0)]
+        def table(convs, fwd, bwd, fwd_two=None, bwd_two=None):
+            desc = [v for c in convs for v in (self.param_offset(c.weight), c.cout, c.cin, c.k * c.k, getattr(c, fwd), getattr(c, bwd),
+                                               getattr(c, fwd_two, 0) if fwd_two else 0, getattr(c, bwd_two, 0) if bwd_two else 0)]
             return torch.tensor(desc, dtype=torch.int32).to(dev) if desc else None
 
         object.__setattr__(self, "_desc", table(self._convs, "wf_off", "wd_off"))
         object.__setattr__(self, "_packed_version", -1)
         object.__setattr__(self, "_x3", torch.empty(max(self._x3_size, 8), dtype=torch.int16, device=dev))
         object.__setattr__(self, "_xdesc", table(self._x3_convs, "xf_off", "xd_off"))
-        object.__setattr__(self, "_x16desc", table(self._x16_convs, "x16f_off", "x16d_off"))
+        object.__setattr__(self, "_x16desc", table(self._x16_convs, "x16f_off", "x16d_off", None, "x16d_two"))
         object.__setattr__(self, "_flag", torch.zeros(1, dtype=torch.int32, device=dev))
         ops._tickets(0, dev)
         ops.amax_begin(dev)
@@ -434,6 +440,7 @@
 WGRAD_R = os.environ.get("WTPSE_WGRAD_R", "1") != "0"
 X16 = os.environ.get("WTPSE_X16", "1") != "0" and X3
 X16_MIN_K = int(os.environ.get("WTPSE_X16_MIN_K", "8"))
+THIN_X2H = os.environ.get("WTPSE_THIN_X2H", "1") != "0" and X16
 
 
 def x3_eligible(k_dim, rows, ksize):
@@ -443,6 +450,8 @@
 def _weights(layer, dgrad=False, wide=False):
     root = layer._root
     x16, x3, w = (layer.x16d_off, layer.xd_off, layer.wd_off) if dgrad else (layer.x16f_off, layer.xf_off, layer.wf_off)
+    if dgrad and layer.x16d_two:
+        return 3, root.x3_ptr(x16)
     if x16 >= 0 and not wide:
         return 2, root.x3_ptr(x16)
     if x3 >= 0:
@@ -495,12 +504,14 @@
             tail += (root.gbias(below.conv),)
         d0, d1, stats, coef = ops.dgrad_bnb(dy, wptr, layout, layer.cin, layer.k, below.y, below.ss, below.mean, below.relu, split,
                                             below1 is not None and below0 is None, tail,
-                                            _gamax(dy) if layout == 1 else getattr(dy, "wt_amax", None) if layout == 2 else None)
+                                            _gamax(dy) if layout == 1 else getattr(dy, "wt_amax", None) if layout >= 2 else None)
         if below0 is not None:
             return PreBN(d0, stats, coef), d1
         return d0, PreBN(d1, stats, coef)
     if layout == 2:
         return ops.conv16_x3(dy, wptr, None, layer.cin, mask_ref=mask_ref, grad_in=True)[0], None
+    if layout == 3:
+        return ops.conv_thin(dy, None, wptr, None, layer.cin, mask_ref=mask_ref, grad_in=True)[0], None
     if layout == 1:
         return ops.conv_fwd_x3(dy, None, wptr, None, layer.cin, layer.k, None, 0, False, False, split, mask_ref, None, _gamax(dy))[:2]
     return ops.conv_fwd(dy, None, wptr, None, layer.cin, layer.k, None, 0, False, False, split, mask_ref)[:2]
diff --git a/wt-pse-code_amd/wtpse_hip/ops.py b/wt-pse-code_amd/wtpse_hip/ops.py
--- a/wt-pse-code_amd/wtpse_hip/ops.py
+++ b/wt-pse-code_amd/wtpse_hip/ops.py
@@ -109,6 +109,35 @@
     if out_amax is not None:
         out.wt_amax = out_amax
     return out, stats, ((gram, nblk // B) if want_gram else None)
+
+
+X16_SIZE2 = 8 + 2 * (X16_SIZE - 8)
+
+
+def conv_thin(in0, in1, wthin_ptr, bias, cout, pro0=None, pro1=None, pro_relu=0, relu_out=False, mask_ref=None, bnb=None,
+              grad_in=False, in_amax0=None, in_amax1=None, out_amax=None):
+    _chk(in0, "in0"); _chk(in1, "in1"); _chk(pro0, "pro0"); _chk(pro1, "pro1"); _chk(mask_ref, "mask_ref")
+    B, C0, H, W = in0.shape
+    C1 = 0 if in1 is None else in1.shape[1]
+    out = torch.empty((B, cout, H, W), dtype=torch.float32, device=in0.device)
+    nblk = _stats_blocks(3, B, H, W)
+    stats = torch.empty((nblk, cout, 2), dtype=torch.float32, device=in0.device) if bnb is not None else None
+    bn_ss = bn_mean = None
+    bn_relu = 0
+    if bnb is not None:
+        mask_ref, bn_ss, bn_mean, bn_relu = bnb
+        _chk(mask_ref, "bn_y"); _chk(bn_ss, "bn_ss"); _chk(bn_mean, "bn_mean")
+        assert mask_ref.shape == out.shape
+    if grad_in:
+        in_amax0 = getattr(in0, "wt_amax", None)
+    if in1 is not None and (in_amax0 is None or in_amax1 is None):
+        in_amax0 = in_amax1 = None
+    lib().call("wtpse_conv_thin", ptr(in0), C0, ptr(in1), C1, wthin_ptr, ptr(bias), ptr(pro0), ptr(pro1), int(pro_relu), ptr(out),
+               ptr(stats), ptr(mask_ref), ptr(bn_ss), ptr(bn_mean), int(bool(bn_relu)), B, H, W, cout, int(relu_out), int(bool(grad_in)),
+               ptr(in_amax0), ptr(in_amax1), ptr(out_amax), stream_ptr())
+    if out_amax is not None:
+        out.wt_amax = out_amax
+    return out, stats
 
 
 def x3_packed_size(rows, k, taps):
@@ -298,6 +327,9 @@
     if layout == 2:
         L.call("wtpse_conv16_x3", ptr(dy), C, wpacked_ptr, 0, 0, 0, ptr(out0), ptr(stats), 0, ptr(bn_y), ptr(bn_ss), ptr(bn_mean),
                int(bool(bn_relu)), B, H, W, cout, 0, 1, ptr(in_amax), 0, stream_ptr())
+    elif layout == 3:
+        L.call("wtpse_conv_thin", ptr(dy), C, 0, 0, wpacked_ptr, 0, 0, 0, 0, ptr(out0), ptr(stats), ptr(bn_y), ptr(bn_ss), ptr(bn_mean),
+               int(bool(bn_relu)), B, H, W, cout, 0, 1, ptr(in_amax), 0, 0, stream_ptr())
     elif layout == 1:
         L.call("wtpse_dgrad_x3_bnb", ptr(dy), C, wpacked_ptr, ptr(out0), ptr(out1), csplit, ptr(bn_y), ptr(bn_ss), ptr(bn_mean),
                int(bool(bn_relu)), c0, c1, ptr(stats), B, H, W, cout, ksize, ptr(in_amax), stream_ptr())
```
